# skyzh/tiny-llm

Hardware: AMD Instinct MI355X
Metric: Qwen3-4B int4 decode tokens/sec/GPU; achieved HBM GB/s vs roofline (higher is better)
Workload: dtype bf16; 1 GPU; Qwen3-4B int4 single-prompt KV-cache decode (BASELINE.json configs[1]); decode_steps=2003, batch_per_gpu=1, parallelism=request-parallel x1 (no collective on the data path), page_size=128, graph_replay=True, prefill_step=128, replay_route=aql

## Files before the change

### include/tinyllm_engine.h

```cpp
#ifndef TINYLLM_ENGINE_H
#define TINYLLM_ENGINE_H

#include <stddef.h>
#include <stdint.h>

#ifdef __cplusplus
extern "C" {
#endif

typedef struct tl_engine tl_engine;

typedef struct tl_w4 {
    const uint32_t *weight_dev;
    const void *scales_dev;
    const void *biases_dev;
    int rows;
    int cols;
} tl_w4;

typedef struct tl_layer_weights {
    tl_w4 wqkv, wo, wgu, wdown;
    const void *input_norm_dev;
    const void *post_norm_dev;
    const void *q_norm_dev;
// ... 75 lines not shown
    long parks, unparks, pages_out, pages_in;
    size_t record_bytes;
} tl_swap_stats;
int tl_engine_swap_space(tl_engine *e, int host_pages);
int tl_engine_park(tl_engine *e, int slot);
int tl_engine_unpark(tl_engine *e, int slot);
int tl_engine_slot_parked(const tl_engine *e, int slot);
int tl_engine_step_pages(const tl_engine *e, int batch, int *need, int *obtainable);
int tl_engine_swap_stats(const tl_engine *e, tl_swap_stats *out);
size_t tl_kv_page_record_bytes(const tl_kv_pool_desc *pools_host, int n_pools, int heads, int page_size);
int tl_kv_gather_pages(const tl_kv_pool_desc *pools_dev, const size_t *record_offsets_dev, int n_pools, int heads, int page_size,
                       const int32_t *page_ids_dev, int n_pages, int tail_rows, void *staging_dev, size_t record_bytes, void *stream);
int tl_kv_scatter_pages(const tl_kv_pool_desc *pools_dev, const size_t *record_offsets_dev, int n_pools, int heads, int page_size,
                        const int32_t *page_ids_dev, int n_pages, int tail_rows, const void *staging_dev, size_t record_bytes, void *stream);

int tl_engine_verify(tl_engine *e, int slot, const int32_t *tokens, int n, int32_t *out_ids);

int tl_engine_verify_sampled(tl_engine *e, int slot, const int32_t *tokens, int n, const void *draft_logits_dev, float draft_temperature,
                             int draft_top_k, float draft_top_p, int32_t *out_ids, int *out_count);

int tl_engine_set_token(tl_engine *e, int slot, int32_t token);

int tl_engine_set_sampling(tl_engine *e, int slot, float temperature, int top_k, float top_p, uint64_t seed);

#define TL_MAX_TOP_LOGPROBS 20
typedef struct tl_token_logprob {
    float logprob;
    int32_t top_ids[TL_MAX_TOP_LOGPROBS];
    float top_logprobs[TL_MAX_TOP_LOGPROBS];
} tl_token_logprob;
int tl_engine_set_logprobs(tl_engine *e, int slot, int top_n);
int tl_engine_read_logprobs(tl_engine *e, int slot, int count, tl_token_logprob *out);
int tl_engine_read_pending_logprobs(tl_engine *e, int count, tl_token_logprob *out);

#define TL_MAX_LOGIT_BIAS 1024
int tl_engine_set_penalties(tl_engine *e, int slot, float repetition_penalty, float presence_penalty, float frequency_penalty);
int tl_engine_set_logit_bias(tl_engine *e, int slot, const int32_t *ids, const float *values, int n);

int tl_engine_set_truncation(tl_engine *e, int slot, float min_p, float typical_p);
int tl_engine_set_mirostat(tl_engine *e, int slot, float tau, float eta);
int tl_engine_mirostat_mu(tl_engine *e, int slot, float *mu);
int tl_engine_copy_filtered_logits(tl_engine *e, void *dst_dev, int rows);

typedef struct tl_vocab tl_vocab;
typedef struct tl_grammar tl_grammar;
#define TL_GRAMMAR_END (-1)
int tl_vocab_create(int vocab, const int32_t *offsets, const uint8_t *bytes, void *stream, tl_vocab **out);
void tl_vocab_destroy(tl_vocab *v);
int tl_grammar_create(const tl_vocab *v, int n_states, const uint16_t *table, const uint8_t *accepting, int start, const int32_t *eos_ids,
                      int n_eos, void *stream, tl_grammar **out);
void tl_grammar_destroy(tl_grammar *g);
int tl_engine_set_grammar(tl_engine *e, int slot, const tl_grammar *g);
int tl_engine_grammar_state(tl_engine *e, int slot, int *state, int *accepting);
int tl_grammar_mask_rows(const tl_grammar *g, const void *logits_dev, int rows, const int32_t *states_dev, void *out_dev, void *stream);

int tl_grammar_create_stack(const tl_vocab *v, int n_states, const uint16_t *table, const uint8_t *ops, int n_pop, const uint16_t *pop_table,
                            const uint8_t *accepting, int start, const int32_t *eos_ids, int n_eos, void *stream, tl_grammar **out);
int tl_engine_grammar_config(tl_engine *e, int slot, int *state, int *depth, uint64_t *stack, int *accepting);
int tl_grammar_mask_rows_stack(const tl_grammar *g, const void *logits_dev, int rows, const int32_t *states_dev, const int32_t *depths_dev,
                               const uint64_t *stacks_dev, void *out_dev, void *stream);

int tl_engine_score(tl_engine *e, int slot, const int32_t *tokens, int n, int32_t next_token, float *out_logprobs, int32_t *out_argmax);

#define TL_POOL_LAST 0
#define TL_POOL_MEAN 1
int tl_engine_embed_packed(tl_engine *e, int n_seqs, const int *slots, const int32_t *tokens, const int *lens, const int *finish, int pooling,
                           int normalize, int dim, float *out_host);
int tl_engine_embed(tl_engine *e, int slot, const int32_t *tokens, int n, int finish, int pooling, int normalize, int dim, float *out_host);

#define TL_MAX_LORA_RANK 64
#define TL_MAX_LORA_ADAPTERS 32
enum { TL_LORA_Q, TL_LORA_K, TL_LORA_V, TL_LORA_O, TL_LORA_GATE, TL_LORA_UP, TL_LORA_DOWN, TL_LORA_TARGETS };
typedef struct tl_lora_layer {
    const void *a_dev[TL_LORA_TARGETS], *b_dev[TL_LORA_TARGETS];
} tl_lora_layer;
typedef struct tl_lora_stats {
    int resident;
    size_t bytes;
    long adapter_steps;
    long adapter_prefill_rows;
} tl_lora_stats;
int tl_engine_lora_load(tl_engine *e, const tl_lora_layer *layers, int rank, float scale, int *adapter);
int tl_engine_lora_unload(tl_engine *e, int adapter);
int tl_engine_set_lora(tl_engine *e, int slot, int adapter);
int tl_engine_slot_lora(const tl_engine *e, int slot);
int tl_engine_lora_stats(const tl_engine *e, tl_lora_stats *out);

enum { TL_LORA_ADD = 0, TL_LORA_RESIDUAL_PRE = 1, TL_LORA_SWIGLU = 2 };
typedef struct tl_lora_matrices {
    const void *a_dev, *b_dev;
    int rank, seg_mask;
    float scale;
} tl_lora_matrices;
int tl_lora_rows(const void *x_dev, int rows, int in, int out, const int32_t *row_adapter_dev, const tl_lora_matrices *adapters, int n_adapters,
                 int seg_mode, int seg_end0, int seg_end1, const int *tile_row0, const int *tile_rows, const int *tile_adapter, int n_tiles, int mode,
                 const void *base_or_residual_dev, void *out_dev, const void *norm_w_dev, float eps, void *stream);

#define TL_MAX_STOP_IDS 16
#define TL_MAX_STOP_STRINGS 16
#define TL_MAX_STOP_BYTES 1024
enum { TL_STOP_NONE = 0, TL_STOP_ID = 1, TL_STOP_STRING = 2, TL_STOP_LENGTH = 3 };
typedef struct tl_stop tl_stop;
typedef struct tl_stop_state {
    int32_t reason, index, generated, context;
    uint32_t text_bytes, cut_bytes;
} tl_stop_state;
int tl_stop_create(const tl_vocab *v, const int32_t *ids, int n_ids, const uint8_t *bytes, const int32_t *offsets, int n_strings, void *stream,
                   tl_stop **out);
void tl_stop_destroy(tl_stop *s);
int tl_engine_set_stop(tl_engine *e, int slot, const tl_stop *set, int max_new_tokens);
int tl_engine_stop_state(tl_engine *e, int slot, tl_stop_state *out);
int tl_stop_rows(const tl_stop *set, const int32_t *tokens_dev, int rows, const int32_t *armed_dev, const int32_t *max_new_dev,
                 int32_t *automaton_dev, tl_stop_state *states_dev, void *stream);

int tl_engine_decode(tl_engine *e, int batch, int steps, int use_graph);

int tl_engine_read_tokens(tl_engine *e, int slot, int count, int32_t *out);

int tl_engine_read_pending(tl_engine *e, int count, int32_t *out);

const void *tl_engine_logits_dev(const tl_engine *e);
int tl_engine_copy_logits(tl_engine *e, void *dst_dev, int rows);
int tl_engine_copy_processed_logits(tl_engine *e, void *dst_dev, int rows);
const int32_t *tl_engine_tokens_dev(const tl_engine *e);

int tl_engine_get_stats(const tl_engine *e, tl_engine_stats *out);

const char *tl_engine_replay_route(const tl_engine *e);

size_t tl_engine_step_bytes(const tl_engine *e, int batch);

typedef struct tl_step_profile {
    double kernel_us[8];
    int launches[8];
    double gemv_bytes[5];
    double span_us;
    int clock_khz;
    int n_splits;
} tl_step_profile;
int tl_engine_profile_step(tl_engine *e, int batch, tl_step_profile *out);

typedef struct tl_step_check {
    int launches, written_once_plan, n_splits;
    long double_writes, elements_written;
    int first_launch, first_kind, first_region;
    long first_offset;
} tl_step_check;
int tl_engine_check_step(tl_engine *e, int batch, tl_step_check *out);


typedef struct tl_tiled_w4 tl_tiled_w4;
int tl_tiled_w4_create(const tl_w4 *w, void *stream, tl_tiled_w4 **out);
void tl_tiled_w4_destroy(tl_tiled_w4 *t);

typedef struct tl_linear_info {
    int kernel;
    int launches;
    int rows_per_pass;
    int p[5];
} tl_linear_info;

size_t tl_decode_linear_workspace_bytes(int M, int rows, int cols);
int tl_decode_linear(const tl_tiled_w4 *w, const void *a_dev, void *out_dev, int M, int prologue, int epilogue,
                     const void *norm_w_dev, const void *residual_dev, float eps, int kernel, void *workspace_dev,
                     size_t workspace_bytes, void *stream, tl_linear_info *info);

typedef struct tl_linear_ex {
    const float *merge_ws_dev;
    int n_splits;
    const float *ss_in_dev;
    int ss_in_n;
    float *ss_out_dev;
    const void *norm_out_dev;
    void *out_w_dev;
    int fragment_order;
} tl_linear_ex;
int tl_decode_linear_ex(const tl_tiled_w4 *w, const void *a_dev, void *out_dev, int M, int prologue, int epilogue,
                        const void *norm_w_dev, const void *residual_dev, float eps, int kernel, void *workspace_dev,
                        size_t workspace_bytes, void *stream, const tl_linear_ex *ex, tl_linear_info *info);

int tl_prefill_weights_bf16(const tl_w4 *w, void *out_dev, void *stream);
int tl_prefill_matmul_bf16(const void *a_dev, const void *w_bf16_dev, void *out_dev, int M, int rows, int cols, int epilogue,
                           const void *residual_dev, void *stream);

int tl_decode_gemv_plan(int M, int rows, int cols, int *out5);
int tl_decode_gemv_variant_compiled(int MR, int KS, int CW, int LM);
int tl_decode_batched_plan(int M, int rows, int cols, int *out6);
int tl_decode_batched_variant_compiled(int MB, int GPW);
int tl_decode_streaming_plan(int M, int rows, int cols, int *out4);
int tl_decode_streaming_variant_compiled(int T, int GPW);
int tl_decode_attention_plan(int batch, int max_context, int num_heads, int num_kv_heads, int *out3);

typedef struct tl_attention_info {
    int n_splits, tokens_per_split, heads_per_workgroup;
    int launches;
} tl_attention_info;
size_t tl_decode_attention_fused_workspace_bytes(int batch, int num_heads, int head_dim);
int tl_decode_attention_fused(const void *qkv_dev, const void *q_norm_dev, const void *k_norm_dev, void *key_pages_dev,
                              void *value_pages_dev, const int32_t *block_table_dev, const int32_t *context_lens_dev,
                              void *out_dev, int batch, int num_heads, int num_kv_heads, int head_dim, int page_size,
                              int max_pages, float rope_theta, float eps, int max_context, void *workspace_dev,
                              size_t workspace_bytes, void *stream, tl_attention_info *info);
int tl_decode_attention_fused_fp8(const void *qkv_dev, const void *q_norm_dev, const void *k_norm_dev, void *key_pages_dev,
                                  float *key_scales_dev, void *value_pages_dev, float *value_scales_dev,
                                  const int32_t *block_table_dev, const int32_t *context_lens_dev, void *out_dev, int batch,
                                  int num_heads, int num_kv_heads, int head_dim, int page_size, int max_pages, float rope_theta,
                                  float eps, int max_context, void *workspace_dev, size_t workspace_bytes, void *stream,
                                  tl_attention_info *info);

int tl_sample_logits(const void *logits_dev, int rows, int vocab, const float *temperature_dev, const int32_t *top_k_dev,
                     const float *top_p_dev, const uint64_t *seed_dev, const int32_t *position_dev, int32_t *ids_dev, void *stream);

int tl_spec_sample_rows(const void *target_logits_dev, const void *draft_logits_dev, int rows, int vocab, const int32_t *proposal_dev,
                        const float *temperature_dev, const int32_t *top_k_dev, const float *top_p_dev, const float *draft_temperature_dev,
                        const int32_t *draft_top_k_dev, const float *draft_top_p_dev, const uint64_t *seed_dev, const int32_t *position_dev,
                        int32_t *accept_dev, int32_t *alt_dev, void *stream);

int tl_logprob_rows(const void *logits_dev, int rows, int vocab, const int32_t *ids_dev, int top_n, float *logprob_dev, int32_t *top_ids_dev,
                    float *top_logprobs_dev, void *stream);

int tl_pool_rows(const void *rows_dev, int hidden, int n_seqs, const int *row0, const int *len, const int *finish, const int *prior, int pooling,
                 float *sums_dev, int normalize, int dim, float *out_dev, void *stream);

int tl_truncate_rows(const void *logits_dev, int rows, int vocab, const float *temperature_dev, const float *min_p_dev, const float *typical_p_dev,
                     const float *mu_dev, void *out_dev, float *kept_logsum_dev, void *stream);
int tl_mirostat_update_rows(const void *filtered_dev, int rows, int vocab, const int32_t *ids_dev, const float *temperature_dev,
                            const float *kept_logsum_dev, const float *tau_dev, const float *eta_dev, float *mu_dev, void *stream);

int tl_process_logits(const void *logits_dev, int rows, int vocab, const uint16_t *history_dev, const float *repetition_dev,
                      const float *presence_dev, const float *frequency_dev, const int32_t *bias_ids_dev, const float *bias_values_dev,
                      const int32_t *bias_n_dev, void *out_dev, void *stream);

#ifdef __cplusplus
}
#endif
#endif
```

### tiny-llm_amd/csrc/decode_linear.h

```cpp
#pragma once

#include <algorithm>
#include <cstdlib>
#include <initializer_list>
#include <map>
#include <memory>
#include <string>
#include <vector>

#include "../../include/tinyllm_engine.h"
#include "common.h"
#include "device_block.h"
#include "engine_kernels.h"
#include "qmv.h"
#include "qmv3.h"
#include "qmm3.h"
#include "qmm6.h"
#include "qmm7.h"
#include "gemm8.h"

namespace tl {

#define TL_TRY(expr)                  \
    do {                              \
        const int rc__ = (expr);      \
        if (rc__ != TL_OK) return rc__; \
    } while (0)

struct WrittenOnceCheck {
    char *region[2] = {nullptr, nullptr};
    size_t bytes[2] = {0, 0};
    uint32_t *shadow[2] = {nullptr, nullptr};
    uint8_t *written[2] = {nullptr, nullptr};
    unsigned long long *report = nullptr;
};

struct ProfCtx {
    hipStream_t stream = nullptr;
    const WrittenOnceCheck *check = nullptr;
    DeviceBlock buf_mem, pairs_mem;
    prof_t *buf = nullptr;
    prof_t *pairs = nullptr;
    std::vector<int> kinds;
    int cap = 0;
    bool alloc(const tl_engine_config &c, int batch, hipStream_t st) {
        stream = st;
        const size_t buf_bytes = (size_t)(std::max(c.vocab_size / 4 + 64, 64 * 4 * c.num_kv_heads * batch) + 1024) * 2 * sizeof(prof_t);
        cap = c.num_layers * 12 + 8;
        if (buf_mem.alloc(buf_bytes, "hipMalloc(stamps) failed") != TL_OK || pairs_mem.alloc((size_t)cap * 2 * sizeof(prof_t), "hipMalloc(stamp pairs) failed") != TL_OK)
            return false;
        buf = buf_mem.at<prof_t>(), pairs = pairs_mem.at<prof_t>();
        return hipMemsetAsync(buf, 0, buf_bytes, stream) == hipSuccess;
    }
};

static void prof_after(ProfCtx *pc, int kind, int n_wg) {
    const int idx = (int)pc->kinds.size();
    if (idx >= pc->cap) return;
    hipLaunchKernelGGL(prof_reduce_kernel, dim3(1), dim3(1024), 0, pc->stream, pc->buf, n_wg, pc->pairs + 2 * (size_t)idx);
    pc->kinds.push_back(kind);
    if (pc->check)
        for (int rg = 0; rg < 2; ++rg)
            if (pc->check->bytes[rg])
                hipLaunchKernelGGL(written_once_check_kernel, dim3(1024), dim3(256), 0, pc->stream, (const uint32_t *)pc->check->region[rg],
                                   pc->check->shadow[rg], pc->check->written[rg], pc->check->bytes[rg] / 4, idx, rg, pc->check->report);
}

struct TiledW4 {
    uint32_t *wt = nullptr, *sbt = nullptr;
};
struct TiledW4Mem {
    DeviceBlock wt, sbt;
};
static int tiled_w4_make(const tl_w4 &w, hipStream_t st, TiledW4Mem &mem, TiledW4 &t, const char *alloc_failed, const char *repack_failed) {
    const size_t wbytes = (size_t)w.rows * w.cols / 2, sbytes = (size_t)w.rows * (w.cols / 128) * 4;
    TiledW4Mem m;
    TL_TRY(m.wt.alloc(wbytes + 16384, alloc_failed));
    TL_TRY(m.sbt.alloc(sbytes + 1024, alloc_failed));
    if (repack_w4_tiled(w.weight_dev, (const uint16_t *)w.scales_dev, (const uint16_t *)w.biases_dev, m.wt.at<uint32_t>(), m.sbt.at<uint32_t>(), w.rows,
                        w.cols, st) != 0)
        return fail(TL_ERR_HIP, repack_failed);
    t.wt = m.wt.at<uint32_t>(), t.sbt = m.sbt.at<uint32_t>();
    mem = std::move(m);
    return TL_OK;
}

struct LinearCtx {
    hipStream_t stream = nullptr;
    float rms_norm_eps = 0.f;
    std::map<const uint32_t *, TiledW4> tiled;
    std::map<const uint32_t *, uint16_t *> bf16w;
    uint16_t *xn = nullptr;
    void *splitk_ws = nullptr;
    size_t splitk_ws_bytes = 0;
    uint16_t *gu = nullptr, *tmp = nullptr;
    bool use_gemm8 = true;
    bool fuse_reduce_norm = true;
    bool gemm_fused_epilogue = true;
    bool gemv_producer_ss = true;
    bool gemv_weighted_rows = true;
    bool fuse_norm = true;
    int qmm3_min_rows = 5;
    bool use_qmm3 = true;
    bool use_qmm6 = true;
    bool use_qmm7 = true, force_qmm7 = false;
    tl_linear_info *linfo = nullptr;
    int force_linear = 0;
    int qmm3_mode = -1;
    void read_env() { if (const char *q = getenv("TL_QMM3_MIN_M")) qmm3_min_rows = std::max(1, atoi(q)); }
};

struct KeptPartials {
    const float *partial = nullptr;
    int slices = 0;
    long plane = 0;
};

struct Proj {
    const tl_w4 *w = nullptr;
    const uint16_t *a = nullptr;
    uint16_t *out = nullptr;
    int M = 0;
    int pro = PRO_NONE, epi = EPI_STORE;
    const void *norm_w = nullptr;
    const uint16_t *residual = nullptr;
    int kind = 0;
    const float *ss_in = nullptr;
    int ss_in_n = QM3_SS;
    float *ss_out = nullptr;
    const void *norm_out = nullptr;
    uint16_t *out_w = nullptr;
    bool frag = false;
    int out_w_frag = -1;
    bool keep = false;
    float *planes = nullptr;
    size_t planes_bytes = 0;
    const float *merge_ws = nullptr;
    int n_splits = 0;
    f32x2 *tile_max = nullptr;
};
static Proj proj(const tl_w4 &w, const uint16_t *a, uint16_t *out, int M) { return Proj{&w, a, out, M}; }

struct ProjResult {
    int ss_n = 0;
    KeptPartials kept;
    int maxima_rows = 0;
};

static int check_w4(const tl_w4 &w, int rows, int cols, const char *name) {
    if (!w.weight_dev || !w.scales_dev || !w.biases_dev)
        return fail(TL_ERR_INVALID, std::string("engine: null weight pointer in ") + name);
    if (w.rows != rows || w.cols != cols)
        return fail(TL_ERR_INVALID, std::string("engine: unexpected shape for ") + name + " (got " +
                                        std::to_string(w.rows) + "x" + std::to_string(w.cols) + ", want " +
                                        std::to_string(rows) + "x" + std::to_string(cols) + ")");
    if ((uintptr_t)w.weight_dev % 16 != 0)
        return fail(TL_ERR_INVALID, std::string("engine: weight not 16-byte aligned: ") + name);
    return TL_OK;
}

static void report_launch(const LinearCtx &ctx, int kernel, int launches, int rows_per_pass, std::initializer_list<int> plan = {}) {
    if (!ctx.linfo) return;
    tl_linear_info &li = *ctx.linfo;
    li.kernel = kernel == 1 && li.kernel == 3 ? 3 : kernel;
    li.launches += launches;
    li.rows_per_pass = rows_per_pass;
    std::copy(plan.begin(), plan.end(), li.p);
}

static int engine_qmv(LinearCtx &ctx, const Proj &p, ProfCtx *pc = nullptr, ProjResult *res = nullptr) {
    ProjResult none, &r = res ? *res : none;
    r = ProjResult{};
    const tl_w4 &w = *p.w;
    const int M = p.M;
    const bool merge = p.pro == PRO_ATTN_MERGE;
    bool all_emitted = p.ss_out != nullptr && p.epi == EPI_RESIDUAL && ctx.gemv_producer_ss;
    int step = std::min(M, 8);
    const auto tiled = ctx.tiled.find(w.weight_dev);
    const bool has_tiled = tiled != ctx.tiled.end();
    auto fits = [&](int rows) {
        return (has_tiled && qmv3_plan(rows, w.cols, w.rows).ok) || qmv_plan(rows, w.cols, w.rows).lds <= 150 * 1024;
    };
    while (!fits(step) && step > 1) step = (step + 1) / 2;
    const int out_cols = p.epi == EPI_SWIGLU ? w.rows / 2 : w.rows;
    for (int m0 = 0; m0 < M; m0 += step) {
        QmvArgs args{};
        args.scales = (const uint16_t *)w.scales_dev;
        args.biases = (const uint16_t *)w.biases_dev;
        args.b = w.weight_dev;
        args.a = p.a + (size_t)m0 * w.cols;
        args.out = p.out + (size_t)m0 * out_cols;
        args.norm_w = (const uint16_t *)p.norm_w;
        args.residual = p.residual ? p.residual + (size_t)m0 * w.rows : nullptr;
        args.eps = ctx.rms_norm_eps;
        args.M = std::min(step, M - m0);
        args.N = w.cols;
        args.K = w.rows;
        args.prof = pc ? pc->buf : nullptr;
        const Qmv3Plan p3 = qmv3_plan(args.M, args.N, args.K);
        if (has_tiled && (p3.ok || merge)) {
            Qmv3Args a3{};
            a3.wt = tiled->second.wt;
            a3.sbt = tiled->second.sbt;
            a3.a = merge ? nullptr : args.a;
            a3.merge_ws = merge ? const_cast<float *>(p.merge_ws) : nullptr;
            a3.out = args.out;
            a3.norm_w = args.norm_w;
            a3.residual = args.residual;
            a3.eps = args.eps;
            a3.M = args.M;
            a3.N = args.N;
            a3.K = args.K;
            a3.prof = args.prof;
            if (ctx.gemv_producer_ss) {
                if ((p.pro == PRO_RMSNORM || p.pro == PRO_RMS_WEIGHTED) && p.ss_in && p.ss_in_n > 0)
                    a3.ss_in = p.ss_in + (size_t)m0 * p.ss_in_n, a3.ss_n = p.ss_in_n;
                if (p.epi == EPI_RESIDUAL && p.ss_out) a3.ss_out = p.ss_out + (size_t)m0 * (w.rows / 16);
            }
            if (p.tile_max && p.epi == EPI_STORE && step == M && w.rows % 16 == 0) {
                a3.tile_max = p.tile_max;
                r.maxima_rows = M;
            }
            if (p.out_w) {
                TL_REQUIRE(p.epi == EPI_RESIDUAL && p.norm_out && step == M, "engine: weighted rows need the residual epilogue and one pass");
                a3.norm_out = (const uint16_t *)p.norm_out;
                a3.out_w = p.out_w;
            }
            if ((merge ? launch_qmv3_attn_merge_bf16(a3, p.n_splits, ctx.stream) : launch_qmv3_bf16(a3, p.pro, p.epi, ctx.stream)) != 0)
                return fail(TL_ERR_UNSUPPORTED, merge ? "engine: no wo GEMV that merges the attention partials for this shape" : "engine: MFMA GEMV launch failed");
            if (pc) prof_after(pc, p.kind, p3.blocks);
            report_launch(ctx, 1, 1, step, {p3.MR, p3.KS, p3.CW, p3.LM, p3.blocks});
            continue;
        }
        all_emitted = false;
        TL_REQUIRE(p.out_w == nullptr && p.pro != PRO_RMS_WEIGHTED && !merge, "engine: weighted rows are a route of the MFMA GEMV only");
        if (launch_qmv_fused_bf16(args, p.pro, p.epi, ctx.stream) != 0)
            return fail(TL_ERR_UNSUPPORTED, "engine: no GEMV configuration for this shape");
        if (pc) prof_after(pc, p.kind, qmv_plan(args.M, args.N, args.K).blocks);
        report_launch(ctx, 3, 1, step);
    }
    TL_CHECK_LAUNCH(merge ? "engine wo gemv with merge" : "engine gemv");
    if (all_emitted && w.rows % 16 == 0) r.ss_n = w.rows / 16;
    return TL_OK;
}

static int ensure_splitk(const LinearCtx &ctx, size_t bytes) {
    if (bytes <= ctx.splitk_ws_bytes) return TL_OK;
    return fail(TL_ERR_INVALID, "engine: matmul workspace too small for this shape (sized at tl_engine_create: " +
                                    std::to_string(ctx.splitk_ws_bytes) + " bytes, need " + std::to_string(bytes) + ")");
}

static int engine_qmm(LinearCtx &ctx, const tl_w4 &w, const uint16_t *a, uint16_t *out, int M) {
    const size_t need = tl_quantized_matmul_workspace_bytes(M, w.cols, w.rows, TL_BF16, 1, 1);
    TL_TRY(ensure_splitk(ctx, need));
    return tl_quantized_matmul(w.scales_dev, w.biases_dev, a, w.weight_dev, out, M, w.cols, w.rows, 128, 4, TL_BF16, 1, 1,
                               ctx.splitk_ws, ctx.splitk_ws_bytes, ctx.stream);
}

constexpr int GEMM8_MIN_ROWS = 1792;
static bool gemm8_wins(int M) { return M >= GEMM8_MIN_ROWS; }
static int engine_gemm(LinearCtx &ctx, const Proj &p, bool *norm_done = nullptr) {
    const tl_w4 &w = *p.w;
    const int M = p.M;
    if (norm_done) *norm_done = false;
    if (ctx.use_gemm8 && gemm8_wins(M)) {
        const auto wb = ctx.bf16w.find(w.weight_dev);
        if (wb != ctx.bf16w.end() && gemm8_applicable(M, w.rows, w.cols)) {
            Gemm8Args g{};
            g.a = p.a, g.w = wb->second, g.out = p.out, g.residual = p.residual, g.M = M, g.N = w.rows, g.K = w.cols;
            if (launch_gemm8_bf16(g, p.epi, ctx.stream) != 0) return fail(TL_ERR_UNSUPPORTED, "engine: bf16 GEMM launch failed");
            TL_CHECK_LAUNCH("engine bf16 matmul");
            return TL_OK;
        }
    }
    if (p.epi != EPI_STORE && M > 8 && ctx.gemm_fused_epilogue) {
        const size_t need = tl_quantized_matmul_workspace_bytes(M, w.cols, w.rows, TL_BF16, 1, 1);
        TL_TRY(ensure_splitk(ctx, need));
        TL_TRY(qmm_bf16_epilogue(w.scales_dev, w.biases_dev, p.a, w.weight_dev, p.out, M, w.cols, w.rows, p.epi, p.residual, ctx.splitk_ws,
                                 ctx.splitk_ws_bytes, ctx.stream, ctx.fuse_reduce_norm ? (const uint16_t *)p.norm_out : nullptr, p.out_w,
                                 ctx.rms_norm_eps, norm_done));
        TL_CHECK_LAUNCH("engine matmul");
        return TL_OK;
    }
    uint16_t *plain = p.epi == EPI_STORE ? p.out : (p.epi == EPI_SWIGLU ? ctx.gu : ctx.tmp);
    TL_TRY(engine_qmm(ctx, w, p.a, plain, M));
    if (p.epi == EPI_SWIGLU) {
        const long n4 = (long)M * (w.rows / 2) / 4;
        hipLaunchKernelGGL(swiglu_interleaved_kernel, dim3(ceil_div(n4, 256)), dim3(256), 0, ctx.stream, plain, p.out, n4);
    } else if (p.epi == EPI_RESIDUAL) {
        const long n8 = (long)M * w.rows / 8;
        hipLaunchKernelGGL(residual_add_kernel, dim3(ceil_div(n8, 256)), dim3(256), 0, ctx.stream, p.residual, plain, p.out, n8);
    }
    TL_CHECK_LAUNCH("engine matmul");
    return TL_OK;
}

static bool qmm6_takes(const LinearCtx &ctx, const tl_w4 &w, int M) {
    return ctx.use_qmm6 && ctx.force_linear == 0 && M >= ctx.qmm3_min_rows && M <= 64 && ctx.tiled.count(w.weight_dev) != 0 &&
           qmm6_plan(M, w.cols, w.rows).ok;
}
static int engine_qmm6(LinearCtx &ctx, const Proj &p, ProfCtx *pc = nullptr, ProjResult *res = nullptr) {
    ProjResult none, &r = res ? *res : none;
    r = ProjResult{};
    const tl_w4 &w = *p.w;
    const int M = p.M;
    const auto tiled = ctx.tiled.find(w.weight_dev);
    TL_REQUIRE(tiled != ctx.tiled.end(), "engine: the register-resident matmul needs the tiled weights");
    const bool a_frag = p.frag && p.ss_in != nullptr && p.epi != EPI_RESIDUAL;
    const Qmm7Plan p7 = (ctx.use_qmm7 || ctx.force_qmm7) && a_frag && p.out_w == nullptr ? qmm7_plan(M, w.cols, w.rows) : Qmm7Plan{};
    TL_REQUIRE(p7.ok || !ctx.force_qmm7, "engine: the row-streaming matmul takes weighted rows in fragment order (store / SwiGLU) at the shapes of qmm7_plan");
    const Qmm6Plan pl = qmm6_plan(M, w.cols, w.rows, a_frag);
    TL_REQUIRE(p7.ok || pl.ok, "engine: the register-resident matmul does not cover this shape");
    Qmm6Args q{};
    q.wt = tiled->second.wt;
    q.sbt = tiled->second.sbt;
    q.a = p.a;
    q.out = p.out;
    q.residual = p.residual;
    q.norm_out = (const uint16_t *)p.norm_out;
    q.out_w = p.out_w;
    q.ss = p.ss_in;
    q.ss_n = p.ss_in ? p.ss_in_n : 0;
    q.ss_out = p.epi == EPI_RESIDUAL ? p.ss_out : nullptr;
    q.eps = ctx.rms_norm_eps;
    q.M = M;
    q.N = w.cols;
    q.K = w.rows;
    q.prof = pc ? pc->buf : nullptr;
    q.a_frag = a_frag;
    q.out_w_frag = (p.out_w_frag >= 0 ? p.out_w_frag != 0 : p.frag) && p.out_w != nullptr;
    int n_wg = 0;
    if (p7.ok) {
        if (launch_qmm7_bf16(q, p.epi, ctx.stream, &n_wg) != 0) return fail(TL_ERR_UNSUPPORTED, "engine: row-streaming matmul launch failed");
        if (pc) prof_after(pc, p.kind, n_wg);
        report_launch(ctx, 6, 1, p7.MB * 16, {p7.MB, p7.GPW, p7.T, p7.row_blocks, n_wg});
        TL_CHECK_LAUNCH("engine row-streaming matmul");
        return TL_OK;
    }
    if (launch_qmm6_bf16(q, p.epi, ctx.stream, &n_wg) != 0) return fail(TL_ERR_UNSUPPORTED, "engine: register-resident matmul launch failed");
    if (pc) prof_after(pc, p.kind, n_wg);
    if (q.ss_out) r.ss_n = w.rows / 16;
    report_launch(ctx, 5, 1, pl.MB * 16, {pl.MB, pl.GPW, pl.NSETS, pl.row_blocks, n_wg});
    TL_CHECK_LAUNCH("engine register-resident matmul");
    return TL_OK;
}

static bool gemv_takes_rows(const LinearCtx &ctx, int M) {
    return ctx.force_linear == 1 || (ctx.force_linear != 2 && (M < ctx.qmm3_min_rows || (M <= 8 && !ctx.use_qmm3)));
}
static bool weighted_rows_apply(const LinearCtx &ctx, const tl_w4 &producer, const tl_w4 &consumer, int M) {
    if (!ctx.gemv_weighted_rows || !ctx.gemv_producer_ss || !gemv_takes_rows(ctx, M) || M > 8) return false;
    if (ctx.tiled.count(producer.weight_dev) == 0 || ctx.tiled.count(consumer.weight_dev) == 0) return false;
    const Qmv3Plan pp = qmv3_plan(M, producer.cols, producer.rows), pcn = qmv3_plan(M, consumer.cols, consumer.rows);
    if (!pp.ok || !pcn.ok || producer.rows != consumer.cols) return false;
    return qmv3_takes_weighted_rows(pcn, consumer.cols, producer.rows / 16);
}
static bool takes_skinny_matmul(const LinearCtx &ctx, const tl_w4 &w, int M) {
    return !gemv_takes_rows(ctx, M) && ctx.use_qmm3 && M <= 64 && ctx.tiled.count(w.weight_dev) != 0 && qmm3_plan(M, w.cols, w.rows, ctx.qmm3_mode).ok;
}

static int engine_linear(LinearCtx &ctx, const Proj &p, ProfCtx *pc = nullptr, ProjResult *res = nullptr) {
    ProjResult none, &r = res ? *res : none;
    r = ProjResult{};
    const tl_w4 &w = *p.w;
    const int M = p.M;
    if (gemv_takes_rows(ctx, M)) return engine_qmv(ctx, p, pc, &r);
    TL_REQUIRE(p.pro != PRO_ATTN_MERGE, "engine: merged attention partials are a route of the fused GEMV only");
    TL_REQUIRE(p.pro != PRO_RMS_WEIGHTED && (p.out_w == nullptr || (p.epi == EPI_RESIDUAL && p.norm_out != nullptr)),
               "engine: the skinny matmul leaves weighted rows behind a residual epilogue only, and takes none");
    const float *ss_in = qmm3_takes_ss(p.ss_in_n) ? p.ss_in : nullptr;
    const uint16_t *in = p.a;
    if (takes_skinny_matmul(ctx, w, M)) {
        const auto tiled = ctx.tiled.find(w.weight_dev);
        const Qmm3Plan p3 = qmm3_plan(M, w.cols, w.rows, ctx.qmm3_mode);
        const bool fused_norm = p.pro == PRO_RMSNORM && ss_in != nullptr && ctx.fuse_norm;
        if (p.pro == PRO_RMSNORM && !fused_norm) {
            TL_TRY(tl_rms_norm(p.a, p.norm_w, ctx.xn, M, w.cols, ctx.rms_norm_eps, TL_BF16, ctx.stream));
            in = ctx.xn;
        }
        if (p.planes) TL_REQUIRE(p3.partial_bytes <= p.planes_bytes, "engine: per-layer slice planes too small for this shape");
        else TL_TRY(ensure_splitk(ctx, p3.partial_bytes));
        Qmm3Args q{};
        q.wt = tiled->second.wt;
        q.sbt = tiled->second.sbt;
        q.a = in;
        q.partial = p.planes ? p.planes : (float *)ctx.splitk_ws;
        q.M = M;
        q.N = w.cols;
        q.K = w.rows;
        q.prof = pc ? pc->buf : nullptr;
        q.norm_w = (const uint16_t *)p.norm_w;
        q.ss = ss_in;
        q.ss_n = p.ss_in_n;
        q.eps = ctx.rms_norm_eps;
        if (launch_qmm3_bf16(q, ctx.stream, fused_norm ? PRO_RMSNORM : PRO_NONE, ctx.qmm3_mode) != 0)
            return fail(TL_ERR_UNSUPPORTED, "engine: skinny matmul launch failed");
        if (pc) prof_after(pc, p.kind, p3.persistent ? p3.grid_x : p3.grid_x * p3.slices);
        float *ss_dst = (p.ss_out && ctx.fuse_norm && qmm3_reduce_can_emit_ss(p.epi, w.rows)) ? p.ss_out : nullptr;
        const bool kept = p.keep && p.epi == EPI_STORE && ss_dst == nullptr;
        if (kept) {
            r.kept.partial = q.partial;
            r.kept.slices = p3.slices;
            r.kept.plane = (long)M * w.rows;
        } else {
            int reduce_wg = 0;
            if (launch_qmm3_reduce_bf16(q.partial, p3.slices, M, w.rows, p.epi, p.residual, p.out, q.prof, ctx.stream, ss_dst, &reduce_wg,
                                        p.out_w ? (const uint16_t *)p.norm_out : nullptr, p.out_w, p.frag ? 1 : 0) != 0)
                return fail(TL_ERR_UNSUPPORTED, "engine: skinny matmul reduction launch failed");
            if (pc) prof_after(pc, p.kind, reduce_wg);
        }
        r.ss_n = ss_dst != nullptr ? QM3_SS : 0;
        TL_CHECK_LAUNCH("engine skinny matmul");
        report_launch(ctx, 2, (kept ? 1 : 2) + (p.pro == PRO_RMSNORM && !fused_norm ? 1 : 0), M,
                      {p3.MB, p3.persistent ? 0 : p3.TW, p3.LM, p3.slices, p3.persistent ? p3.grid_x : p3.grid_x * p3.slices});
        return TL_OK;
    }
    if (ctx.force_linear == 2) return fail(TL_ERR_UNSUPPORTED, "engine: the skinny matmul does not cover this shape");
    TL_REQUIRE(p.out_w == nullptr, "engine: no kernel leaves weighted rows for this shape");
    if (M <= 8) return engine_qmv(ctx, p, pc, &r);
    Proj g = p;
    if (p.pro == PRO_RMSNORM) {
        TL_TRY(tl_rms_norm(p.a, p.norm_w, ctx.xn, M, w.cols, ctx.rms_norm_eps, TL_BF16, ctx.stream));
        g.a = ctx.xn;
    }
    if (ctx.linfo) ctx.linfo->kernel = 4;
    g.norm_out = nullptr;
    return engine_gemm(ctx, g);
}

struct LayerRoute {
    bool batched = false;
    bool qkv6 = false, wo6 = false;
    enum Down { DOWN_ROUTER, DOWN_SLICED_WEIGHTED, DOWN_QMM6 } down = DOWN_ROUTER;
    bool gemv_weighted = false;
    bool batched_written_once() const { return batched && qkv6 && down != DOWN_ROUTER; }
};
static LayerRoute plan_layer(const LinearCtx &ctx, const tl_layer_weights &w, int batch, bool is_moe) {
    LayerRoute r;
    if (is_moe || w.wgu.weight_dev == nullptr) return r;
    auto sliced_leaves_weighted = [&](const tl_w4 &m) {
        return takes_skinny_matmul(ctx, m, batch) && ctx.fuse_norm && qmm3_reduce_can_emit_ss(EPI_RESIDUAL, m.rows);
    };
    auto qmm6_leaves_weighted = [&](const tl_w4 &m) { return qmm6_takes(ctx, m, batch) && qmm3_takes_ss(m.rows / 16); };
    r.gemv_weighted = weighted_rows_apply(ctx, w.wo, w.wgu, batch);
    r.wo6 = qmm6_leaves_weighted(w.wo);
    r.batched = qmm6_takes(ctx, w.wgu, batch) && (r.wo6 || sliced_leaves_weighted(w.wo));
    r.qkv6 = qmm6_takes(ctx, w.wqkv, batch);
    r.down = sliced_leaves_weighted(w.wdown) ? LayerRoute::DOWN_SLICED_WEIGHTED
                                             : (qmm6_leaves_weighted(w.wdown) ? LayerRoute::DOWN_QMM6 : LayerRoute::DOWN_ROUTER);
    return r;
}
static bool rows_travel_in_fragment_order(const LinearCtx &ctx, const tl_layer_weights &first, int batch) {
    if (batch > 8) return true;
    if (!ctx.use_qmm7 || !first.wgu.weight_dev) return false;
    return qmm7_plan(batch, first.wgu.cols, first.wgu.rows).ok && qmm7_plan(batch, first.wqkv.cols, first.wqkv.rows).ok;
}

}

struct tl_tiled_w4 {
    tl_w4 w{};
    tl::TiledW4 t{};
    tl::TiledW4Mem mem;
};

extern "C" int tl_tiled_w4_create(const tl_w4 *w, void *stream, tl_tiled_w4 **out) {
    using namespace tl;
    TL_REQUIRE(w && out, "tiled_w4_create: null argument");
    TL_TRY(check_w4(*w, w->rows, w->cols, "tiled_w4_create"));
    TL_REQUIRE(w->rows > 0 && w->rows % 16 == 0 && w->cols > 0 && w->cols % 128 == 0,
               "tiled_w4_create: rows must be a multiple of 16 and cols a multiple of 128");
    auto t = std::make_unique<tl_tiled_w4>();
    t->w = *w;
    TL_TRY(tiled_w4_make(*w, (hipStream_t)stream, t->mem, t->t, "tiled_w4_create: hipMalloc failed", "tiled_w4_create: repack launch failed"));
    *out = t.release();
    return TL_OK;
}

extern "C" void tl_tiled_w4_destroy(tl_tiled_w4 *t) { delete t; }

extern "C" size_t tl_decode_linear_workspace_bytes(int M, int rows, int cols) {
    using namespace tl;
    if (M <= 0 || rows <= 0 || cols <= 0) return 0;
    size_t need = align_up((size_t)((M + 15) / 16 * 16) * cols * 2, 256);
    size_t partial = 0;
    for (int mode = 0; mode < 2; ++mode) {
        const Qmm3Plan p3 = qmm3_plan(std::min(M, 64), cols, rows, mode);
        if (p3.ok) partial = std::max(partial, p3.partial_bytes);
    }
    return need + partial;
}

static int decode_linear_impl(const tl_tiled_w4 *w, const void *a_dev, void *out_dev, int M, int prologue, int epilogue,
                              const void *norm_w_dev, const void *residual_dev, float eps, int kernel, void *workspace_dev,
                              size_t workspace_bytes, void *stream, const tl_linear_ex *ex, tl_linear_info *info) {
    using namespace tl;
    TL_REQUIRE(w && out_dev, "decode_linear: null argument");
    TL_REQUIRE(M >= 1 && M <= 64, "decode_linear: between 1 and 64 activation rows");
    TL_REQUIRE(prologue == PRO_NONE || prologue == PRO_RMSNORM || (ex && (prologue == PRO_ATTN_MERGE || prologue == PRO_RMS_WEIGHTED)),
               "decode_linear: prologue is 0 (none) or 1 (RMSNorm); tl_decode_linear_ex also takes 2 (merge of attention partials) and 3 (weighted rows)");
    TL_REQUIRE(epilogue == EPI_STORE || epilogue == EPI_RESIDUAL || epilogue == EPI_SWIGLU,
               "decode_linear: epilogue is 0 (store), 1 (residual add) or 2 (SwiGLU over interleaved rows)");
    TL_REQUIRE(prologue == PRO_ATTN_MERGE || a_dev, "decode_linear: null activation rows");
    TL_REQUIRE(prologue != PRO_RMSNORM || norm_w_dev, "decode_linear: the RMSNorm prologue needs its weight");
    TL_REQUIRE(epilogue != EPI_RESIDUAL || residual_dev, "decode_linear: the residual epilogue needs the residual rows");
    TL_REQUIRE(kernel >= 0 && kernel <= 6,
               "decode_linear: kernel is 0 (engine routing), 1 (fused GEMV), 2 (skinny matmul), 3 / 4 (its one-shot / persistent grid), 5 (register-resident matmul), 6 (row-streaming matmul)");
    TL_REQUIRE(epilogue != EPI_SWIGLU || w->w.rows % 2 == 0, "decode_linear: SwiGLU needs an even number of weight rows");
    TL_REQUIRE((prologue == PRO_NONE && epilogue != EPI_SWIGLU) || (prologue == PRO_RMSNORM && epilogue != EPI_RESIDUAL) ||
                   (prologue == PRO_ATTN_MERGE && epilogue == EPI_RESIDUAL) || (prologue == PRO_RMS_WEIGHTED && epilogue == EPI_SWIGLU) ||
                   ((kernel == 5 || kernel == 6) && prologue == PRO_RMS_WEIGHTED && epilogue == EPI_STORE),
               "decode_linear: no fused variant for this prologue / epilogue pair");
    const size_t need = tl_decode_linear_workspace_bytes(M, w->w.rows, w->w.cols);
    TL_REQUIRE(workspace_dev && workspace_bytes >= need, "decode_linear: workspace is missing or too small");
    if (info) *info = tl_linear_info{};
    LinearCtx ctx;
    ctx.rms_norm_eps = eps;
    ctx.stream = (hipStream_t)stream;
    ctx.tiled[w->w.weight_dev] = w->t;
    ctx.xn = (uint16_t *)workspace_dev;
    const size_t xn_bytes = align_up((size_t)((M + 15) / 16 * 16) * w->w.cols * 2, 256);
    ctx.splitk_ws = (char *)workspace_dev + xn_bytes;
    ctx.splitk_ws_bytes = workspace_bytes - xn_bytes;
    ctx.force_linear = kernel >= 2 && kernel <= 4 ? 2 : (kernel >= 5 ? 0 : kernel);
    ctx.use_qmm7 = false, ctx.force_qmm7 = kernel == 6;
    ctx.qmm3_mode = kernel == 3 ? 0 : (kernel == 4 ? 1 : -1);
    ctx.linfo = info;
    ctx.read_env();
    Proj p = proj(w->w, (const uint16_t *)a_dev, (uint16_t *)out_dev, M);
    p.pro = prologue, p.epi = epilogue, p.norm_w = norm_w_dev, p.residual = (const uint16_t *)residual_dev;
    if (ex) {
        p.ss_out = ex->ss_out_dev;
        p.norm_out = ex->norm_out_dev, p.out_w = (uint16_t *)ex->out_w_dev;
    }
    if (kernel == 6 && (prologue != PRO_RMS_WEIGHTED || epilogue == EPI_RESIDUAL))
        return fail(TL_ERR_INVALID, "decode_linear: the row-streaming matmul takes weighted rows with ss_in (prologue 3) and stores or applies SwiGLU (epilogue 0 / 2)");
    if (kernel == 5 || kernel == 6) {
        const bool weighted = prologue == PRO_RMS_WEIGHTED;
        if (prologue == PRO_RMSNORM || prologue == PRO_ATTN_MERGE)
            return fail(TL_ERR_INVALID, "decode_linear: the register-resident matmul takes plain rows (prologue 0) or weighted rows with ss_in (prologue 3)");
        if (weighted && (!ex || !ex->ss_in_dev || !qmm3_takes_ss(ex->ss_in_n)))
            return fail(TL_ERR_INVALID, "decode_linear_ex: weighted rows need ss_in (a multiple of 4, at most 256 partials per row)");
        if (ex && ((ex->out_w_dev != nullptr) != (ex->norm_out_dev != nullptr) || ((ex->out_w_dev || ex->ss_out_dev) && epilogue != EPI_RESIDUAL)))
            return fail(TL_ERR_INVALID, "decode_linear_ex: ss_out / (norm_out, out_w) belong to the residual epilogue; norm_out and out_w come together");
        if (kernel == 5 && !qmm6_plan(M, w->w.cols, w->w.rows).ok)
            return fail(TL_ERR_UNSUPPORTED, "decode_linear: the register-resident matmul does not cover this shape");
        if (kernel == 6 && !qmm7_plan(M, w->w.cols, w->w.rows).ok)
            return fail(TL_ERR_UNSUPPORTED, "decode_linear: the row-streaming matmul does not cover this shape");
        if (weighted && !ex->fragment_order) {
            const long n8 = (long)M * w->w.cols / 8;
            hipLaunchKernelGGL(weight_rows_kernel, dim3(ceil_div(n8, 256)), dim3(256), 0, ctx.stream, p.a, (const uint16_t *)nullptr, ctx.xn, n8, w->w.cols / 8, 1);
            p.a = ctx.xn;
        }
        if (weighted) p.ss_in = ex->ss_in_dev, p.ss_in_n = ex->ss_in_n;
        p.frag = weighted;
        p.out_w_frag = ex && ex->fragment_order ? 1 : 0;
        return engine_qmm6(ctx, p);
    }
    if (!ex) return engine_linear(ctx, p);
    const bool skinny_forced = kernel >= 2 && kernel <= 4;
    const bool gemv_only = prologue == PRO_ATTN_MERGE || prologue == PRO_RMS_WEIGHTED || ex->ss_out_dev || (ex->out_w_dev && !skinny_forced);
    if (gemv_only && !(kernel == 1 || (kernel == 0 && M < ctx.qmm3_min_rows)))
        return fail(TL_ERR_INVALID, "decode_linear_ex: merged partials, weighted rows, ss_out and out_w are routes of the fused GEMV (kernel 1, or 0 with fewer than 5 rows)");
    if ((ex->out_w_dev != nullptr) != (ex->norm_out_dev != nullptr) || (ex->out_w_dev && epilogue != EPI_RESIDUAL) ||
        (ex->ss_out_dev && epilogue != EPI_RESIDUAL))
        return fail(TL_ERR_INVALID, "decode_linear_ex: ss_out / (norm_out, out_w) belong to the residual epilogue; norm_out and out_w come together");
    if (ex->ss_in_dev && (ex->ss_in_n <= 0 || !(prologue == PRO_RMSNORM || prologue == PRO_RMS_WEIGHTED)))
        return fail(TL_ERR_INVALID, "decode_linear_ex: ss_in needs ss_in_n > 0 and a normalising prologue (1 or 3)");
    if (prologue == PRO_ATTN_MERGE) {
        if (M != 1 || !ex->merge_ws_dev) return fail(TL_ERR_INVALID, "decode_linear_ex: the merging prologue takes ONE row and the split partials (merge_ws_dev)");
        p.merge_ws = ex->merge_ws_dev, p.n_splits = ex->n_splits;
    }
    if (prologue == PRO_RMS_WEIGHTED) {
        const Qmv3Plan pl = qmv3_plan(std::min(M, 8), w->w.cols, w->w.rows);
        if (!ex->ss_in_dev || M > 8 || !qmv3_takes_weighted_rows(pl, w->w.cols, ex->ss_in_n))
            return fail(TL_ERR_INVALID, "decode_linear_ex: weighted rows need ss_in (a multiple of 4, at most 256 partials per row), at most 8 rows and a row that fits the staging registers");
    }
    p.ss_in = ex->ss_in_dev, p.ss_in_n = ex->ss_in_n;
    if (gemv_only || kernel == 1 || (kernel == 0 && M < ctx.qmm3_min_rows)) {
        if (M > 8) return fail(TL_ERR_INVALID, "decode_linear_ex: the fused GEMV takes at most 8 rows");
        ProjResult r;
        TL_TRY(engine_qmv(ctx, p, nullptr, &r));
        if (ex->ss_out_dev && r.ss_n != w->w.rows / 16)
            return fail(TL_ERR_UNSUPPORTED, "decode_linear_ex: the GEMV that ran left no sums of squares (packed-dot fallback or several passes)");
        return TL_OK;
    }
    if (ex->ss_in_dev && !qmm3_takes_ss(ex->ss_in_n))
        return fail(TL_ERR_INVALID, "decode_linear_ex: the skinny matmul reads a multiple of 4, at most 256, partial sums of squares per row");
    if (!ex->ss_in_dev) p.ss_in_n = 0;
    p.frag = ex->fragment_order != 0;
    return engine_linear(ctx, p);
}

extern "C" int tl_decode_linear(const tl_tiled_w4 *w, const void *a_dev, void *out_dev, int M, int prologue, int epilogue,
                                const void *norm_w_dev, const void *residual_dev, float eps, int kernel, void *workspace_dev,
                                size_t workspace_bytes, void *stream, tl_linear_info *info) {
    return decode_linear_impl(w, a_dev, out_dev, M, prologue, epilogue, norm_w_dev, residual_dev, eps, kernel, workspace_dev,
                              workspace_bytes, stream, nullptr, info);
}

extern "C" int tl_decode_linear_ex(const tl_tiled_w4 *w, const void *a_dev, void *out_dev, int M, int prologue, int epilogue,
                                   const void *norm_w_dev, const void *residual_dev, float eps, int kernel, void *workspace_dev,
                                   size_t workspace_bytes, void *stream, const tl_linear_ex *ex, tl_linear_info *info) {
    TL_REQUIRE(ex, "decode_linear_ex: null extension block (use tl_decode_linear)");
    return decode_linear_impl(w, a_dev, out_dev, M, prologue, epilogue, norm_w_dev, residual_dev, eps, kernel, workspace_dev,
                              workspace_bytes, stream, ex, info);
}
```

### tiny-llm_amd/csrc/engine.hip

```cpp
#include <dlfcn.h>

#include <cstddef>
#include <cstring>
#include <memory>

#include "decode_linear.h"
#include "device_block.h"
#include "step_end.h"
#include "logit_process.h"
#include "truncate.h"
#include "grammar_stack.h"
#include "attn_mfma.h"
#include "aql.h"
#include "prefix_cache.h"
#include "kv_copy.h"
#include "kv_swap.h"
#include "pool.h"
#include "lora.h"
#include "slot_table.h"
#include "stop.h"
#include "stop_set.h"

namespace tl {

// ... 1296 lines not shown
    const size_t o_log = carve((size_t)std::max(c.max_batch, 8) * c.vocab_size * 2);
    const size_t o_vid = carve(8 * 4);
    const size_t o_tmax = carve((size_t)8 * (c.vocab_size / 16 + 1) * sizeof(f32x2));
    const size_t ss_per_row = (size_t)std::max(QM3_SS, c.hidden_size / 16 + 1);
    const size_t o_ssx = carve((size_t)c.max_batch * ss_per_row * 4);
    const size_t o_ssh = carve((size_t)c.max_batch * ss_per_row * 4);
    const size_t ws_row = (size_t)c.head_dim + ATTN_WS_PAD;
    e->attn_ws_bytes = std::max((size_t)std::max(c.max_batch * 64, 4 * 256) * c.num_heads * ws_row * 4, (size_t)c.num_heads * 8 * 64 * ws_row * 4);
    for (int L = 1; L <= c.max_prefill_rows; ++L)
        e->attn_ws_bytes = std::max(e->attn_ws_bytes, tl_paged_attention_workspace_bytes(c.num_heads, L, c.head_dim, c.page_size,
                                                                                         c.max_pages_per_seq, c.num_heads,
                                                                                         c.num_kv_heads, 0));
    const size_t o_ws = carve(e->attn_ws_bytes);
    e->arena_bytes = carve.off;

    TL_TRY(e->arena.alloc(e->arena_bytes, "engine_create: hipMalloc(arena) failed"));
    TL_TRY(e->smp_mem.alloc((size_t)c.max_batch * 20, "engine_create: hipMalloc(sampling) failed"));
    e->smp_seed = e->smp_mem.at<uint64_t>();
    e->smp_temp = e->smp_mem.at<float>((size_t)c.max_batch * 8);
    e->smp_topk = e->smp_mem.at<int32_t>((size_t)c.max_batch * 12);
    e->smp_topp = e->smp_mem.at<float>((size_t)c.max_batch * 16);
    if (hipMemsetAsync(e->smp_mem.at(), 0, (size_t)c.max_batch * 20, e->stream) != hipSuccess) return fail(TL_ERR_HIP, "engine_create: memset failed");
    e->layer_pool_elems = (size_t)c.num_pages * c.num_kv_heads * c.page_size * c.head_dim;
    const size_t pool_bytes = e->layer_pool_elems * e->kv_elem_bytes() * c.num_layers;
    TL_TRY(e->kv_mem[0].alloc(pool_bytes, "engine_create: hipMalloc(key pages) failed"));
    TL_TRY(e->kv_mem[1].alloc(pool_bytes, "engine_create: hipMalloc(value pages) failed"));
    e->kpool = e->kv_mem[0].at<uint16_t>(), e->vpool = e->kv_mem[1].at<uint16_t>();
    e->kv_bytes = 2 * pool_bytes;
    if (kv_format == TL_KV_FP8_E4M3) {
        e->layer_scale_elems = (size_t)c.num_pages * c.num_kv_heads * c.page_size;
        const size_t scale_bytes = e->layer_scale_elems * 4 * c.num_layers;
        TL_TRY(e->kv_mem[2].alloc(scale_bytes, "engine_create: hipMalloc(key scales) failed"));
        TL_TRY(e->kv_mem[3].alloc(scale_bytes, "engine_create: hipMalloc(value scales) failed"));
        e->kscale_pool = e->kv_mem[2].at<float>(), e->vscale_pool = e->kv_mem[3].at<float>();
        if (hipMemsetAsync(e->kscale_pool, 0, scale_bytes, e->stream) != hipSuccess ||
            hipMemsetAsync(e->vscale_pool, 0, scale_bytes, e->stream) != hipSuccess)
            return fail(TL_ERR_HIP, "engine_create: memset(KV scales) failed");
        e->kv_bytes += 2 * scale_bytes;
    }
    if (hipMemsetAsync(e->kpool, 0, pool_bytes, e->stream) != hipSuccess ||
        hipMemsetAsync(e->vpool, 0, pool_bytes, e->stream) != hipSuccess)
        return fail(TL_ERR_HIP, "engine_create: memset(KV pools) failed");

    char *A = e->arena.at();
    e->block_table = (int32_t *)(A + o_bt);
    e->context_lens = (int32_t *)(A + o_ctx);
    e->tokens = (int32_t *)(A + o_tok);
    e->live = (int32_t *)(A + o_live);
    e->produced = (int32_t *)(A + o_prod);
    e->ring = (int32_t *)(A + o_ring);
    e->scratch_ctx = (int32_t *)(A + o_sctx);
    e->prefill_tokens = (int32_t *)(A + o_ptok);
    e->x = (uint16_t *)(A + o_x);
    e->h = (uint16_t *)(A + o_h);
    e->xn = (uint16_t *)(A + o_xn);
    e->lin.tmp = (uint16_t *)(A + o_tmp);
    e->qkv = (uint16_t *)(A + o_qkv);
    e->q_t = (uint16_t *)(A + o_qt);
    e->attn_t = (uint16_t *)(A + o_at);
    e->attn = (uint16_t *)(A + o_attn);
    e->lin.gu = (uint16_t *)(A + o_gu);
    e->act = (uint16_t *)(A + o_act);
    e->logits = (uint16_t *)(A + o_log);
    e->attn_ws = (float *)(A + o_ws);
    e->verify_ids = (int32_t *)(A + o_vid);
    e->lm_tile_max = (f32x2 *)(A + o_tmax);
    e->ss_x = (float *)(A + o_ssx);
    e->ss_h = (float *)(A + o_ssh);
    e->lin.stream = e->stream, e->lin.rms_norm_eps = c.rms_norm_eps, e->lin.xn = e->xn;
    e->lin.read_env();
    read_attention_knobs(e);
    const char *aql_env = getenv("TL_AQL");
    if (aql_env == nullptr || atoi(aql_env) != 0) {
        {
            AqlRuntime &rt = AqlRuntime::for_device(e->device);
            e->aql_rt = &rt;
            std::string why;
            e->aql_queue = std::make_unique<AqlQueue>();
            if (!rt.ensure_loaded(library_dir()) || !e->aql_queue->create(rt, why)) {
                e->aql_why = rt.ok() ? why : rt.why();
                e->aql_queue.reset();
                if (aql_env != nullptr) {
                    return fail(TL_ERR_UNSUPPORTED, "engine_create: TL_AQL=1 but the AQL route is not available: " + e->aql_why);
                }
            }
        }
        if (e->aql_queue) {
            e->aql_on = true;
            e->aql_fences.inner_acquire = e->aql_fences.inner_release = HSA_FENCE_SCOPE_NONE;
            {
                const int rows = std::min(c.max_batch, 64);
                const size_t ssr = (size_t)std::max(QM3_SS, c.hidden_size / 16 + 1);
                const size_t b_xf = align_up((size_t)((rows + 15) / 16 * 16) * c.hidden_size * 2, 256);
                const size_t b_x = align_up((size_t)rows * c.hidden_size * 2, 256), b_qkv = align_up((size_t)rows * qkv_dim * 2, 256),
                             b_attn = align_up((size_t)rows * q_dim * 2, 256), b_act = align_up((size_t)rows * c.intermediate_size * 2, 256),
                             b_ss = align_up((size_t)rows * ssr * 4, 256),
                             b_ws = align_up((size_t)std::min(rows * 64, std::max(4 * 64, std::min(rows * 16, 1024))) * c.num_heads * ws_row * 4, 256);
                size_t b_pl[2] = {0, 0};
                for (int M = std::min(5, e->lin.qmm3_min_rows); M <= rows; ++M) {
                    const Qmm3Plan pw = qmm3_plan(M, q_dim, c.hidden_size, -1), pd = qmm3_plan(M, c.intermediate_size, c.hidden_size, -1);
                    if (pw.ok) b_pl[0] = std::max(b_pl[0], align_up(pw.partial_bytes, 256));
                    if (pd.ok) b_pl[1] = std::max(b_pl[1], align_up(pd.partial_bytes, 256));
                }
                const size_t per_layer = 2 * b_x + 2 * b_xf + b_qkv + b_attn + b_act + 2 * b_ss + b_ws + b_pl[0] + b_pl[1];
                TL_TRY(e->layer_act_mem.alloc(per_layer * c.num_layers, "engine_create: hipMalloc(per-layer decode activations) failed"));
                if (hipMemsetAsync(e->layer_act_mem.at(), 0, per_layer * c.num_layers, e->stream) != hipSuccess)
                    return fail(TL_ERR_HIP, "engine_create: hipMalloc(per-layer decode activations) failed");
                e->layer_act.resize(c.num_layers);
                for (int l = 0; l < c.num_layers; ++l) {
                    char *m = e->layer_act_mem.at((size_t)l * per_layer);
                    tl_engine::LayerAct &a = e->layer_act[l];
                    a.x_out = (uint16_t *)m, m += b_x;
                    a.h = (uint16_t *)m, m += b_x;
                    a.xn = (uint16_t *)m, m += b_xf;
                    a.xw = (uint16_t *)m, m += b_xf;
                    a.qkv = (uint16_t *)m, m += b_qkv;
                    a.attn = (uint16_t *)m, m += b_attn;
                    a.act = (uint16_t *)m, m += b_act;
                    a.ss_x_out = (float *)m, m += b_ss;
                    a.ss_h = (float *)m, m += b_ss;
                    a.attn_ws = (float *)m, m += b_ws;
                    a.planes[0] = (float *)m, m += b_pl[0];
                    a.planes[1] = (float *)m;
                }
                e->layer_plane_bytes[0] = b_pl[0], e->layer_plane_bytes[1] = b_pl[1];
                e->layer_act_bytes = per_layer * c.num_layers;
                e->layer_act_rows = rows;
                e->layer_ws_bytes = b_ws;
            }
        }
    }

    if (hipMemsetAsync(e->arena.at(), 0, o_x, e->stream) != hipSuccess) return fail(TL_ERR_HIP, "engine_create: memset failed");
    const int bt_n = c.max_batch * c.max_pages_per_seq;
    hipLaunchKernelGGL(fill_i32_kernel, dim3(ceil_div(bt_n, 256)), dim3(256), 0, e->stream, e->block_table, -1, bt_n);
    if (hipGetLastError() != hipSuccess) return fail(TL_ERR_HIP, "engine_create: block-table init failed");

    {
        const long max_pos = std::min<long>((long)c.max_pages_per_seq * c.page_size + 1, 1 << 20);
        e->rope_positions = (int)max_pos;
        const int half = c.head_dim / 2;
        TL_TRY(e->rope_table_mem.alloc((size_t)max_pos * half * sizeof(float2), "engine_create: hipMalloc(rope table) failed"));
        e->rope_table = e->rope_table_mem.at<float2>();
        hipLaunchKernelGGL(rope_table_kernel, dim3(ceil_div(max_pos * half, 256)), dim3(256), 0, e->stream, e->rope_table,
                           (int)max_pos, half, c.rope_theta);
        if (hipGetLastError() != hipSuccess) return fail(TL_ERR_HIP, "engine_create: rope table kernel failed");
        TL_TRY(e->rope_cur_mem.alloc((size_t)c.max_batch * half * sizeof(float2), "engine_create: hipMalloc(rope state) failed"));
        e->rope_cur = e->rope_cur_mem.at<float2>();
        if (hipMemsetAsync(e->rope_cur, 0, (size_t)c.max_batch * half * sizeof(float2), e->stream) != hipSuccess)
            return fail(TL_ERR_HIP, "engine_create: hipMalloc(rope state) failed");
    }

    {
        auto add_tiled = [&](const tl_w4 &w) -> bool {
            if (w.rows % 16 != 0 || w.cols % 128 != 0 || e->lin.tiled.count(w.weight_dev)) return true;
            const char *failed = "engine_create: hipMalloc(tiled weights) failed";
            e->tiled_mem.emplace_back();
            if (tiled_w4_make(w, e->stream, e->tiled_mem.back(), e->lin.tiled[w.weight_dev], failed, failed) != TL_OK) return false;
            e->tiled_bytes += (size_t)w.rows * w.cols / 2 + (size_t)w.rows * (w.cols / 128) * 4;
            return true;
        };
        bool ok = true;
        for (const auto &l : e->layers) {
            ok = ok && add_tiled(l.wqkv) && add_tiled(l.wo);
            if (l.wgu.weight_dev) ok = ok && add_tiled(l.wgu) && add_tiled(l.wdown);
        }
        ok = ok && add_tiled(e->head());
        if (!ok) return fail(TL_ERR_HIP, "engine_create: hipMalloc(tiled weights) failed");
    }
    if (c.max_prefill_rows >= GEMM8_MIN_ROWS) {
        auto add_bf16 = [&](const tl_w4 &w) -> bool {
            if (!w.weight_dev || w.cols % 128 != 0 || e->lin.bf16w.count(w.weight_dev) || !gemm8_applicable(c.max_prefill_rows, w.rows, w.cols)) return true;
            const size_t bytes = (size_t)w.rows * w.cols * 2;
            DeviceBlock copy;
            if (copy.alloc(bytes, "engine_create: hipMalloc(bf16 weights for the prefill GEMM) failed") != TL_OK) return false;
            uint16_t *wb = copy.at<uint16_t>();
            if (dequant_w4_to_bf16(w.weight_dev, (const uint16_t *)w.scales_dev, (const uint16_t *)w.biases_dev, wb, w.rows, w.cols, e->stream) != 0) return false;
            e->bf16w_mem.push_back(std::move(copy));
            e->lin.bf16w[w.weight_dev] = wb;
            e->bf16w_bytes += bytes;
            return true;
        };
        bool ok = true;
        for (const auto &l : e->layers) {
            ok = ok && add_bf16(l.wqkv) && add_bf16(l.wo);
            if (l.wgu.weight_dev) ok = ok && add_bf16(l.wgu) && add_bf16(l.wdown);
        }
        if (!ok) return fail(TL_ERR_HIP, "engine_create: hipMalloc(bf16 weights for the prefill GEMM) failed");
    }

    {
        size_t need = 0;
        const tl_layer_weights *dense = &e->layers[0];
        for (const auto &l : e->layers)
            if (l.wgu.weight_dev) {
                dense = &l;
                break;
            }
        const tl_w4 *mats[5] = {&e->layers[0].wqkv, &e->layers[0].wo, &dense->wgu, &dense->wdown, &e->head()};
        for (const tl_w4 *w : mats) {
            if (!w->weight_dev) continue;
            for (int M = 1; M <= std::min(64, e->rows_cap); ++M) {
                const Qmm3Plan p3 = qmm3_plan(M, w->cols, w->rows);
                if (p3.ok) need = std::max(need, p3.partial_bytes);
            }
            for (int M = 9; M <= e->rows_cap; ++M)
                need = std::max(need, tl_quantized_matmul_workspace_bytes(M, w->cols, w->rows, TL_BF16, 1, 1));
        }
        if (need > 0) {
            TL_TRY(e->splitk_mem.alloc(need, "engine_create: hipMalloc(matmul workspace) failed"));
            e->lin.splitk_ws = e->splitk_mem.at<void>(), e->lin.splitk_ws_bytes = need;
        }
    }

    e->moe.assign(c.num_layers, tl_moe_weights{});
    e->table.init(c.max_batch, c.num_pages, c.page_size, c.max_pages_per_seq);
    e->smp.assign(c.max_batch, tl_engine::SampleParams{});
    e->pen.assign(c.max_batch, tl_engine::PenaltyParams{});
    e->trn.assign(c.max_batch, tl_engine::TruncParams{});
    e->gr_pending.assign(c.max_batch, 0);
    e->emb_rows.assign(c.max_batch, -1);
    e->lora_of.assign(c.max_batch, LORA_NONE);
    e->stop.assign(c.max_batch, tl_engine::StopSlot{});
    e->stats.kv_bytes = e->kv_bytes;
    e->stats.workspace_bytes = e->arena_bytes + e->tiled_bytes + e->bf16w_bytes;
    *out = owner.release();
    return TL_OK;
}

extern "C" int tl_engine_set_moe_layer(tl_engine *e, int layer, const tl_moe_weights *w) {
    TL_REQUIRE(e && w, "engine_set_moe_layer: null argument");
    const tl_engine_config &c = e->cfg;
    TL_REQUIRE(layer >= 0 && layer < c.num_layers, "engine_set_moe_layer: layer out of range");
    TL_REQUIRE(e->plans.empty() && e->stats.decode_steps == 0 && e->stats.prefill_tokens == 0,
               "engine_set_moe_layer: call it before the first prefill / decode");
    TL_REQUIRE(w->num_experts > 0 && w->num_experts <= 1024 && w->experts_per_token > 0 && w->experts_per_token <= 16 &&
                   w->experts_per_token <= w->num_experts,
               "engine_set_moe_layer: need 1 <= experts_per_token <= min(16, num_experts) and num_experts <= 1024");
    TL_REQUIRE(w->intermediate_size > 0 && w->intermediate_size % 128 == 0, "engine_set_moe_layer: intermediate_size must be a positive multiple of 128");
    TL_TRY(check_w4(w->router, w->num_experts, c.hidden_size, "moe router"));
    TL_REQUIRE(w->gate_dev && w->up_dev && w->down_dev && w->gate_scales_dev && w->gate_biases_dev && w->up_scales_dev &&
                   w->up_biases_dev && w->down_scales_dev && w->down_biases_dev,
               "engine_set_moe_layer: null expert tensor");
    TL_REQUIRE((long)e->rows_cap * w->experts_per_token <= 65535, "engine_set_moe_layer: max_prefill_rows x experts_per_token must stay below 65536 (one grouped launch)");
    for (int M : {1, 8, 9, e->rows_cap})
        TL_REQUIRE(tl_quantized_matmul_workspace_bytes(std::min(M, e->rows_cap), c.hidden_size, w->num_experts, TL_BF16, 1, 1) <= e->lin.splitk_ws_bytes,
                   "engine_set_moe_layer: the router matmul does not fit the engine's matmul workspace");
    const int k = std::max(e->moe_k_max, w->experts_per_token), E = std::max(e->moe_e_max, w->num_experts),
              I = std::max(e->moe_i_max, w->intermediate_size);
    if (k != e->moe_k_max || E != e->moe_e_max || I != e->moe_i_max) {
        const size_t R = (size_t)e->rows_cap;
        Carve carve;
        const size_t o_log = carve(R * E * 2), o_ids = carve(R * k * 4), o_sc = carve(R * k * 2), o_g = carve(R * k * I * 2),
                     o_u = carve(R * k * I * 2), o_a = carve(R * k * I * 2), o_y = carve(R * k * c.hidden_size * 2);
        TL_HIP(hipStreamSynchronize(e->stream));
        TL_TRY(e->moe_ws.alloc(carve.off, "hipMalloc((void **)&e->moe_ws, carve.off): " + std::string(hipGetErrorString(hipErrorOutOfMemory))));
        e->moe_ws_bytes = carve.off;
        char *A = e->moe_ws.at();
        e->moe_logits = (uint16_t *)(A + o_log);
        e->moe_ids = (int32_t *)(A + o_ids);
        e->moe_scores = (uint16_t *)(A + o_sc);
        e->moe_gate = (uint16_t *)(A + o_g);
        e->moe_up = (uint16_t *)(A + o_u);
        e->moe_act = (uint16_t *)(A + o_a);
        e->moe_y = (uint16_t *)(A + o_y);
        e->moe_k_max = k, e->moe_e_max = E, e->moe_i_max = I;
        e->stats.workspace_bytes = e->arena_bytes + e->tiled_bytes + e->moe_ws_bytes;
    }
    e->moe[layer] = *w;
    if (e->layer_act_mem) {
        TL_HIP(hipStreamSynchronize(e->stream));
        e->layer_act_mem.reset();
        e->layer_act.clear();
        e->layer_act_rows = 0, e->layer_act_bytes = 0, e->layer_ws_bytes = 0;
        e->layer_plane_bytes[0] = e->layer_plane_bytes[1] = 0;
    }
    return TL_OK;
}

extern "C" int tl_engine_set_option(tl_engine *e, const char *name, int value) {
    TL_REQUIRE(e && name, "engine_set_option: null argument");
    TL_REQUIRE(e->plans.empty() && e->stats.decode_steps == 0 && e->stats.prefill_tokens == 0,
               "engine_set_option: call it before the first prefill / decode (captured steps hold the routes they were captured with)");
    const std::string n = name;
    const bool on = value != 0;
    if (n == "qmm3") e->lin.use_qmm3 = on;
    else if (n == "qmm6") e->lin.use_qmm6 = on;
    else if (n == "qmm7") e->lin.use_qmm7 = on;
    else if (n == "attn_qkv_partials") e->attn_qkv_partials = on;
    else if (n == "lmhead_tile_max") e->lm_tile_max_on = on;
    else if (n == "gemm_fused_epilogue") e->lin.gemm_fused_epilogue = on;
    else if (n == "gemm8") e->lin.use_gemm8 = on;
    else if (n == "prefill_reduce_norm") e->lin.fuse_reduce_norm = on;
    else if (n == "aql_fences") e->aql_fences.inner_acquire = e->aql_fences.inner_release = on ? HSA_FENCE_SCOPE_AGENT : HSA_FENCE_SCOPE_NONE;
    else return fail(TL_ERR_INVALID, "engine_set_option: unknown option '" + n + "' (qmm3, qmm6, qmm7, gemm8, prefill_reduce_norm, attn_qkv_partials, lmhead_tile_max, gemm_fused_epilogue, aql_fences)");
    return TL_OK;
}

static void drop_plans(tl_engine *e) {
    for (auto &kv : e->plans) (void)hipGraphExecDestroy(kv.second.exec);
    e->plans.clear();
}

extern "C" void tl_engine_destroy(tl_engine *e) {
    if (!e) return;
    (void)aql_drain(e);
    (void)hipStreamSynchronize(e->stream);
    drop_plans(e);
    delete e;
}

extern "C" int tl_engine_kv_format(const tl_engine *e) { return e ? e->kv_format : TL_KV_BF16; }

extern "C" const char *tl_engine_replay_route(const tl_engine *e) {
    static thread_local std::string text;
    if (!e) return "";
    text = e->aql_on ? std::string("aql") : ("hipgraph" + (e->aql_why.empty() ? std::string() : ": " + e->aql_why));
    const char *why = e->aql_on ? graph_only_reason(step_features(e, 0, e->cfg.max_batch)) : nullptr;
    if (why) text = std::string("hipgraph: ") + why;
    return text.c_str();
}

extern "C" int tl_engine_synchronize(tl_engine *e) {
    TL_REQUIRE(e, "engine_synchronize: null engine");
    TL_HIP(hipStreamSynchronize(e->stream));
    return TL_OK;
}

extern "C" int tl_engine_begin(tl_engine *e, int slot) {
    TL_REQUIRE(e, "engine: null engine");
    TL_TRY(table_rc(e->table.begin(slot)));
    Pokes pk;
    pk.emplace_back(e->live + slot, 1);
    pk.emplace_back(e->context_lens + slot, 0);
    pk.emplace_back(e->produced + slot, 0);
    pk.emplace_back(e->tokens + slot, 0);
    TL_TRY(poke(e, pk));
    return settings_reset(e, slot);
}

extern "C" int tl_engine_reserve(tl_engine *e, int slot, int total_tokens) {
    TL_TRY(slot_check_unparked(e, slot));
    TL_REQUIRE(total_tokens >= 0, "engine_reserve: total_tokens must be nonnegative");
    SlotEdits ed;
    Pokes pk;
    TL_TRY(table_rc(e->table.reserve(slot, total_tokens, ed)));
    TL_TRY(apply_edits(e, ed, pk));
    return poke(e, pk);
}

extern "C" int tl_engine_release(tl_engine *e, int slot) {
    TL_REQUIRE(e, "engine: null engine");
    SlotEdits ed;
    Pokes pk;
    TL_TRY(table_rc(e->table.release(slot, ed)));
    TL_TRY(apply_edits(e, ed, pk));
    pk.emplace_back(e->live + slot, 0);
    pk.emplace_back(e->context_lens + slot, 0);
    pk.emplace_back(e->tokens + slot, 0);
    TL_TRY(poke(e, pk));
    return settings_reset(e, slot);
}

extern "C" int tl_engine_rewind(tl_engine *e, int slot, int n) {
    TL_TRY(slot_check_unparked(e, slot));
    TL_REQUIRE(!e->pen[slot].processes(), "engine_rewind: the slot processes its logits (its history would keep the dropped tokens; make it neutral first)");
    TL_REQUIRE(!e->trn[slot].mirostat(), "engine_rewind: the slot has Mirostat on (mu would no longer belong to the tokens held; switch it off first)");
    SlotEdits ed;
    Pokes pk;
    TL_TRY(table_rc(e->table.rewind(slot, n, ed)));
    e->emb_rows[slot] = -1;
    TL_TRY(apply_edits(e, ed, pk));
    pk.emplace_back(e->context_lens + slot, e->table.slots[slot].ctx);
    return poke(e, pk);
}

extern "C" int tl_engine_fork(tl_engine *e, int src, int dst) {
    TL_REQUIRE(e, "engine: null engine");
    TL_TRY(stop_reconcile(e));
    SlotEdits ed;
    Pokes pk;
    TL_TRY(table_rc(e->table.fork(src, dst, ed)));
    TL_TRY(apply_edits(e, ed, pk));
    pk.emplace_back(e->live + dst, e->table.slots[dst].stopped ? 0 : 1);
    pk.emplace_back(e->context_lens + dst, e->table.slots[dst].ctx);
    pk.emplace_back(e->produced + dst, 0);
    TL_TRY(poke(e, pk));
    return settings_carry(e, src, dst, false);
}

static int ensure_pool_table(tl_engine *e) {
    if (e->kv_pools_dev) return TL_OK;
    const tl_engine_config &c = e->cfg;
    std::vector<tl_kv_pool_desc> pools;
    for (int l = 0; l < c.num_layers; ++l) {
        pools.push_back({e->layer_k(l), (size_t)c.head_dim * e->kv_elem_bytes()});
        pools.push_back({e->layer_v(l), (size_t)c.head_dim * e->kv_elem_bytes()});
        if (e->kv_format == TL_KV_FP8_E4M3) {
            pools.push_back({e->layer_ks(l), sizeof(float)});
            pools.push_back({e->layer_vs(l), sizeof(float)});
        }
    }
    TL_TRY(alloc_filled(e->kv_pools_mem, pools.size() * sizeof(tl_kv_pool_desc), "engine: hipMalloc(pool table) failed", [&](char *m) -> int {
        const hipError_t rc = hipMemcpy(m, pools.data(), pools.size() * sizeof(tl_kv_pool_desc), hipMemcpyHostToDevice);
        return rc == hipSuccess ? TL_OK : fail(TL_ERR_HIP, std::string("engine: hipMemcpy(pool table): ") + hipGetErrorString(rc));
    }));
    e->kv_pools_dev = e->kv_pools_mem.at<tl_kv_pool_desc>();
    e->kv_pools_n = (int)pools.size();
    e->kv_pools_host = std::move(pools);
    return TL_OK;
}

extern "C" int tl_engine_prefix_cache(tl_engine *e, int enabled, int max_retained_pages) {
    TL_REQUIRE(e, "engine_prefix_cache: null engine");
    TL_REQUIRE(enabled == 0 || enabled == 1, "engine_prefix_cache: enabled is 0 or 1");
    TL_REQUIRE(max_retained_pages >= 0, "engine_prefix_cache: max_retained_pages must be nonnegative (0 = no cap)");
    if (!enabled) {
        e->table.prefix_disable();
        return TL_OK;
    }
    TL_TRY(ensure_pool_table(e));
    e->table.prefix_enable(max_retained_pages);
    return TL_OK;
}

extern "C" int tl_engine_prefix_clear(tl_engine *e) {
    TL_REQUIRE(e, "engine_prefix_clear: null engine");
    e->table.pool.clear();
    return TL_OK;
}

extern "C" int tl_engine_prefix_stats(const tl_engine *e, tl_prefix_stats *out) {
    TL_REQUIRE(e && out, "engine_prefix_stats: null argument");
    const PagePool &pool = e->table.pool;
    const PrefixCounters &k = pool.ctr;
    *out = tl_prefix_stats{k.lookups, k.hits, k.tokens_matched, k.tail_rows_copied, k.pages_registered, k.pages_evicted,
                           pool.n_entries, pool.retained, pool.max_retained, pool.enabled ? 1 : 0};
    return TL_OK;
}

extern "C" int tl_engine_prefix_extend(tl_engine *e, int slot, const int32_t *tokens, int n) {
    TL_TRY(slot_check_unparked(e, slot));
    TL_REQUIRE(tokens && n >= 1, "engine_prefix_extend: need at least one token");
    if (!e->table.pool.enabled || e->lora_slot(slot)) return TL_OK;
    for (int i = 0; i < n; ++i) TL_REQUIRE(tokens[i] >= 0 && tokens[i] < e->cfg.vocab_size, "engine_prefix_extend: token id out of range");
    return table_rc(e->table.extend(slot, tokens, n));
}

// ... 1623 lines not shown
    launch_embed_slots(e, batch);
    for (int rg = 0; rg < 2 && ok; ++rg)
        if (ck.bytes[rg]) ok = hipMemcpyAsync(ck.shadow[rg], ck.region[rg], ck.bytes[rg], hipMemcpyDeviceToDevice, e->stream) == hipSuccess &&
                               hipMemsetAsync(ck.written[rg], 0, ck.bytes[rg] / 2, e->stream) == hipSuccess;
    if (!ok) return fail(TL_ERR_HIP, "engine_check_step: shadow copy failed");
    SplitPlan sp;
    int rc = prepare_step(e, batch, &sp);
    if (rc == TL_OK) {
        pc.check = &ck;
        rc = enqueue_step(e, batch, sp, step_features(e, 0, batch), &pc);
    }
    if (rc != TL_OK) return rc;
    e->warmed = true;
    step_done(e, batch);
    (void)stop_reconcile(e);
    unsigned long long report[8] = {0};
    hipError_t he = hipStreamSynchronize(e->stream);
    if (he == hipSuccess) he = hipMemcpy(report, ck.report, sizeof(report), hipMemcpyDeviceToHost);
    const std::vector<int> &kinds = pc.kinds;
    if (he != hipSuccess) return fail(TL_ERR_HIP, std::string("engine_check_step: ") + hipGetErrorString(he));
    out->launches = (int)kinds.size();
    out->written_once_plan = e->step_written_once ? 1 : 0;
    out->n_splits = sp.n_splits;
    out->double_writes = (long)report[0];
    out->elements_written = (long)report[3];
    if (report[0]) {
        out->first_launch = (int)report[1];
        out->first_kind = report[1] < kinds.size() ? kinds[report[1]] : -1;
        out->first_region = (int)report[2];
        out->first_offset = (long)report[4];
    }
    return TL_OK;
}

extern "C" int tl_prefill_weights_bf16(const tl_w4 *w, void *out_dev, void *stream) {
    TL_REQUIRE(w && out_dev, "prefill_weights_bf16: null argument");
    TL_TRY(check_w4(*w, w->rows, w->cols, "prefill_weights_bf16"));
    TL_REQUIRE(w->cols % 128 == 0, "prefill_weights_bf16: columns must be a multiple of the quantisation group (128)");
    if (dequant_w4_to_bf16(w->weight_dev, (const uint16_t *)w->scales_dev, (const uint16_t *)w->biases_dev, (uint16_t *)out_dev, w->rows, w->cols, (hipStream_t)stream) != 0)
        return fail(TL_ERR_HIP, "prefill_weights_bf16: launch failed");
    return TL_OK;
}
extern "C" int tl_prefill_matmul_bf16(const void *a_dev, const void *w_bf16_dev, void *out_dev, int M, int rows, int cols, int epilogue,
                                      const void *residual_dev, void *stream) {
    TL_REQUIRE(a_dev && w_bf16_dev && out_dev, "prefill_matmul_bf16: null argument");
    TL_REQUIRE(epilogue == EPI_STORE || epilogue == EPI_RESIDUAL || epilogue == EPI_SWIGLU, "prefill_matmul_bf16: epilogue is 0 (store), 1 (residual add) or 2 (SwiGLU over interleaved rows)");
    TL_REQUIRE(epilogue != EPI_RESIDUAL || residual_dev, "prefill_matmul_bf16: the residual epilogue needs the residual rows");
    TL_REQUIRE(gemm8_applicable(M, rows, cols), "prefill_matmul_bf16: needs M >= 1, an even number of weight rows and columns in whole 64-wide steps");
    Gemm8Args g{};
    g.a = (const uint16_t *)a_dev, g.w = (const uint16_t *)w_bf16_dev, g.out = (uint16_t *)out_dev, g.residual = (const uint16_t *)residual_dev;
    g.M = M, g.N = rows, g.K = cols;
    if (launch_gemm8_bf16(g, epilogue, (hipStream_t)stream) != 0) return fail(TL_ERR_UNSUPPORTED, "prefill_matmul_bf16: launch failed");
    TL_CHECK_LAUNCH("prefill_matmul_bf16");
    return TL_OK;
}

__global__ __launch_bounds__(64) void rope_rows_kernel(const int32_t *__restrict__ context_lens, float2 *__restrict__ rope_cur,
                                                       int half, float base) {
    const int b = blockIdx.x;
    const int pos = context_lens[b];
    for (int item = threadIdx.x; item < half; item += 64) {
        const float fp = -(float)item / (float)half;
        const float angle = (float)pos * exp2f(fp * log2f(base));
        float sn, cs;
        sincosf(angle, &sn, &cs);
        rope_cur[(long)b * half + item] = make_float2(cs, sn);
    }
}

extern "C" size_t tl_decode_attention_fused_workspace_bytes(int batch, int num_heads, int head_dim) {
    if (batch <= 0 || num_heads <= 0 || head_dim <= 0) return 0;
    return align_up((size_t)batch * (head_dim / 2) * sizeof(float2), 256) +
           (size_t)batch * num_heads * 256 * (head_dim + ATTN_WS_PAD) * sizeof(float);
}

static int decode_attention_fused_impl(const void *qkv_dev, const void *q_norm_dev, const void *k_norm_dev, void *key_pages_dev,
                                       float *key_scales_dev, void *value_pages_dev, float *value_scales_dev,
                                       const int32_t *block_table_dev, const int32_t *context_lens_dev, void *out_dev, int batch,
                                       int num_heads, int num_kv_heads, int head_dim, int page_size, int max_pages, float rope_theta,
                                       float eps, int max_context, void *workspace_dev, size_t workspace_bytes, void *stream,
                                       tl_attention_info *info) {
    TL_REQUIRE(qkv_dev && q_norm_dev && k_norm_dev && key_pages_dev && value_pages_dev && block_table_dev && context_lens_dev &&
                   out_dev, "decode_attention_fused: null pointer");
    TL_REQUIRE(batch >= 1 && batch <= 256, "decode_attention_fused: between 1 and 256 sequences");
    TL_REQUIRE(num_heads > 0 && num_kv_heads > 0 && num_heads % num_kv_heads == 0,
               "decode_attention_fused: num_heads must be divisible by num_kv_heads");
    TL_REQUIRE(head_dim == 32 || head_dim == 64 || head_dim == 128, "decode_attention_fused: head_dim must be 32, 64 or 128");
    TL_REQUIRE(page_size > 0 && max_pages > 0 && max_context >= 0, "decode_attention_fused: bad page geometry");
    const size_t need = tl_decode_attention_fused_workspace_bytes(batch, num_heads, head_dim);
    TL_REQUIRE(workspace_dev && workspace_bytes >= need, "decode_attention_fused: workspace is missing or too small");
    tl_engine e;
    e.cfg.num_heads = num_heads;
    e.cfg.num_kv_heads = num_kv_heads;
    e.cfg.head_dim = head_dim;
    e.cfg.page_size = page_size;
    e.cfg.max_pages_per_seq = max_pages;
    e.cfg.rope_theta = rope_theta;
    e.cfg.rms_norm_eps = eps;
    e.stream = (hipStream_t)stream;
    e.block_table = const_cast<int32_t *>(block_table_dev);
    e.context_lens = const_cast<int32_t *>(context_lens_dev);
    e.rope_cur = (float2 *)workspace_dev;
    const size_t rc_bytes = align_up((size_t)batch * (head_dim / 2) * sizeof(float2), 256);
    e.attn_ws_bytes = workspace_bytes - rc_bytes;
    read_attention_knobs(&e);
    hipLaunchKernelGGL(rope_rows_kernel, dim3(batch), dim3(64), 0, e.stream, context_lens_dev, e.rope_cur, head_dim / 2, rope_theta);
    TL_CHECK_LAUNCH("decode_attention_fused rope");
    const SplitPlan sp = pick_decode_splits(&e, batch, std::max(1, max_context + 1));
    AttnCall at{};
    at.qkv = (const uint16_t *)qkv_dev, at.q_norm = q_norm_dev, at.k_norm = k_norm_dev, at.out = (uint16_t *)out_dev;
    at.key_pages = (uint16_t *)key_pages_dev, at.value_pages = (uint16_t *)value_pages_dev, at.key_scales = key_scales_dev, at.value_scales = value_scales_dev;
    at.ws = (float *)((char *)workspace_dev + rc_bytes);
    const int rc = engine_attention(&e, at, batch, sp, nullptr);
    if (info) {
        info->n_splits = sp.n_splits;
        info->tokens_per_split = sp.tokens_per_split;
        info->heads_per_workgroup = sp.rq;
        info->launches = e.last_attn_launches;
    }
    return rc;
}

extern "C" int tl_decode_attention_fused(const void *qkv_dev, const void *q_norm_dev, const void *k_norm_dev,
                                         void *key_pages_dev, void *value_pages_dev, const int32_t *block_table_dev,
                                         const int32_t *context_lens_dev, void *out_dev, int batch, int num_heads,
                                         int num_kv_heads, int head_dim, int page_size, int max_pages, float rope_theta,
                                         float eps, int max_context, void *workspace_dev, size_t workspace_bytes,
                                         void *stream, tl_attention_info *info) {
    return decode_attention_fused_impl(qkv_dev, q_norm_dev, k_norm_dev, key_pages_dev, nullptr, value_pages_dev, nullptr, block_table_dev,
                                       context_lens_dev, out_dev, batch, num_heads, num_kv_heads, head_dim, page_size, max_pages, rope_theta,
                                       eps, max_context, workspace_dev, workspace_bytes, stream, info);
}

extern "C" int tl_decode_attention_fused_fp8(const void *qkv_dev, const void *q_norm_dev, const void *k_norm_dev, void *key_pages_dev,
                                             float *key_scales_dev, void *value_pages_dev, float *value_scales_dev,
                                             const int32_t *block_table_dev, const int32_t *context_lens_dev, void *out_dev, int batch,
                                             int num_heads, int num_kv_heads, int head_dim, int page_size, int max_pages,
                                             float rope_theta, float eps, int max_context, void *workspace_dev, size_t workspace_bytes,
                                             void *stream, tl_attention_info *info) {
    TL_REQUIRE(key_scales_dev && value_scales_dev, "decode_attention_fused_fp8: null scale pointer");
    TL_REQUIRE(head_dim == 128, "decode_attention_fused_fp8: FP8 pages need head_dim 128");
    return decode_attention_fused_impl(qkv_dev, q_norm_dev, k_norm_dev, key_pages_dev, key_scales_dev, value_pages_dev, value_scales_dev,
                                       block_table_dev, context_lens_dev, out_dev, batch, num_heads, num_kv_heads, head_dim, page_size,
                                       max_pages, rope_theta, eps, max_context, workspace_dev, workspace_bytes, stream, info);
}

extern "C" int tl_decode_gemv_plan(int M, int rows, int cols, int *out5) {
    if (!out5 || M < 1 || rows <= 0 || cols <= 0) return 0;
    const Qmv3Plan pl = qmv3_plan(M, cols, rows);
    out5[0] = pl.MR, out5[1] = pl.KS, out5[2] = pl.CW, out5[3] = pl.LM, out5[4] = pl.blocks;
    return pl.ok ? 1 : 0;
}
extern "C" int tl_decode_gemv_variant_compiled(int MR, int KS, int CW, int LM) { return qmv3_variant_in_table(MR, KS, CW, LM) ? 1 : 0; }
extern "C" int tl_decode_batched_plan(int M, int rows, int cols, int *out6) {
    if (!out6 || M < 1 || rows <= 0 || cols <= 0) return 0;
    const Qmm6Plan pl = qmm6_plan(M, cols, rows);
    out6[0] = pl.MB, out6[1] = pl.GPW, out6[2] = pl.NSETS, out6[3] = pl.row_blocks, out6[4] = pl.wgs, out6[5] = pl.tiles_per_wg;
    return pl.ok ? 1 : 0;
}
extern "C" int tl_decode_batched_variant_compiled(int MB, int GPW) { return qmm6_variant_in_table(MB, GPW) ? 1 : 0; }
extern "C" int tl_decode_streaming_plan(int M, int rows, int cols, int *out4) {
    if (!out4 || M < 1 || rows <= 0 || cols <= 0) return 0;
    const Qmm7Plan pl = qmm7_plan(M, cols, rows);
    out4[0] = pl.MB, out4[1] = pl.T, out4[2] = pl.GPW, out4[3] = pl.wgs;
    return pl.ok ? 1 : 0;
}
extern "C" int tl_decode_streaming_variant_compiled(int T, int GPW) { return qmm7_variant_in_table(T, GPW) ? 1 : 0; }
extern "C" int tl_decode_attention_plan(int batch, int max_context, int num_heads, int num_kv_heads, int *out3) {
    if (!out3 || batch < 1 || max_context < 0 || num_heads <= 0 || num_kv_heads <= 0 || num_heads % num_kv_heads != 0) return 0;
    tl_engine e;
    e.cfg.num_heads = num_heads;
    e.cfg.num_kv_heads = num_kv_heads;
    e.cfg.head_dim = 128;
    e.cfg.page_size = 128;
    read_attention_knobs(&e);
    const SplitPlan sp = pick_decode_splits(&e, batch, std::max(1, max_context + 1));
    out3[0] = sp.n_splits, out3[1] = sp.tokens_per_split, out3[2] = sp.rq;
    return 1;
}

extern "C" int tl_kv_copy_rows(const tl_kv_pool_desc *pools_dev, int n_pools, int heads, int page_size, int from_page, int to_page,
                               int rows, void *stream) {
    return kv_copy_rows(pools_dev, n_pools, heads, page_size, from_page, to_page, rows, (hipStream_t)stream);
}

extern "C" size_t tl_kv_page_record_bytes(const tl_kv_pool_desc *pools_host, int n_pools, int heads, int page_size) {
    return kv_page_record_bytes(pools_host, n_pools, heads, page_size);
}
extern "C" int tl_kv_gather_pages(const tl_kv_pool_desc *pools_dev, const size_t *record_offsets_dev, int n_pools, int heads, int page_size,
                                  const int32_t *page_ids_dev, int n_pages, int tail_rows, void *staging_dev, size_t record_bytes, void *stream) {
    return kv_swap_pages<true>(pools_dev, record_offsets_dev, n_pools, heads, page_size, page_ids_dev, n_pages, tail_rows, staging_dev, record_bytes,
                               (hipStream_t)stream);
}
extern "C" int tl_kv_scatter_pages(const tl_kv_pool_desc *pools_dev, const size_t *record_offsets_dev, int n_pools, int heads, int page_size,
                                   const int32_t *page_ids_dev, int n_pages, int tail_rows, const void *staging_dev, size_t record_bytes, void *stream) {
    return kv_swap_pages<false>(pools_dev, record_offsets_dev, n_pools, heads, page_size, page_ids_dev, n_pages, tail_rows, (void *)staging_dev,
                                record_bytes, (hipStream_t)stream);
}
```

### tiny-llm_amd/csrc/qmv3.h

```cpp
#pragma once
#include "common.h"
#include "qmv.h"

namespace tl {

constexpr int Q3_LMAX = 10;
constexpr int Q3_PAD = 8;

struct Qmv3Args {
    const uint32_t *wt;
    const uint32_t *sbt;
    const uint16_t *a;
    uint16_t *out;
    const uint16_t *norm_w;
    const uint16_t *residual;
    float eps;
    int M, N, K;
    prof_t *prof;
#ifdef QMV3_TRACE
#define Q3_STAMP(i) do { if (p.trace && threadIdx.x == 0) p.trace[(size_t)blockIdx.x * 8 + (i)] = wall_clock64(); } while (0)
#else
#define Q3_STAMP(i) do { } while (0)
#endif
#ifdef QMV3_LAB
    int ablate;
#endif
#ifdef QMV3_TRACE
    unsigned long long *trace;
#endif
    const float *merge_ws;
    const float *ss_in;
    int ss_n;
    float *ss_out;
    const uint16_t *norm_out;
    uint16_t *out_w;
    f32x2 *tile_max;
};

#ifndef Q3_STORE_MODE
#define Q3_STORE_MODE 0
#endif
template <typename T> __device__ __forceinline__ void q3_store(T *ptr, T v) {
#if Q3_STORE_MODE == 1
    __builtin_nontemporal_store(v, ptr);
#elif Q3_STORE_MODE == 2
    __hip_atomic_store(ptr, v, __ATOMIC_RELAXED, __HIP_MEMORY_SCOPE_SYSTEM);
#else
    act_store(ptr, v);
#endif
}
#ifdef QMV3_LAB
#define Q3_ABL(bit) (p.ablate & (bit))
#else
#define Q3_ABL(bit) 0
#endif

__host__ __device__ inline size_t qmv3_lds_xsum_off(int MR, int N) {
    return (((size_t)MR * (N + Q3_PAD) + (size_t)Q3_LMAX * 128) * 2 + 15) & ~(size_t)15;
}
__host__ __device__ inline size_t qmv3_lds_red_off(int MR, int N) {
    return qmv3_lds_xsum_off(MR, N) + (size_t)(N / 128 + Q3_LMAX) * 16 * 4;
}
__host__ __device__ inline size_t qmv3_lds_bytes(int MR, int N, int KS, int CW) {
    size_t red = KS > 1 ? (size_t)CW * MR * 16 * 4 : 0;
    return qmv3_lds_red_off(MR, N) + red + (size_t)MR * CW * 4 + 64;
}

__device__ __forceinline__ u32x4 unpack_w4_bf16(uint32_t w, uint32_t mask_s, uint32_t magic_v) {
    return u32x4{(w & mask_s) | magic_v, ((w >> 4) & mask_s) | magic_v, ((w >> 8) & mask_s) | magic_v,
                 ((w >> 12) & mask_s) | magic_v};
}

template <int MR, int KS, int CW, int PRO, int EPI, int LM, int NS = 0>
__global__ __launch_bounds__(CW * 64) void qmv3_kernel(const Qmv3Args p) {
    static_assert(PRO != PRO_ATTN_MERGE || (MR == 1 && (NS == 2 || NS == 4 || NS == 8)), "PRO_ATTN_MERGE: one row, 2 / 4 / 8 splits");
    extern __shared__ __attribute__((aligned(16))) char smem[];
    constexpr int T = CW * 64;
    constexpr int WR = CW / KS;
    constexpr int ROWS = MR < 4 ? MR : 4;
    const prof_t prof_t0 = prof_begin(p.prof);
    Q3_STAMP(0);
    const int tid = threadIdx.x;
    const int wave = __builtin_amdgcn_readfirstlane(tid >> 6);
    const int lane = tid & 63;
    const int N = p.N, K = p.K, G = N >> 7;
    const int xstride = N + Q3_PAD;
    uint16_t *xs = reinterpret_cast<uint16_t *>(smem);
    float *xsum = reinterpret_cast<float *>(smem + qmv3_lds_xsum_off(MR, N));
    float *red = reinterpret_cast<float *>(smem + qmv3_lds_red_off(MR, N));

    const int r = lane & 15;
    const int c = lane >> 4;
    const int wt = wave / KS;
    const int ks = wave - wt * KS;
    const int tiles = K >> 4;
    const int tile = blockIdx.x * WR + wt;
    const bool tile_ok = tile < tiles;
    const int tile_c = tile_ok ? tile : 0;
    const int Lper = (G + KS - 1) / KS;
    const int g0 = ks * Lper;
    const int g1 = min(g0 + Lper, G);

    const int cpr = N >> 3;
    constexpr int CCU = MR <= 2 ? 3 : 2;
    const bool reg_path = cpr <= CCU * T;
    u32x4 xv[CCU][MR], nwv[CCU];
    constexpr int MS = PRO == PRO_ATTN_MERGE ? NS : 1;
    constexpr int MCCU = PRO == PRO_ATTN_MERGE ? 2 : 1;
    constexpr int MWS = 128 + 4;
    f32x4 mval[MCCU][MS][2];
    f32x2 mml[MCCU][MS];
    if constexpr (PRO == PRO_ATTN_MERGE) {
#pragma unroll
        for (int k = 0; k < MCCU; ++k) {
            const int cc = min(tid + k * T, cpr - 1);
            const float *hb = p.merge_ws + (size_t)(cc >> 4) * NS * MWS;
#pragma unroll
            for (int s2 = 0; s2 < NS; ++s2) mml[k][s2] = act_load(reinterpret_cast<const f32x2 *>(hb + s2 * MWS + 128));
#pragma unroll
            for (int s2 = 0; s2 < NS; ++s2)
#pragma unroll
                for (int e = 0; e < 2; ++e) mval[k][s2][e] = act_load(reinterpret_cast<const f32x4 *>(hb + s2 * MWS + (cc & 15) * 8 + 4 * e));
        }
    }
    const int orow = (tile_c << 4) + r;
    uint16_t resv[ROWS], nwo = 0;
    if constexpr (EPI == EPI_RESIDUAL) {
#pragma unroll
        for (int i2 = 0; i2 < ROWS; ++i2) {
            const int arow = 4 * c + i2;
            resv[i2] = act_load(p.residual + (size_t)((arow < MR && arow < p.M) ? arow : 0) * K + orow);
        }
        nwo = (p.out_w ? p.norm_out : p.residual)[orow];
    }
    constexpr bool NORMED = PRO == PRO_RMSNORM || PRO == PRO_RMS_WEIGHTED;
    const bool ss_given = NORMED && p.ss_in != nullptr && reg_path && p.ss_n <= 256 && (p.ss_n & 3) == 0;
    f32x4 ssv[MR];
    if constexpr (NORMED) {
#pragma unroll
        for (int m = 0; m < MR; ++m) {
            const bool ok = ss_given && m < p.M && 4 * lane < p.ss_n;
            const float *src = ss_given ? p.ss_in : reinterpret_cast<const float *>(p.norm_w);
            const f32x4 v = act_load(reinterpret_cast<const f32x4 *>(src + (ok ? (size_t)m * p.ss_n + 4 * lane : 0)));
            ssv[m] = ok ? v : f32x4{0.f, 0.f, 0.f, 0.f};
        }
    }
#pragma unroll
    for (int k = 0; k < CCU; ++k) {
        const int cc = tid + k * T;
        const bool okc = reg_path && cc < cpr;
        const size_t coff = (size_t)(okc ? cc : 0) * 8;
#pragma unroll
        for (int m = 0; m < MR; ++m) {
            if constexpr (PRO == PRO_ATTN_MERGE) {
                xv[k][m] = u32x4{0u, 0u, 0u, 0u};
                continue;
            }
            const bool ok = okc && m < p.M;
            if (Q3_ABL(4)) {
                xv[k][m] = u32x4{0x3f803f80u, 0x3f803f80u, 0x3f803f80u, 0x3f803f80u};
                continue;
            }
            xv[k][m] = act_load(reinterpret_cast<const u32x4 *>(p.a + (ok ? (size_t)m * N + coff : 0)));
            if (!ok) xv[k][m] = u32x4{0u, 0u, 0u, 0u};
        }
        if constexpr (PRO == PRO_RMSNORM)
            nwv[k] = *reinterpret_cast<const u32x4 *>(p.norm_w + coff);
        else
            nwv[k] = u32x4{0u, 0u, 0u, 0u};
    }
    Q3_STAMP(1);
    __builtin_amdgcn_sched_barrier(0);
    u32x4 wq[LM];
    uint32_t sq[LM];
    {
        const uint32_t *sp = p.sbt + (size_t)tile_c * G * 16 + r;
#pragma unroll
        for (int i = 0; i < LM; ++i) sq[i] = sp[(size_t)min(g0 + i, G - 1) * 16];
        const u32x4 *wp = reinterpret_cast<const u32x4 *>(p.wt) + (size_t)tile_c * G * 64 + lane;
#pragma unroll
        for (int i = 0; i < LM; ++i) wq[i] = __builtin_nontemporal_load(wp + (size_t)min(g0 + i, G - 1) * 64);
    }
    __builtin_amdgcn_sched_barrier(0);
    Q3_STAMP(2);

    {
        u32x4 *zx = reinterpret_cast<u32x4 *>(xs + (size_t)MR * xstride);
        for (int i = tid; i < Q3_LMAX * 16; i += T) zx[i] = u32x4{0u, 0u, 0u, 0u};
        if (tid < MR) *reinterpret_cast<u32x4 *>(xs + (size_t)tid * xstride + N) = u32x4{0u, 0u, 0u, 0u};
        f32x4 *zs = reinterpret_cast<f32x4 *>(xsum + (size_t)G * 16);
        for (int i = tid; i < Q3_LMAX * 4; i += T) zs[i] = f32x4{0.f, 0.f, 0.f, 0.f};
    }
    auto chunk_sumsq = [](const u32x4 &v) {
        float part = 0.f;
#pragma unroll
        for (int e = 0; e < 4; ++e) {
            const float lo = BF16::to_float((uint16_t)(v[e] & 0xffffu));
            const float hi = BF16::to_float((uint16_t)(v[e] >> 16));
            part += lo * lo + hi * hi;
        }
        return part;
    };
    auto finish_chunk = [&](int m, int cc, u32x4 v, const u32x4 &g, float iv) {
        float f[8];
#pragma unroll
        for (int e = 0; e < 4; ++e) {
            f[2 * e] = BF16::to_float((uint16_t)(v[e] & 0xffffu));
            f[2 * e + 1] = BF16::to_float((uint16_t)(v[e] >> 16));
        }
        if constexpr (PRO == PRO_RMSNORM) {
#pragma unroll
            for (int e = 0; e < 4; ++e) {
                f[2 * e] = bf16_round(f[2 * e] * iv * BF16::to_float((uint16_t)(g[e] & 0xffffu)));
                f[2 * e + 1] = bf16_round(f[2 * e + 1] * iv * BF16::to_float((uint16_t)(g[e] >> 16)));
                v[e] = BF16::pack2(f[2 * e], f[2 * e + 1]);
            }
        }
        *reinterpret_cast<u32x4 *>(xs + (size_t)m * xstride + (size_t)cc * 8) = v;
        float sum = ((f[0] + f[1]) + (f[2] + f[3])) + ((f[4] + f[5]) + (f[6] + f[7]));
        sum = group16_sum(sum);
        if ((cc & 15) == 0) xsum[(cc >> 4) * 16 + m] = sum;
    };
    if constexpr (PRO == PRO_ATTN_MERGE) {
#pragma unroll
        for (int k = 0; k < MCCU; ++k) {
            float gm = -1e30f;
#pragma unroll
            for (int s2 = 0; s2 < NS; ++s2) gm = fmaxf(gm, mml[k][s2][0]);
            float gl = 0.f, f2[NS];
#pragma unroll
            for (int s2 = 0; s2 < NS; ++s2) {
                f2[s2] = exp2_hw(mml[k][s2][0] - gm);
                gl += mml[k][s2][1] * f2[s2];
            }
            float o[8];
#pragma unroll
            for (int e = 0; e < 8; ++e) {
                float acc1 = 0.f;
#pragma unroll
                for (int s2 = 0; s2 < NS; ++s2) acc1 += mval[k][s2][e >> 2][e & 3] * f2[s2];
                o[e] = gl == 0.f ? 0.f : acc1 / gl;
            }
            const bool okc = reg_path && tid + k * T < cpr;
#pragma unroll
            for (int e = 0; e < 4; ++e) xv[k][0][e] = okc ? BF16::pack2(o[2 * e], o[2 * e + 1]) : 0u;
        }
    }
    float inv[MR];
#pragma unroll
    for (int m = 0; m < MR; ++m) inv[m] = 1.0f;
    auto inv_from_partials = [&]() {
#pragma unroll
        for (int m = 0; m < MR; ++m) {
            float v = (ssv[m][0] + ssv[m][1]) + (ssv[m][2] + ssv[m][3]);
            v = wave_sum(v);
            inv[m] = rsqrtf(v / (float)N + p.eps);
        }
    };
    if constexpr (PRO == PRO_RMSNORM) {
      if (ss_given) {
        inv_from_partials();
      } else if (!Q3_ABL(8)) {
        float ss[MR];
#pragma unroll
        for (int m = 0; m < MR; ++m) ss[m] = 0.f;
        if (reg_path) {
#pragma unroll
            for (int k = 0; k < CCU; ++k)
#pragma unroll
                for (int m = 0; m < MR; ++m) ss[m] += chunk_sumsq(xv[k][m]);
        } else {
            for (int cc = tid; cc < cpr; cc += T) {
#pragma unroll
                for (int m = 0; m < MR; ++m) {
                    const bool ok = m < p.M;
                    u32x4 v = act_load(reinterpret_cast<const u32x4 *>(p.a + (ok ? ((size_t)m * N + (size_t)cc * 8) : 0)));
                    if (!ok) v = u32x4{0u, 0u, 0u, 0u};
                    *reinterpret_cast<u32x4 *>(xs + (size_t)m * xstride + (size_t)cc * 8) = v;
                    ss[m] += chunk_sumsq(v);
                }
            }
        }
        float *scratch = red + (KS > 1 ? (size_t)CW * MR * 16 : 0);
#pragma unroll
        for (int m = 0; m < MR; ++m) {
            const float v = wave_sum(ss[m]);
            if (lane == 0) scratch[m * CW + wave] = v;
        }
        __syncthreads();
#pragma unroll
        for (int m = 0; m < MR; ++m) {
            float tot = 0.f;
#pragma unroll
            for (int w = 0; w < CW; ++w) tot += scratch[m * CW + w];
            inv[m] = rsqrtf(tot / (float)N + p.eps);
        }
      }
    }
    if (reg_path && !Q3_ABL(2)) {
#pragma unroll
        for (int k = 0; k < CCU; ++k) {
            const int cc = tid + k * T;
            if (cc < cpr) {
#pragma unroll
                for (int m = 0; m < MR; ++m) finish_chunk(m, cc, xv[k][m], nwv[k], inv[m]);
            }
        }
    } else if (!reg_path) {
        for (int cc = tid; cc < cpr; cc += T) {
            u32x4 g = u32x4{0u, 0u, 0u, 0u};
            if constexpr (PRO == PRO_RMSNORM) g = *reinterpret_cast<const u32x4 *>(p.norm_w + (size_t)cc * 8);
#pragma unroll
            for (int m = 0; m < MR; ++m) {
                u32x4 v;
                if constexpr (PRO == PRO_RMSNORM) {
                    v = *reinterpret_cast<const u32x4 *>(xs + (size_t)m * xstride + (size_t)cc * 8);
                } else {
                    const bool ok = m < p.M;
                    v = act_load(reinterpret_cast<const u32x4 *>(p.a + (ok ? ((size_t)m * N + (size_t)cc * 8) : 0)));
                    if (!ok) v = u32x4{0u, 0u, 0u, 0u};
                }
                finish_chunk(m, cc, v, g, inv[m]);
            }
        }
    }
    __syncthreads();
    Q3_STAMP(3);

    float acc[ROWS];
#pragma unroll
    for (int i2 = 0; i2 < ROWS; ++i2) acc[i2] = 0.f;
    const uint16_t *xbase = xs + (size_t)(r % MR) * xstride + 32 * c + (size_t)g0 * 128;
    const float *sbase = xsum + (size_t)g0 * 16 + 4 * c;
    uint32_t nib_mask = 0x000f000fu;
    uint32_t magic = 0x43004300u;
    asm volatile("" : "+s"(nib_mask));
    asm volatile("" : "+v"(magic));
#pragma unroll
    for (int i = 0; i < LM; ++i) {
        if (Q3_ABL(1)) {
            acc[0] += __uint_as_float((wq[i][0] ^ wq[i][1] ^ wq[i][2] ^ wq[i][3]) & 0x3fffffffu) + __uint_as_float(sq[i] & 0x3fffffffu);
            continue;
        }
        f32x4 d = {0.f, 0.f, 0.f, 0.f};
#pragma unroll
        for (int t = 0; t < 4; ++t) {
            const u32x4 bq = unpack_w4_bf16(wq[i][t], nib_mask, magic);
            const u32x4 ax = *reinterpret_cast<const u32x4 *>(xbase + i * 128 + 8 * t);
            d = __builtin_amdgcn_mfma_f32_16x16x32_bf16(__builtin_bit_cast(bf16x8_t, ax), __builtin_bit_cast(bf16x8_t, bq), d,
                                                        0, 0, 0);
        }
        const uint32_t sw = (g0 + i) < g1 ? sq[i] : 0u;
        const float sc = __uint_as_float(sw << 16);
        const float be = __uint_as_float(sw & 0xffff0000u) - 128.0f * sc;
        if constexpr (ROWS == 4) {
            const f32x4 xg = *reinterpret_cast<const f32x4 *>(sbase + i * 16);
#pragma unroll
            for (int i2 = 0; i2 < 4; ++i2) acc[i2] += sc * d[i2] + be * xg[i2];
        } else {
#pragma unroll
            for (int i2 = 0; i2 < ROWS; ++i2) acc[i2] += sc * d[i2] + be * sbase[i * 16 + i2];
        }
    }

    Q3_STAMP(4);
    if constexpr (KS > 1) {
#pragma unroll
        for (int i2 = 0; i2 < ROWS; ++i2) {
            const int arow = 4 * c + i2;
            if (arow < MR) red[((size_t)wave * MR + arow) * 16 + r] = acc[i2];
        }
        __syncthreads();
        if (ks != 0) {
            prof_end(p.prof, prof_t0);
            return;
        }
#pragma unroll
        for (int i2 = 0; i2 < ROWS; ++i2) {
            const int arow = 4 * c + i2;
            if (arow < MR) {
#pragma unroll
                for (int k2 = 1; k2 < KS; ++k2) acc[i2] += red[((size_t)(wave + k2) * MR + arow) * 16 + r];
            }
        }
    }

    if constexpr (PRO == PRO_RMS_WEIGHTED) {
        inv_from_partials();
#pragma unroll
        for (int i2 = 0; i2 < ROWS; ++i2) acc[i2] *= (MR > 4 && c == 1) ? inv[(4 + i2) % MR] : inv[i2 % MR];
    }
#pragma unroll
    for (int i2 = 0; i2 < ROWS; ++i2) {
        const int arow = 4 * c + i2;
        const bool live = tile_ok && arow < MR && arow < p.M;
        if constexpr (EPI == EPI_SWIGLU) {
            const float gv = bf16_round(acc[i2]);
            const float uv = lane_xor1(gv);
            if (live && (r & 1) == 0)
                q3_store(&p.out[(size_t)arow * (K >> 1) + (orow >> 1)], BF16::from_float((gv / (1.0f + expf(-gv))) * uv));
        } else if constexpr (EPI == EPI_RESIDUAL) {
            float sq_v = 0.f;
            if (live) {
                const size_t o = (size_t)arow * K + orow;
                const uint16_t ov = BF16::from_float(BF16::to_float(resv[i2]) + bf16_round(acc[i2]));
                q3_store(&p.out[o], ov);
                sq_v = BF16::to_float(ov) * BF16::to_float(ov);
                if (p.out_w) q3_store(&p.out_w[o], BF16::from_float(BF16::to_float(ov) * BF16::to_float(nwo)));
            }
            if (p.ss_out) {
                sq_v = group16_sum(sq_v);
                if (r == 0 && tile_ok && arow < MR && arow < p.M) q3_store(&p.ss_out[(size_t)arow * tiles + tile_c], sq_v);
            }
        } else {
            const uint16_t ov = BF16::from_float(acc[i2]);
            if (live) q3_store(&p.out[(size_t)arow * K + orow], ov);
            if (p.tile_max) {
                const float v = live ? BF16::to_float(ov) : -INFINITY;
                const float m = group16_max(v);
                const float cand = (v == m && live) ? (float)orow : 3.0e38f;
                const float lowest = -group16_max(-cand);
                if (r == 0 && tile_ok && arow < MR && arow < p.M) act_store(&p.tile_max[(size_t)arow * tiles + tile_c], f32x2{m, lowest});
            }
        }
    }
    Q3_STAMP(5);
    prof_end(p.prof, prof_t0);
}

struct Qmv3Plan {
    int MR, KS, CW, LM, blocks;
    size_t lds;
    bool ok;
};
inline bool qmv3_has_variant(int MR, int KS, int CW, int LM) {
    const bool mr = MR == 1 || MR == 2 || MR == 4 || MR == 8;
    const bool lm4 = LM == 4 || LM == 5 || LM == 8 || LM == 10, hi = LM == 8 || LM == 10;
    if (CW == 4 && KS == 1) return mr && lm4;
    if (CW == 4 && (KS == 2 || KS == 4)) return mr && (MR == 8 ? hi : lm4);
    if (CW == 8 && KS == 8) return mr && hi && !(MR == 4 && LM == 10);
    return MR == 4 && KS == 16 && CW == 16 && (LM == 4 || LM == 5);
}
inline int qmv3_round_lm(int lper) { return lper <= 4 ? 4 : (lper <= 5 ? 5 : (lper <= 8 ? 8 : Q3_LMAX)); }
inline Qmv3Plan qmv3_plan(int M, int N, int K, int force_ks = 0, int force_cw = 0) {
    Qmv3Plan pl{};
    pl.MR = M <= 1 ? 1 : (M <= 2 ? 2 : (M <= 4 ? 4 : 8));
    const int G = N / 128;
    const int tiles = K / 16;
    int ks = 1;
    while (ks < 8 && (G + ks - 1) / ks > Q3_LMAX) ks *= 2;
    {
        const int blocks = (tiles + (4 / ks) - 1) / (4 / (ks > 4 ? 4 : ks));
        const double x = blocks / 256.0;
        const double rounds = (double)(int)(x + 0.999999);
        if (M <= 4 && ks < 4 && x >= 1.0 && x < 4.0 && rounds / x > 1.2 && (G + 2 * ks - 1) / (2 * ks) >= 4) ks *= 2;
    }
    if (pl.MR == 4 && ks == 8 && (G + 15) / 16 >= 4 && (G + 15) / 16 <= 5) ks = 16;
    if (force_ks > 0) ks = force_ks;
    pl.KS = ks;
    pl.CW = ks >= 8 ? ks : 4;
    if (force_cw > 0 && force_cw >= ks) pl.CW = force_cw;
    pl.LM = qmv3_round_lm((G + ks - 1) / ks);
    const int wr = pl.CW / pl.KS;
    pl.blocks = (tiles + wr - 1) / wr;
    pl.lds = qmv3_lds_bytes(pl.MR, N, pl.KS, pl.CW);
    pl.ok = K > 0 && K % 16 == 0 && N % 128 == 0 && M >= 1 && M <= 8 && (G + ks - 1) / ks <= Q3_LMAX &&
            pl.lds <= 150 * 1024 && qmv3_has_variant(pl.MR, pl.KS, pl.CW, pl.LM);
    return pl;
}

inline bool qmv3_takes_weighted_rows(const Qmv3Plan &pl, int N, int ss_n) {
    return pl.ok && N / 8 <= (pl.MR <= 2 ? 3 : 2) * pl.CW * 64 && ss_n > 0 && ss_n <= 256 && (ss_n & 3) == 0;
}

bool qmv3_variant_in_table(int MR, int KS, int CW, int LM);
int launch_qmv3_bf16(const Qmv3Args &args, int pro, int epi, hipStream_t st, int force_ks = 0, int force_cw = 0);
int launch_qmv3_attn_merge_bf16(const Qmv3Args &args, int n_splits, hipStream_t st);
int repack_w4_tiled(const uint32_t *w, const uint16_t *scales, const uint16_t *biases, uint32_t *wt, uint32_t *sbt, int K,
                    int N, hipStream_t st);

}
```

### tiny-llm_amd/csrc/qmv3.hip

```cpp
#include "qmv3.h"

namespace tl {

__global__ __launch_bounds__(256) void repack_w4_tiled_kernel(const uint32_t *__restrict__ w,
                                                              const uint16_t *__restrict__ scales,
                                                              const uint16_t *__restrict__ biases,
                                                              uint32_t *__restrict__ wt, uint32_t *__restrict__ sbt, int K,
                                                              int N) {
    const int G = N >> 7, words = N >> 3;
    const size_t total = (size_t)K * words;
    const size_t idx = (size_t)blockIdx.x * 256 + threadIdx.x;
    if (idx < total) {
        const int t = (int)(idx & 3);
        const int lane = (int)((idx >> 2) & 63);
        const size_t tg = idx >> 8;
        const int g = (int)(tg % G);
        const size_t tile = tg / G;
        const int r = lane & 15, c = lane >> 4;
        const uint32_t v = w[(tile * 16 + r) * words + g * 16 + 4 * c + t];
        uint32_t o = 0;
#pragma unroll
        for (int i = 0; i < 4; ++i) {
            o |= ((v >> (8 * i)) & 0xfu) << (4 * i);
            o |= ((v >> (8 * i + 4)) & 0xfu) << (4 * i + 16);
        }
        wt[idx] = o;
    }
    const size_t stotal = (size_t)K * G;
    if (idx < stotal) {
        const int r = (int)(idx & 15);
        const size_t tg = idx >> 4;
        const int g = (int)(tg % G);
        const size_t tile = tg / G;
        const size_t src = (tile * 16 + r) * G + g;
        sbt[idx] = (uint32_t)scales[src] | ((uint32_t)biases[src] << 16);
    }
}

int repack_w4_tiled(const uint32_t *w, const uint16_t *scales, const uint16_t *biases, uint32_t *wt, uint32_t *sbt, int K,
                    int N, hipStream_t st) {
    const size_t total = (size_t)K * (N / 8);
    hipLaunchKernelGGL(repack_w4_tiled_kernel, dim3((unsigned)((total + 255) / 256)), dim3(256), 0, st, w, scales, biases, wt,
                       sbt, K, N);
    return hipGetLastError() == hipSuccess ? 0 : -1;
}

#define Q3_LM4(X, MRv, KSv, CWv) X(MRv, KSv, CWv, 4) X(MRv, KSv, CWv, 5) X(MRv, KSv, CWv, 8) X(MRv, KSv, CWv, 10)
#define Q3_LMHI(X, MRv, KSv, CWv) X(MRv, KSv, CWv, 8) X(MRv, KSv, CWv, 10)
#define Q3_TABLE(X)                                                                                                     \
    Q3_LM4(X, 1, 1, 4) Q3_LM4(X, 1, 2, 4) Q3_LM4(X, 1, 4, 4) Q3_LMHI(X, 1, 8, 8)                                        \
    Q3_LM4(X, 2, 1, 4) Q3_LM4(X, 2, 2, 4) Q3_LM4(X, 2, 4, 4) Q3_LMHI(X, 2, 8, 8)                                        \
    Q3_LM4(X, 4, 1, 4) Q3_LM4(X, 4, 2, 4) Q3_LM4(X, 4, 4, 4) X(4, 8, 8, 8)                                              \
    X(4, 16, 16, 4) X(4, 16, 16, 5)    \
    Q3_LM4(X, 8, 1, 4) Q3_LMHI(X, 8, 2, 4) Q3_LMHI(X, 8, 4, 4) Q3_LMHI(X, 8, 8, 8)

bool qmv3_variant_in_table(int MR, int KS, int CW, int LM) {
#define Q3_MEMBER(MRv, KSv, CWv, LMv) if (MR == MRv && KS == KSv && CW == CWv && LM == LMv) return true;
    Q3_TABLE(Q3_MEMBER)
#undef Q3_MEMBER
    return false;
}

template <int PRO, int EPI>
static int launch_variant3(const Qmv3Args &args, hipStream_t st, int force_ks, int force_cw) {
    const Qmv3Plan pl = qmv3_plan(args.M, args.N, args.K, force_ks, force_cw);
    if (!pl.ok) return -1;
    const dim3 grid(pl.blocks), block(pl.CW * 64);
#define Q3_CASE(MRv, KSv, CWv, LMv)                                                                                 \
    if (pl.MR == MRv && pl.KS == KSv && pl.CW == CWv && pl.LM == LMv) {                                             \
        auto kern = qmv3_kernel<MRv, KSv, CWv, PRO, EPI, LMv>;                                                      \
        if (pl.lds > 64 * 1024)                                                                                     \
            (void)hipFuncSetAttribute((const void *)kern, hipFuncAttributeMaxDynamicSharedMemorySize, (int)pl.lds); \
        hipLaunchKernelGGL(kern, grid, block, pl.lds, st, args);                                                    \
        return 0;                                                                                                   \
    }
    Q3_TABLE(Q3_CASE)
#undef Q3_CASE
    return -2;
}

template <int NS>
static int launch_merge_variant3(const Qmv3Args &args, hipStream_t st, const Qmv3Plan &pl) {
    const dim3 grid(pl.blocks), block(pl.CW * 64);
#define Q3_MCASE(KSv, CWv, LMv)                                                                                      \
    if (pl.KS == KSv && pl.CW == CWv && pl.LM == LMv) {                                                              \
        auto kern = qmv3_kernel<1, KSv, CWv, PRO_ATTN_MERGE, EPI_RESIDUAL, LMv, NS>;                                  \
        if (pl.lds > 64 * 1024)                                                                                      \
            (void)hipFuncSetAttribute((const void *)kern, hipFuncAttributeMaxDynamicSharedMemorySize, (int)pl.lds);  \
        hipLaunchKernelGGL(kern, grid, block, pl.lds, st, args);                                                     \
        return 0;                                                                                                    \
    }
#define Q3_MLM(KSv, CWv) Q3_MCASE(KSv, CWv, 4) Q3_MCASE(KSv, CWv, 5) Q3_MCASE(KSv, CWv, 8) Q3_MCASE(KSv, CWv, 10)
    Q3_MLM(2, 4) Q3_MLM(4, 4) Q3_MCASE(8, 8, 8) Q3_MCASE(8, 8, 10)
#undef Q3_MLM
#undef Q3_MCASE
    return -1;
}
int launch_qmv3_attn_merge_bf16(const Qmv3Args &args, int n_splits, hipStream_t st) {
    if (args.M != 1 || !args.merge_ws || !args.residual || args.N % 128 != 0) return -1;
    const Qmv3Plan pl = qmv3_plan(1, args.N, args.K);
    if (!pl.ok || pl.MR != 1 || args.N / 8 > 2 * pl.CW * 64) return -1;
    if (n_splits == 2) return launch_merge_variant3<2>(args, st, pl);
    if (n_splits == 4) return launch_merge_variant3<4>(args, st, pl);
    if (n_splits == 8) return launch_merge_variant3<8>(args, st, pl);
    return -1;
}

int launch_qmv3_bf16(const Qmv3Args &args, int pro, int epi, hipStream_t st, int force_ks, int force_cw) {
    if (pro == PRO_NONE && epi == EPI_STORE) return launch_variant3<PRO_NONE, EPI_STORE>(args, st, force_ks, force_cw);
    if (pro == PRO_RMSNORM && epi == EPI_STORE) return launch_variant3<PRO_RMSNORM, EPI_STORE>(args, st, force_ks, force_cw);
    if (pro == PRO_NONE && epi == EPI_RESIDUAL) return launch_variant3<PRO_NONE, EPI_RESIDUAL>(args, st, force_ks, force_cw);
    if (pro == PRO_RMSNORM && epi == EPI_SWIGLU) return launch_variant3<PRO_RMSNORM, EPI_SWIGLU>(args, st, force_ks, force_cw);
    if (pro == PRO_RMS_WEIGHTED && epi == EPI_SWIGLU) {
        if (!args.ss_in || !qmv3_takes_weighted_rows(qmv3_plan(args.M, args.N, args.K, force_ks, force_cw), args.N, args.ss_n)) return -1;
        return launch_variant3<PRO_RMS_WEIGHTED, EPI_SWIGLU>(args, st, force_ks, force_cw);
    }
    return -2;
}

}
```

### tiny-llm_amd/extensions_hip/tiny_llm_ext_hip/__init__.py

```python

from __future__ import annotations

import ctypes
import os
from pathlib import Path

import torch

_LIB_NAME = "libtinyllm_hip.so"
_LIB_PATH = Path(__file__).resolve().parent / _LIB_NAME

if not _LIB_PATH.exists():
    raise ImportError(
        f"{_LIB_PATH} is missing: build it with `python -c 'import __graft_entry__ as g; g.build()'` "
        "or `make -C tiny-llm_amd/csrc` (hipcc, gfx950). There is no CPU fallback."
    )

_lib = ctypes.CDLL(str(_LIB_PATH), mode=os.RTLD_LOCAL if hasattr(os, "RTLD_LOCAL") else 0)

_c_void_p = ctypes.c_void_p
_c_int = ctypes.c_int
_c_float = ctypes.c_float
_c_size_t = ctypes.c_size_t

# ... 2 lines not shown

_SIGNATURES = {
    "tl_last_error": (ctypes.c_char_p, []),
    "tl_abi_version": (_c_int, []),
    "tl_load_library": (_c_int, [ctypes.c_char_p]),
    "tl_quantized_matmul": (
        _c_int,
        [_c_void_p] * 5 + [_c_int] * 5 + [_c_int, _c_int, _c_int, _c_void_p, _c_size_t, _c_void_p],
    ),
    "tl_quantized_matmul_workspace_bytes": (_c_size_t, [_c_int] * 6),
    "tl_gather_quantized_matvec": (_c_int, [_c_void_p] * 6 + [_c_int] * 7 + [_c_void_p]),
    "tl_quantized_matmul_split_k": (_c_int, [_c_int] * 5),
    "tl_quantized_embedding": (_c_int, [_c_void_p, _c_int] + [_c_void_p] * 4 + [_c_int] * 6 + [_c_void_p]),
    "tl_rms_norm": (_c_int, [_c_void_p] * 3 + [_c_int, _c_int, _c_float, _c_int, _c_void_p]),
    "tl_rope": (_c_int, [_c_void_p] * 3 + [_c_int] * 5 + [_c_float, _c_int, _c_int, _c_void_p]),
    "tl_swiglu": (_c_int, [_c_void_p] * 3 + [_c_size_t, _c_int, _c_void_p]),
    "tl_decode_attention": (_c_int, [_c_void_p] * 5 + [_c_int] * 6 + [_c_float, _c_int, _c_int, _c_int, _c_void_p]),
    "tl_paged_cache_update": (_c_int, [_c_void_p] * 2 + [_c_int] * 8 + [_c_void_p]),
    "tl_paged_attention": (
        _c_int,
        [_c_void_p] * 6 + [_c_int] * 8 + [_c_float, _c_int, _c_int, _c_int, _c_void_p, _c_size_t, _c_void_p],
    ),
    "tl_paged_attention_workspace_bytes": (_c_size_t, [_c_int] * 8),
    "tl_paged_attention_waves": (_c_int, [_c_int]),
    "tl_kv_fp8_quantize_rows": (_c_int, [_c_void_p, _c_void_p, _c_void_p, ctypes.c_long, _c_int, _c_void_p]),
    "tl_kv_fp8_dequantize_rows": (_c_int, [_c_void_p, _c_void_p, _c_void_p, ctypes.c_long, _c_int, _c_void_p]),
    "tl_paged_cache_update_fp8": (_c_int, [_c_void_p] * 3 + [_c_int] * 7 + [_c_void_p]),
    "tl_paged_attention_fp8": (
        _c_int,
        [_c_void_p] * 8 + [_c_int] * 8 + [_c_float, _c_int, _c_int, _c_void_p, _c_size_t, _c_void_p],
    ),
}



class TlW4(ctypes.Structure):
    _fields_ = [("weight_dev", _c_void_p), ("scales_dev", _c_void_p), ("biases_dev", _c_void_p),
                ("rows", _c_int), ("cols", _c_int)]


class TlLayerWeights(ctypes.Structure):
    _fields_ = [("wqkv", TlW4), ("wo", TlW4), ("wgu", TlW4), ("wdown", TlW4),
                ("input_norm_dev", _c_void_p), ("post_norm_dev", _c_void_p),
                ("q_norm_dev", _c_void_p), ("k_norm_dev", _c_void_p)]


class TlMoeWeights(ctypes.Structure):
    _fields_ = [("router", TlW4), ("gate_dev", _c_void_p), ("up_dev", _c_void_p), ("down_dev", _c_void_p),
                ("gate_scales_dev", _c_void_p), ("gate_biases_dev", _c_void_p), ("up_scales_dev", _c_void_p),
                ("up_biases_dev", _c_void_p), ("down_scales_dev", _c_void_p), ("down_biases_dev", _c_void_p),
                ("num_experts", _c_int), ("experts_per_token", _c_int), ("intermediate_size", _c_int),
                ("norm_topk_prob", _c_int)]


class TlEngineConfig(ctypes.Structure):
    _fields_ = [("hidden_size", _c_int), ("num_layers", _c_int), ("num_heads", _c_int), ("num_kv_heads", _c_int),
                ("head_dim", _c_int), ("intermediate_size", _c_int), ("vocab_size", _c_int),
                ("rope_theta", _c_float), ("rms_norm_eps", _c_float),
                ("page_size", _c_int), ("num_pages", _c_int), ("max_batch", _c_int), ("max_pages_per_seq", _c_int),
                ("max_prefill_rows", _c_int)]


class TlEngineStats(ctypes.Structure):
    _fields_ = [("pages_in_use", _c_int), ("pages_free", _c_int), ("peak_pages_in_use", _c_int),
                ("page_allocations", ctypes.c_long), ("reused_page_allocations", ctypes.c_long),
                ("decode_steps", ctypes.c_long), ("graph_captures", ctypes.c_long), ("graph_replays", ctypes.c_long),
                ("prefill_tokens", ctypes.c_long), ("kv_bytes", _c_size_t), ("workspace_bytes", _c_size_t),
                ("graph_cache_flushes", ctypes.c_long), ("aql_steps", ctypes.c_long)]


class TlStepProfile(ctypes.Structure):
    _fields_ = [("kernel_us", ctypes.c_double * 8), ("launches", _c_int * 8), ("gemv_bytes", ctypes.c_double * 5),
                ("span_us", ctypes.c_double), ("clock_khz", _c_int), ("n_splits", _c_int)]


class TlStepCheck(ctypes.Structure):
    _fields_ = [("launches", _c_int), ("written_once_plan", _c_int), ("n_splits", _c_int), ("double_writes", ctypes.c_long),
                ("elements_written", ctypes.c_long), ("first_launch", _c_int), ("first_kind", _c_int), ("first_region", _c_int),
                ("first_offset", ctypes.c_long)]


TL_MAX_TOP_LOGPROBS = 20
TL_MAX_LOGIT_BIAS = 1024


class TlTokenLogprob(ctypes.Structure):
    _fields_ = [("logprob", ctypes.c_float), ("top_ids", ctypes.c_int32 * TL_MAX_TOP_LOGPROBS),
                ("top_logprobs", ctypes.c_float * TL_MAX_TOP_LOGPROBS)]


class TlLinearInfo(ctypes.Structure):
    _fields_ = [("kernel", _c_int), ("launches", _c_int), ("rows_per_pass", _c_int), ("p", _c_int * 5)]


class TlLinearEx(ctypes.Structure):
    _fields_ = [("merge_ws_dev", _c_void_p), ("n_splits", _c_int), ("ss_in_dev", _c_void_p), ("ss_in_n", _c_int),
                ("ss_out_dev", _c_void_p), ("norm_out_dev", _c_void_p), ("out_w_dev", _c_void_p), ("fragment_order", _c_int)]


class TlPrefixStats(ctypes.Structure):
    _fields_ = [("lookups", ctypes.c_long), ("hits", ctypes.c_long), ("tokens_matched", ctypes.c_long),
                ("tail_rows_copied", ctypes.c_long), ("pages_registered", ctypes.c_long), ("pages_evicted", ctypes.c_long),
                ("entries", _c_int), ("pages_retained", _c_int), ("max_retained_pages", _c_int), ("enabled", _c_int)]


class TlKvPoolDesc(ctypes.Structure):
    _fields_ = [("base_dev", _c_void_p), ("row_bytes", _c_size_t)]


class TlSwapStats(ctypes.Structure):
    _fields_ = [("host_pages", _c_int), ("host_pages_in_use", _c_int), ("parks", ctypes.c_long), ("unparks", ctypes.c_long),
                ("pages_out", ctypes.c_long), ("pages_in", ctypes.c_long), ("record_bytes", _c_size_t)]


TL_MAX_LORA_RANK = 64
TL_MAX_LORA_ADAPTERS = 32
LORA_TARGETS = ("q", "k", "v", "o", "gate", "up", "down")
LORA_MODES = {"add": 0, "residual_pre": 1, "swiglu": 2}
LORA_SEG_MODES = {"plain": 0, "blocks": 1, "interleaved": 2}


class TlLoraLayer(ctypes.Structure):
    _fields_ = [("a_dev", _c_void_p * len(LORA_TARGETS)), ("b_dev", _c_void_p * len(LORA_TARGETS))]


class TlLoraStats(ctypes.Structure):
    _fields_ = [("resident", _c_int), ("bytes", _c_size_t), ("adapter_steps", ctypes.c_long), ("adapter_prefill_rows", ctypes.c_long)]


class TlLoraMatrices(ctypes.Structure):
    _fields_ = [("a_dev", _c_void_p), ("b_dev", _c_void_p), ("rank", _c_int), ("seg_mask", _c_int), ("scale", _c_float)]


TL_MAX_STOP_IDS = 16
TL_MAX_STOP_STRINGS = 16
TL_MAX_STOP_BYTES = 1024
STOP_REASONS = ("none", "id", "string", "length")


class TlStopState(ctypes.Structure):
    _fields_ = [("reason", ctypes.c_int32), ("index", ctypes.c_int32), ("generated", ctypes.c_int32), ("context", ctypes.c_int32),
                ("text_bytes", ctypes.c_uint32), ("cut_bytes", ctypes.c_uint32)]


class TlAttentionInfo(ctypes.Structure):
    _fields_ = [("n_splits", _c_int), ("tokens_per_split", _c_int), ("heads_per_workgroup", _c_int),
                ("launches", _c_int)]


_P = ctypes.POINTER
_SIGNATURES.update({
    "tl_tiled_w4_create": (_c_int, [_P(TlW4), _c_void_p, _P(_c_void_p)]),
    "tl_tiled_w4_destroy": (None, [_c_void_p]),
    "tl_decode_linear_workspace_bytes": (_c_size_t, [_c_int, _c_int, _c_int]),
    "tl_decode_linear": (_c_int, [_c_void_p, _c_void_p, _c_void_p, _c_int, _c_int, _c_int, _c_void_p, _c_void_p, _c_float,
                                  _c_int, _c_void_p, _c_size_t, _c_void_p, _P(TlLinearInfo)]),
    "tl_decode_linear_ex": (_c_int, [_c_void_p, _c_void_p, _c_void_p, _c_int, _c_int, _c_int, _c_void_p, _c_void_p, _c_float,
                                     _c_int, _c_void_p, _c_size_t, _c_void_p, _P(TlLinearEx), _P(TlLinearInfo)]),
    "tl_prefill_weights_bf16": (_c_int, [_P(TlW4), _c_void_p, _c_void_p]),
    "tl_prefill_matmul_bf16": (_c_int, [_c_void_p, _c_void_p, _c_void_p, _c_int, _c_int, _c_int, _c_int, _c_void_p, _c_void_p]),
    "tl_decode_gemv_variant_compiled": (_c_int, [_c_int, _c_int, _c_int, _c_int]),
    "tl_decode_attention_fused_workspace_bytes": (_c_size_t, [_c_int, _c_int, _c_int]),
    "tl_decode_attention_fused": (_c_int, [_c_void_p] * 8 + [_c_int] * 6 + [_c_float, _c_float, _c_int, _c_void_p, _c_size_t,
                                                             _c_void_p, _P(TlAttentionInfo)]),
    "tl_engine_profile_step": (_c_int, [_c_void_p, _c_int, _P(TlStepProfile)]),
    "tl_engine_check_step": (_c_int, [_c_void_p, _c_int, _P(TlStepCheck)]),
    "tl_engine_create": (_c_int, [_P(TlEngineConfig), _P(TlLayerWeights), _P(TlW4), _c_void_p, _P(TlW4), _c_void_p,
                                  _P(_c_void_p)]),
    "tl_engine_create_kv": (_c_int, [_P(TlEngineConfig), _P(TlLayerWeights), _P(TlW4), _c_void_p, _P(TlW4), _c_void_p, _c_int,
                                     _P(_c_void_p)]),
    "tl_engine_kv_format": (_c_int, [_c_void_p]),
    "tl_decode_attention_fused_fp8": (_c_int, [_c_void_p] * 10 + [_c_int] * 6 + [_c_float, _c_float, _c_int, _c_void_p, _c_size_t,
                                                                  _c_void_p, _P(TlAttentionInfo)]),
    "tl_engine_set_moe_layer": (_c_int, [_c_void_p, _c_int, _P(TlMoeWeights)]),
    "tl_decode_gemv_plan": (_c_int, [_c_int, _c_int, _c_int, _P(_c_int)]),
    "tl_decode_batched_plan": (_c_int, [_c_int, _c_int, _c_int, _P(_c_int)]),
    "tl_decode_batched_variant_compiled": (_c_int, [_c_int, _c_int]),
    "tl_decode_streaming_plan": (_c_int, [_c_int, _c_int, _c_int, _P(_c_int)]),
    "tl_decode_streaming_variant_compiled": (_c_int, [_c_int, _c_int]),
    "tl_decode_attention_plan": (_c_int, [_c_int, _c_int, _c_int, _c_int, _P(_c_int)]),
    "tl_engine_set_option": (_c_int, [_c_void_p, ctypes.c_char_p, _c_int]),
    "tl_engine_destroy": (None, [_c_void_p]),
    "tl_engine_synchronize": (_c_int, [_c_void_p]),
    "tl_engine_begin": (_c_int, [_c_void_p, _c_int]),
    "tl_engine_reserve": (_c_int, [_c_void_p, _c_int, _c_int]),
    "tl_engine_release": (_c_int, [_c_void_p, _c_int]),
    "tl_engine_rewind": (_c_int, [_c_void_p, _c_int, _c_int]),
    "tl_engine_context_len": (_c_int, [_c_void_p, _c_int]),
    "tl_engine_move": (_c_int, [_c_void_p, _c_int, _c_int]),
    "tl_engine_fork": (_c_int, [_c_void_p, _c_int, _c_int]),
    "tl_engine_read_pending": (_c_int, [_c_void_p, _c_int, _P(ctypes.c_int32)]),
    "tl_engine_prefix_cache": (_c_int, [_c_void_p, _c_int, _c_int]),
    "tl_engine_prefix_attach": (_c_int, [_c_void_p, _c_int, _P(ctypes.c_int32), _c_int, _P(_c_int)]),
    "tl_engine_prefix_extend": (_c_int, [_c_void_p, _c_int, _P(ctypes.c_int32), _c_int]),
    "tl_engine_prefix_clear": (_c_int, [_c_void_p]),
    "tl_engine_prefix_stats": (_c_int, [_c_void_p, _P(TlPrefixStats)]),
    "tl_kv_copy_rows": (_c_int, [_c_void_p, _c_int, _c_int, _c_int, _c_int, _c_int, _c_int, _c_void_p]),
    "tl_engine_swap_space": (_c_int, [_c_void_p, _c_int]),
    "tl_engine_park": (_c_int, [_c_void_p, _c_int]),
    "tl_engine_unpark": (_c_int, [_c_void_p, _c_int]),
    "tl_engine_slot_parked": (_c_int, [_c_void_p, _c_int]),
    "tl_engine_step_pages": (_c_int, [_c_void_p, _c_int, _P(_c_int), _P(_c_int)]),
    "tl_engine_swap_stats": (_c_int, [_c_void_p, _P(TlSwapStats)]),
    "tl_kv_page_record_bytes": (_c_size_t, [_c_void_p, _c_int, _c_int, _c_int]),
    "tl_kv_gather_pages": (_c_int, [_c_void_p, _c_void_p, _c_int, _c_int, _c_int, _c_void_p, _c_int, _c_int, _c_void_p, _c_size_t, _c_void_p]),
    "tl_kv_scatter_pages": (_c_int, [_c_void_p, _c_void_p, _c_int, _c_int, _c_int, _c_void_p, _c_int, _c_int, _c_void_p, _c_size_t, _c_void_p]),
    "tl_engine_prefill": (_c_int, [_c_void_p, _c_int, _P(ctypes.c_int32), _c_int, _c_int]),
    "tl_engine_prefill_packed": (_c_int, [_c_void_p, _c_int, _P(ctypes.c_int), _P(ctypes.c_int32), _P(ctypes.c_int), _P(ctypes.c_int)]),
    "tl_engine_verify": (_c_int, [_c_void_p, _c_int, _P(ctypes.c_int32), _c_int, _P(ctypes.c_int32)]),
    "tl_engine_verify_sampled": (_c_int, [_c_void_p, _c_int, _P(ctypes.c_int32), _c_int, _c_void_p, ctypes.c_float, _c_int, ctypes.c_float,
                                          _P(ctypes.c_int32), _P(_c_int)]),
    "tl_engine_set_token": (_c_int, [_c_void_p, _c_int, ctypes.c_int32]),
    "tl_engine_set_sampling": (_c_int, [_c_void_p, _c_int, _c_float, _c_int, _c_float, ctypes.c_uint64]),
    "tl_sample_logits": (_c_int, [_c_void_p, _c_int, _c_int] + [_c_void_p] * 7),
    "tl_engine_set_logprobs": (_c_int, [_c_void_p, _c_int, _c_int]),
    "tl_engine_set_penalties": (_c_int, [_c_void_p, _c_int, _c_float, _c_float, _c_float]),
    "tl_engine_set_logit_bias": (_c_int, [_c_void_p, _c_int, _P(ctypes.c_int32), _P(_c_float), _c_int]),
    "tl_process_logits": (_c_int, [_c_void_p, _c_int, _c_int] + [_c_void_p] * 9),
    "tl_engine_set_truncation": (_c_int, [_c_void_p, _c_int, _c_float, _c_float]),
    "tl_engine_set_mirostat": (_c_int, [_c_void_p, _c_int, _c_float, _c_float]),
    "tl_engine_mirostat_mu": (_c_int, [_c_void_p, _c_int, _P(_c_float)]),
    "tl_engine_copy_filtered_logits": (_c_int, [_c_void_p, _c_void_p, _c_int]),
    "tl_truncate_rows": (_c_int, [_c_void_p, _c_int, _c_int] + [_c_void_p] * 7),
    "tl_spec_sample_rows": (_c_int, [_c_void_p, _c_void_p, _c_int, _c_int] + [_c_void_p] * 12),
    "tl_mirostat_update_rows": (_c_int, [_c_void_p, _c_int, _c_int] + [_c_void_p] * 7),
    "tl_vocab_create": (_c_int, [_c_int, _c_void_p, _c_void_p, _c_void_p, _P(_c_void_p)]),
    "tl_vocab_destroy": (None, [_c_void_p]),
    "tl_grammar_create": (_c_int, [_c_void_p, _c_int, _c_void_p, _c_void_p, _c_int, _c_void_p, _c_int, _c_void_p, _P(_c_void_p)]),
    "tl_grammar_destroy": (None, [_c_void_p]),
    "tl_engine_set_grammar": (_c_int, [_c_void_p, _c_int, _c_void_p]),
    "tl_engine_grammar_state": (_c_int, [_c_void_p, _c_int, _P(_c_int), _P(_c_int)]),
    "tl_grammar_mask_rows": (_c_int, [_c_void_p, _c_void_p, _c_int, _c_void_p, _c_void_p, _c_void_p]),
    "tl_grammar_create_stack": (_c_int, [_c_void_p, _c_int, _c_void_p, _c_void_p, _c_int, _c_void_p, _c_void_p, _c_int, _c_void_p, _c_int,
                                         _c_void_p, _P(_c_void_p)]),
    "tl_engine_grammar_config": (_c_int, [_c_void_p, _c_int, _P(_c_int), _P(_c_int), _P(ctypes.c_uint64), _P(_c_int)]),
    "tl_grammar_mask_rows_stack": (_c_int, [_c_void_p, _c_void_p, _c_int, _c_void_p, _c_void_p, _c_void_p, _c_void_p, _c_void_p]),
    "tl_engine_read_logprobs": (_c_int, [_c_void_p, _c_int, _c_int, _P(TlTokenLogprob)]),
    "tl_engine_read_pending_logprobs": (_c_int, [_c_void_p, _c_int, _P(TlTokenLogprob)]),
    "tl_engine_score": (_c_int, [_c_void_p, _c_int, _P(ctypes.c_int32), _c_int, ctypes.c_int32, _P(_c_float), _P(ctypes.c_int32)]),
    "tl_logprob_rows": (_c_int, [_c_void_p, _c_int, _c_int, _c_void_p, _c_int, _c_void_p, _c_void_p, _c_void_p, _c_void_p]),
    "tl_engine_embed_packed": (_c_int, [_c_void_p, _c_int, _P(ctypes.c_int), _P(ctypes.c_int32), _P(ctypes.c_int), _P(ctypes.c_int), _c_int, _c_int,
                                        _c_int, _P(_c_float)]),
    "tl_engine_embed": (_c_int, [_c_void_p, _c_int, _P(ctypes.c_int32), _c_int, _c_int, _c_int, _c_int, _c_int, _P(_c_float)]),
    "tl_pool_rows": (_c_int, [_c_void_p, _c_int, _c_int, _P(ctypes.c_int), _P(ctypes.c_int), _P(ctypes.c_int), _P(ctypes.c_int), _c_int, _c_void_p,
                              _c_int, _c_int, _c_void_p, _c_void_p]),
    "tl_engine_lora_load": (_c_int, [_c_void_p, _P(TlLoraLayer), _c_int, _c_float, _P(_c_int)]),
    "tl_engine_lora_unload": (_c_int, [_c_void_p, _c_int]),
    "tl_engine_set_lora": (_c_int, [_c_void_p, _c_int, _c_int]),
    "tl_engine_slot_lora": (_c_int, [_c_void_p, _c_int]),
    "tl_engine_lora_stats": (_c_int, [_c_void_p, _P(TlLoraStats)]),
    "tl_lora_rows": (_c_int, [_c_void_p, _c_int, _c_int, _c_int, _c_void_p, _P(TlLoraMatrices), _c_int, _c_int, _c_int, _c_int, _P(ctypes.c_int),
                              _P(ctypes.c_int), _P(ctypes.c_int), _c_int, _c_int, _c_void_p, _c_void_p, _c_void_p, _c_float, _c_void_p]),
    "tl_stop_create": (_c_int, [_c_void_p, _P(ctypes.c_int32), _c_int, _c_void_p, _P(ctypes.c_int32), _c_int, _c_void_p, _P(_c_void_p)]),
    "tl_stop_destroy": (None, [_c_void_p]),
    "tl_engine_set_stop": (_c_int, [_c_void_p, _c_int, _c_void_p, _c_int]),
    "tl_engine_stop_state": (_c_int, [_c_void_p, _c_int, _P(TlStopState)]),
    "tl_stop_rows": (_c_int, [_c_void_p, _c_void_p, _c_int, _c_void_p, _c_void_p, _c_void_p, _c_void_p, _c_void_p]),
    "tl_engine_decode": (_c_int, [_c_void_p, _c_int, _c_int, _c_int]),
    "tl_engine_read_tokens": (_c_int, [_c_void_p, _c_int, _c_int, _P(ctypes.c_int32)]),
    "tl_engine_logits_dev": (_c_void_p, [_c_void_p]),
    "tl_engine_copy_logits": (_c_int, [_c_void_p, _c_void_p, _c_int]),
    "tl_engine_copy_processed_logits": (_c_int, [_c_void_p, _c_void_p, _c_int]),
    "tl_engine_tokens_dev": (_c_void_p, [_c_void_p]),
    "tl_engine_get_stats": (_c_int, [_c_void_p, _P(TlEngineStats)]),
    "tl_engine_replay_route": (ctypes.c_char_p, [_c_void_p]),
    "tl_engine_step_bytes": (_c_size_t, [_c_void_p, _c_int]),
})

for _name, (_res, _args) in _SIGNATURES.items():
    _fn = getattr(_lib, _name)
    _fn.restype = _res
    _fn.argtypes = _args


def _bind_optional(name: str, restype, argtypes) -> bool:
    fn = getattr(_lib, name, None)
    if fn is None:
        return False
    fn.restype = restype
    fn.argtypes = argtypes
    return True


def lib() -> ctypes.CDLL:
    return _lib


def check(status: int) -> None:
    _check(status)


def library_path() -> str:
    return str(_LIB_PATH)


def _check(status: int) -> None:
    if status != 0:
        message = _lib.tl_last_error()
        raise RuntimeError(message.decode() if message else f"tinyllm_hip error {status}")


def _stream() -> int:
    return torch.cuda.current_stream().cuda_stream


def _require_gpu(op: str, *tensors: torch.Tensor) -> None:
# ... 215 lines not shown
    if (
        query.dim() != 3 or key.dim() != 3 or value.dim() != 3 or query.shape[2] > 256
        or query.shape[2] != key.shape[2] or query.shape[2] != value.shape[2] or key.shape != value.shape
        or num_heads % num_kv_heads != 0
    ):
        raise RuntimeError("decode_attention: incompatible attention shapes")
    if has_mask and (
        mask.dim() != 3 or mask.shape[0] != query.shape[0] or mask.shape[1] != query.shape[1]
        or mask.shape[2] != key.shape[1]
    ):
        raise RuntimeError("decode_attention: mask must have shape [B*Hq,L,S]")
    _require_gpu("decode_attention", query, key, value)
    if has_mask:
        _require_gpu("decode_attention", mask)
    query, key, value, mask = query.contiguous(), key.contiguous(), value.contiguous(), mask.contiguous()
    out = torch.empty_like(query)
    q_rows, L, D = query.shape
    S = key.shape[1]
    _check(
        _lib.tl_decode_attention(
            _ptr(query), _ptr(key), _ptr(value), _ptr(mask) if has_mask else None, _ptr(out), q_rows, L, S, D,
            int(num_heads), int(num_kv_heads), float(scale), int(bool(is_causal)), int(bool(has_mask)),
            _DTYPES[query.dtype], _stream(),
        )
    )
    return out


def paged_cache_update(pages: torch.Tensor, values: torch.Tensor, page_id: int, start: int, stream=None) -> torch.Tensor:
    if pages.dtype not in (torch.float32, torch.bfloat16) or values.dtype != pages.dtype:
        raise RuntimeError("paged_cache_update: pages and values must have the same float32 or bfloat16 dtype")
    if pages.dim() != 4 or values.dim() != 4 or values.shape[0] != 1:
        raise RuntimeError("paged_cache_update: expected pages [P, H, page_size, D] and values [1, H, length, D]")
    if values.shape[1] != pages.shape[1] or values.shape[3] != pages.shape[3]:
        raise RuntimeError("paged_cache_update: values must match the page head count and head dimension")
    if page_id < 0 or page_id >= pages.shape[0] or start < 0 or start + values.shape[2] > pages.shape[2]:
        raise RuntimeError("paged_cache_update: destination slice is outside page storage")
    _require_gpu("paged_cache_update", pages, values)
    if not pages.is_contiguous() or not values.is_contiguous():
        raise RuntimeError("paged_cache_update: pages and values must be contiguous")
    P, H, page_size, D = pages.shape
    _check(
        _lib.tl_paged_cache_update(_ptr(pages), _ptr(values), P, H, page_size, D, values.shape[2], int(page_id),
                                   int(start), _DTYPES[pages.dtype], _stream())
    )
    return pages


def paged_attention(
    query: torch.Tensor,
    key_pages: torch.Tensor,
    value_pages: torch.Tensor,
    block_table: torch.Tensor,
    context_lens: torch.Tensor,
    scale: float = 1.0,
    is_causal: bool = False,
    *,
    num_kv_heads: int,
    num_heads: int,
    stream=None,
    max_context_hint: int = 0,
) -> torch.Tensor:
    if query.dtype not in (torch.float32, torch.bfloat16) or key_pages.dtype != query.dtype \
            or value_pages.dtype != query.dtype:
        raise RuntimeError(
            "paged_attention: q, key_pages, and value_pages must have the same float32 or bfloat16 dtype")
    if block_table.dtype != torch.int32 or context_lens.dtype != torch.int32:
        raise RuntimeError("paged_attention: block_table and context_lens must be int32")
    if query.dim() != 3:
        raise RuntimeError("paged_attention: q must be 3D [B * H_q, L, D]")
    if key_pages.dim() != 4 or value_pages.dim() != 4:
        raise RuntimeError("paged_attention: page tensors must be 4D [P, H_kv, page_size, D]")
    if block_table.dim() != 2 or context_lens.dim() != 1:
        raise RuntimeError("paged_attention: block_table must be 2D and context_lens must be 1D")
    if num_heads % num_kv_heads != 0:
        raise RuntimeError("paged_attention: num_heads must be divisible by num_kv_heads")
    if query.shape[0] % num_heads != 0:
        raise RuntimeError("paged_attention: q.shape[0] must be divisible by num_heads")
    if key_pages.shape != value_pages.shape:
        raise RuntimeError("paged_attention: key_pages and value_pages must have the same shape")
    if key_pages.shape[1] != num_kv_heads:
        raise RuntimeError("paged_attention: page tensor head count must equal num_kv_heads")
    if query.shape[2] != key_pages.shape[3]:
        raise RuntimeError("paged_attention: q and page tensors must have the same head dimension")
    if block_table.shape[0] != context_lens.shape[0]:
        raise RuntimeError("paged_attention: block_table and context_lens batch sizes must match")
    if query.shape[0] // num_heads != block_table.shape[0]:
        raise RuntimeError("paged_attention: q batch size must match block_table batch size")
    _require_gpu("paged_attention", query, key_pages, value_pages, block_table, context_lens)
    N, L, D = query.shape
    P, _, page_size, _ = key_pages.shape
    max_pages = block_table.shape[1]
    if D > 128:
        raise RuntimeError("paged_attention: head dimension must be at most 128")
    if L > 8 and query.dtype == torch.bfloat16 and D != 128:
        raise RuntimeError("paged_attention: bfloat16 prefill requires head dimension 128")
    for name, t in (("q", query), ("key_pages", key_pages), ("value_pages", value_pages),
                    ("block_table", block_table), ("context_lens", context_lens)):
        if not t.is_contiguous():
            raise RuntimeError(f"paged_attention: {name} must be contiguous")
    out = torch.empty_like(query)
    ws_bytes = _lib.tl_paged_attention_workspace_bytes(N, L, D, page_size, max_pages, num_heads, num_kv_heads,
                                                       int(max_context_hint))
    ws = _workspace(ws_bytes, query.device)
    _check(
        _lib.tl_paged_attention(
            _ptr(query), _ptr(key_pages), _ptr(value_pages), _ptr(block_table), _ptr(context_lens), _ptr(out), N, L,
            D, P, page_size, max_pages, int(num_heads), int(num_kv_heads), float(scale), int(bool(is_causal)),
            int(max_context_hint), _DTYPES[query.dtype], _ptr(ws) if ws is not None else None,
            ws.numel() if ws is not None else 0, _stream(),
        )
    )
    return out


__all__ = [
    "load_library",
    "quantized_matmul",
    "gather_quantized_matvec",
    "quantized_embedding",
    "rms_norm",
    "rope",
    "swiglu",
    "decode_attention",
    "paged_cache_update",
    "paged_attention",
]


PRO_NONE, PRO_RMSNORM, PRO_ATTN_MERGE, PRO_RMS_WEIGHTED = 0, 1, 2, 3
EPI_STORE, EPI_RESIDUAL, EPI_SWIGLU = 0, 1, 2
ATTN_PARTIAL_ROW = 128 + 4
LINEAR_KERNELS = {1: "qmv3 (fused MFMA GEMV)", 2: "qmm3 (skinny MFMA matmul + slice reduction)",
                  3: "qmv (packed-dot GEMV fallback)", 4: "prefill GEMM path", 5: "qmm6 (register-resident batched matmul)"}


class TiledW4:

    def __init__(self, weight: torch.Tensor, scales: torch.Tensor, biases: torch.Tensor):
        _require_gpu("TiledW4", weight, scales, biases)
        if weight.dtype not in (torch.int32, torch.uint32) or weight.dim() != 2:
            raise RuntimeError("TiledW4: weight must be a 2-D uint32 tensor [rows, cols/8]")
        if scales.dtype != torch.bfloat16 or biases.dtype != torch.bfloat16:
            raise RuntimeError("TiledW4: the decode path is bfloat16")
        self.weight, self.scales, self.biases = weight.contiguous(), scales.contiguous(), biases.contiguous()
        self.rows, self.cols = int(weight.shape[0]), int(weight.shape[1]) * 8
        if tuple(self.scales.shape) != (self.rows, self.cols // 128) or self.scales.shape != self.biases.shape:
            raise RuntimeError("TiledW4: scales / biases must be [rows, cols/128]")
        w4 = TlW4(_ptr(self.weight), _ptr(self.scales), _ptr(self.biases), self.rows, self.cols)
        handle = _c_void_p()
        _check(_lib.tl_tiled_w4_create(ctypes.byref(w4), _stream(), ctypes.byref(handle)))
        self._h = handle

    def close(self) -> None:
        if getattr(self, "_h", None):
            torch.cuda.synchronize()
            _lib.tl_tiled_w4_destroy(self._h)
            self._h = None

    def __del__(self):
        try:
            self.close()
        except Exception:
            pass


def decode_linear(w: TiledW4, a: torch.Tensor | None, *, prologue: int = PRO_NONE, epilogue: int = EPI_STORE,
                  norm_weight: torch.Tensor | None = None, residual: torch.Tensor | None = None, eps: float = 1e-6,
                  kernel: int = 0, merge_partials: torch.Tensor | None = None, ss_in: torch.Tensor | None = None,
                  want_ss_out: bool = False, norm_out: torch.Tensor | None = None, fragment_order: bool = False,
                  fragment_rows: int | None = None):
    extended = merge_partials is not None or ss_in is not None or want_ss_out or norm_out is not None or fragment_order \
        or prologue in (PRO_ATTN_MERGE, PRO_RMS_WEIGHTED)
    if prologue == PRO_ATTN_MERGE:
        if merge_partials is None or a is not None:
            raise RuntimeError("decode_linear: the merging prologue takes merge_partials and no activation rows")
        _require_gpu("decode_linear", merge_partials)
        if merge_partials.dtype != torch.float32 or merge_partials.dim() != 3 or not merge_partials.is_contiguous() \
                or merge_partials.shape[0] * 128 != w.cols or merge_partials.shape[2] != ATTN_PARTIAL_ROW:
            raise RuntimeError("decode_linear: merge_partials must be contiguous float32 [cols / 128, n_splits, 132]")
        M, device = 1, merge_partials.device
    else:
        _require_gpu("decode_linear", a)
        if a.dtype != torch.bfloat16 or a.dim() != 2 or a.shape[1] != w.cols or not a.is_contiguous():
            raise RuntimeError("decode_linear: a must be a contiguous bfloat16 [M, cols] tensor")
        M, device = int(a.shape[0]), a.device
        if fragment_order and prologue == PRO_RMS_WEIGHTED:
            if M % 16 != 0 or fragment_rows is None or not (M - 16 < fragment_rows <= M):
                raise RuntimeError("decode_linear: rows in fragment order come as [ceil16(M), cols] with fragment_rows = M")
            M = int(fragment_rows)
    out_cols = w.rows // 2 if epilogue == EPI_SWIGLU else w.rows
    out = torch.empty((M, out_cols), dtype=torch.bfloat16, device=device)
    if residual is not None and (residual.dtype != torch.bfloat16 or tuple(residual.shape) != (M, w.rows)
                                 or not residual.is_contiguous()):
        raise RuntimeError("decode_linear: residual must be a contiguous bfloat16 [M, rows] tensor")
    if norm_weight is not None and (norm_weight.dtype != torch.bfloat16 or tuple(norm_weight.shape) != (w.cols,)):
        raise RuntimeError("decode_linear: norm_weight must be bfloat16 [cols]")
    ws_bytes = _lib.tl_decode_linear_workspace_bytes(M, w.rows, w.cols)
    ws = _workspace(ws_bytes, device)
    info = TlLinearInfo()
    common = (w._h, _ptr(a) if a is not None else None, _ptr(out), M, int(prologue), int(epilogue),
              _ptr(norm_weight) if norm_weight is not None else None, _ptr(residual) if residual is not None else None,
              float(eps), int(kernel), _ptr(ws) if ws is not None else None, ws.numel() if ws is not None else 0, _stream())
    extra = {}
    if not extended:
        _check(_lib.tl_decode_linear(*common, ctypes.byref(info)))
    else:
        ex = TlLinearEx()
        if merge_partials is not None:
            ex.merge_ws_dev, ex.n_splits = _ptr(merge_partials), int(merge_partials.shape[1])
        if ss_in is not None:
            if ss_in.dtype != torch.float32 or ss_in.dim() != 2 or ss_in.shape[0] != M or not ss_in.is_contiguous():
                raise RuntimeError("decode_linear: ss_in must be contiguous float32 [M, partials]")
            _require_gpu("decode_linear", ss_in)
            ex.ss_in_dev, ex.ss_in_n = _ptr(ss_in), int(ss_in.shape[1])
        if want_ss_out:
            extra["ss_out"] = torch.full((M, w.rows // 16), float("nan"), dtype=torch.float32, device=device)
            ex.ss_out_dev = _ptr(extra["ss_out"])
        if norm_out is not None:
            if norm_out.dtype != torch.bfloat16 or tuple(norm_out.shape) != (w.rows,):
                raise RuntimeError("decode_linear: norm_out must be bfloat16 [rows]")
            extra["out_w"] = torch.zeros(((M + 15) // 16 * 16 if fragment_order else M, w.rows), dtype=torch.bfloat16, device=device)
            ex.norm_out_dev, ex.out_w_dev = _ptr(norm_out), _ptr(extra["out_w"])
        ex.fragment_order = 1 if fragment_order else 0
        _check(_lib.tl_decode_linear_ex(*common, ctypes.byref(ex), ctypes.byref(info)))
    return out, {"kernel": info.kernel, "kernel_name": LINEAR_KERNELS.get(info.kernel, "?"), "launches": info.launches,
                 "rows_per_pass": info.rows_per_pass, "p": list(info.p), **extra}


def prefill_weights_bf16(weight: torch.Tensor, scales: torch.Tensor, biases: torch.Tensor) -> torch.Tensor:
    _require_gpu("prefill_weights_bf16", weight, scales, biases)
    rows, cols = int(weight.shape[0]), int(weight.shape[1]) * 8
    w4 = TlW4(_ptr(weight.contiguous()), _ptr(scales.contiguous()), _ptr(biases.contiguous()), rows, cols)
    out = torch.empty((rows, cols), dtype=torch.bfloat16, device=weight.device)
    _check(_lib.tl_prefill_weights_bf16(ctypes.byref(w4), _ptr(out), _stream()))
    return out


def prefill_matmul_bf16(a: torch.Tensor, w_bf16: torch.Tensor, *, epilogue: int = 0, residual: torch.Tensor | None = None) -> torch.Tensor:
    _require_gpu("prefill_matmul_bf16", a, w_bf16)
    if a.dtype != torch.bfloat16 or w_bf16.dtype != torch.bfloat16 or a.dim() != 2 or w_bf16.dim() != 2 or a.shape[1] != w_bf16.shape[1]:
        raise RuntimeError("prefill_matmul_bf16: a [M, cols] and w_bf16 [rows, cols] must be bfloat16 with the same cols")
    M, rows, cols = int(a.shape[0]), int(w_bf16.shape[0]), int(a.shape[1])
    out = torch.empty((M, rows // 2 if epilogue == 2 else rows), dtype=torch.bfloat16, device=a.device)
    res = residual.contiguous() if residual is not None else None
    _check(_lib.tl_prefill_matmul_bf16(_ptr(a.contiguous()), _ptr(w_bf16.contiguous()), _ptr(out), M, rows, cols, int(epilogue),
                                       _ptr(res) if res is not None else None, _stream()))
    return out


def fragment_order_of(rows: torch.Tensor) -> torch.Tensor:
    M, cols = rows.shape
    pad = (M + 15) // 16 * 16
    x = torch.zeros((pad, cols), dtype=rows.dtype, device=rows.device)
    x[:M] = rows
    x = x.reshape(pad // 16, 16, cols // 128, 4, 4, 8)
    return x.permute(0, 2, 4, 3, 1, 5).contiguous().reshape(pad, cols)


def rows_from_fragment_order(frag: torch.Tensor, M: int) -> torch.Tensor:
    pad, cols = frag.shape
    x = frag.reshape(pad // 16, cols // 128, 4, 4, 16, 8)
    return x.permute(0, 4, 1, 3, 2, 5).contiguous().reshape(pad, cols)[:M]


def decode_attention_fused(qkv: torch.Tensor, q_norm: torch.Tensor, k_norm: torch.Tensor, key_pages: torch.Tensor,
                           value_pages: torch.Tensor, block_table: torch.Tensor, context_lens: torch.Tensor, *,
                           num_heads: int, num_kv_heads: int, rope_theta: float, eps: float,
                           max_context: int) -> tuple[torch.Tensor, dict]:
    _require_gpu("decode_attention_fused", qkv, q_norm, k_norm, key_pages, value_pages, block_table, context_lens)
    B = int(qkv.shape[0])
    P, Hkv, page, D = (int(x) for x in key_pages.shape)
    if Hkv != num_kv_heads or tuple(value_pages.shape) != tuple(key_pages.shape):
        raise RuntimeError("decode_attention_fused: page pools must be [P, num_kv_heads, page_size, D] and alike")
    if qkv.dim() != 2 or qkv.shape[1] != (num_heads + 2 * num_kv_heads) * D:
        raise RuntimeError("decode_attention_fused: qkv must be [batch, (Hq + 2 Hkv) * D]")
    for name, t in (("qkv", qkv), ("key_pages", key_pages), ("value_pages", value_pages), ("q_norm", q_norm),
                    ("k_norm", k_norm)):
        if t.dtype != torch.bfloat16 or not t.is_contiguous():
            raise RuntimeError(f"decode_attention_fused: {name} must be contiguous bfloat16")
    if block_table.dtype != torch.int32 or context_lens.dtype != torch.int32 or block_table.dim() != 2 \
            or block_table.shape[0] != B or tuple(context_lens.shape) != (B,):
        raise RuntimeError("decode_attention_fused: block_table [B, max_pages] and context_lens [B] must be int32")
    out = torch.empty((B, num_heads * D), dtype=torch.bfloat16, device=qkv.device)
    ws_bytes = _lib.tl_decode_attention_fused_workspace_bytes(B, num_heads, D)
    ws = _workspace(ws_bytes, qkv.device)
    info = TlAttentionInfo()
    _check(_lib.tl_decode_attention_fused(_ptr(qkv), _ptr(q_norm), _ptr(k_norm), _ptr(key_pages), _ptr(value_pages),
                                          _ptr(block_table.contiguous()), _ptr(context_lens), _ptr(out), B, num_heads,
                                          num_kv_heads, D, page, int(block_table.shape[1]), float(rope_theta), float(eps),
                                          int(max_context), _ptr(ws), ws.numel(), _stream(), ctypes.byref(info)))
    return out, {name: getattr(info, name) for name, _ in info._fields_}


KV_BF16, KV_FP8_E4M3 = 0, 1


def kv_fp8_quantize_rows(values: torch.Tensor) -> tuple[torch.Tensor, torch.Tensor]:
    _require_gpu("kv_fp8_quantize_rows", values)
    if values.dtype != torch.bfloat16 or values.shape[-1] != 128 or not values.is_contiguous():
        raise RuntimeError("kv_fp8_quantize_rows: contiguous bfloat16 rows of 128 values")
    rows = values.numel() // 128
    codes = torch.empty(values.shape, dtype=torch.uint8, device=values.device)
    scales = torch.empty(values.shape[:-1], dtype=torch.float32, device=values.device)
    _check(_lib.tl_kv_fp8_quantize_rows(_ptr(values), _ptr(codes), _ptr(scales), rows, 128, _stream()))
    return codes, scales
# ... 373 lines not shown
```

Before: 964.5 tokens/s.

## Add slice-major scale/bias layout for one-row qmv3 decode GEMV

Adds a second copy of each tiled int4 weight's scales and biases, repacked slice-major so every lane's LM scale words sit next to each other. These can then be loaded with vector loads instead of LM strided scalar loads. The one-row qmv3 kernel gets a SLICED template variant, and optionally a trimmed chunk-set count, which the engine selects for CW=4 non-merge plans. This costs extra device memory for the duplicated scales and more kernel instantiations.

```diff
diff --git a/include/tinyllm_engine.h b/include/tinyllm_engine.h
--- a/include/tinyllm_engine.h
+++ b/include/tinyllm_engine.h
@@ -251,6 +251,8 @@
 typedef struct tl_tiled_w4 tl_tiled_w4;
 int tl_tiled_w4_create(const tl_w4 *w, void *stream, tl_tiled_w4 **out);
 void tl_tiled_w4_destroy(tl_tiled_w4 *t);
+int tl_tiled_w4_set_sliced_scales(tl_tiled_w4 *t, int on);
+int tl_tiled_w4_sliced_scales(const tl_tiled_w4 *t, int *out2);
 
 typedef struct tl_linear_info {
     int kernel;
@@ -284,6 +286,9 @@
 
 int tl_decode_gemv_plan(int M, int rows, int cols, int *out5);
 int tl_decode_gemv_variant_compiled(int MR, int KS, int CW, int LM);
+long tl_decode_gemv_sbs_offset(int KS, int LM, int tile, int ks, int r, int i);
+int tl_decode_gemv_sbs_group(int G, int KS, int LM, int ks, int i);
+long tl_decode_gemv_sbs_words(int rows, int KS, int LM);
 int tl_decode_batched_plan(int M, int rows, int cols, int *out6);
 int tl_decode_batched_variant_compiled(int MB, int GPW);
 int tl_decode_streaming_plan(int M, int rows, int cols, int *out4);
diff --git a/tiny-llm_amd/csrc/decode_linear.h b/tiny-llm_amd/csrc/decode_linear.h
--- a/tiny-llm_amd/csrc/decode_linear.h
+++ b/tiny-llm_amd/csrc/decode_linear.h
@@ -68,9 +68,12 @@
 
 struct TiledW4 {
     uint32_t *wt = nullptr, *sbt = nullptr;
+    uint32_t *sbs = nullptr;
+    int sbs_ks = 0, sbs_lm = 0;
+    size_t sbs_bytes = 0;
 };
 struct TiledW4Mem {
-    DeviceBlock wt, sbt;
+    DeviceBlock wt, sbt, sbs;
 };
 static int tiled_w4_make(const tl_w4 &w, hipStream_t st, TiledW4Mem &mem, TiledW4 &t, const char *alloc_failed, const char *repack_failed) {
     const size_t wbytes = (size_t)w.rows * w.cols / 2, sbytes = (size_t)w.rows * (w.cols / 128) * 4;
@@ -80,8 +83,21 @@
     if (repack_w4_tiled(w.weight_dev, (const uint16_t *)w.scales_dev, (const uint16_t *)w.biases_dev, m.wt.at<uint32_t>(), m.sbt.at<uint32_t>(), w.rows,
                         w.cols, st) != 0)
         return fail(TL_ERR_HIP, repack_failed);
+    t = TiledW4{};
     t.wt = m.wt.at<uint32_t>(), t.sbt = m.sbt.at<uint32_t>();
     mem = std::move(m);
+    return TL_OK;
+}
+static int tiled_w4_add_sliced_scales(const tl_w4 &w, hipStream_t st, TiledW4Mem &mem, TiledW4 &t, const char *alloc_failed, const char *repack_failed, bool every_plan) {
+    const Qmv3Plan one = qmv3_plan(1, w.cols, w.rows);
+    if (!(every_plan ? one.ok : qmv3_sliced_pays(one, false))) return TL_OK;
+    const size_t bytes = qmv3_sbs_words(w.rows, one.KS, one.LM) * 4;
+    DeviceBlock b;
+    TL_TRY(b.alloc(bytes, alloc_failed));
+    if (repack_w4_sbs((const uint16_t *)w.scales_dev, (const uint16_t *)w.biases_dev, b.at<uint32_t>(), w.rows, w.cols, one.KS, one.LM, st) != 0)
+        return fail(TL_ERR_HIP, repack_failed);
+    mem.sbs = std::move(b);
+    t.sbs = mem.sbs.at<uint32_t>(), t.sbs_ks = one.KS, t.sbs_lm = one.LM, t.sbs_bytes = bytes;
     return TL_OK;
 }
 
@@ -99,6 +115,8 @@
     bool gemm_fused_epilogue = true;
     bool gemv_producer_ss = true;
     bool gemv_weighted_rows = true;
+    int qmv3_sliced_scales = 1;
+    bool qmv3_sliced_everywhere = false;
     bool fuse_norm = true;
     int qmm3_min_rows = 5;
     bool use_qmm3 = true;
@@ -202,6 +220,9 @@
             Qmv3Args a3{};
             a3.wt = tiled->second.wt;
             a3.sbt = tiled->second.sbt;
+            if (ctx.qmv3_sliced_scales && tiled->second.sbs && p3.ok && p3.MR == 1 && p3.KS == tiled->second.sbs_ks && p3.LM == tiled->second.sbs_lm &&
+                (ctx.qmv3_sliced_everywhere || qmv3_sliced_pays(p3, merge)))
+                a3.sbt = tiled->second.sbs, a3.sliced = ctx.qmv3_sliced_scales == 2 ? 1 : 3;
             a3.a = merge ? nullptr : args.a;
             a3.merge_ws = merge ? const_cast<float *>(p.merge_ws) : nullptr;
             a3.out = args.out;
@@ -462,6 +483,7 @@
     tl_w4 w{};
     tl::TiledW4 t{};
     tl::TiledW4Mem mem;
+    int sliced_scales = 1;
 };
 
 extern "C" int tl_tiled_w4_create(const tl_w4 *w, void *stream, tl_tiled_w4 **out) {
@@ -473,11 +495,25 @@
     auto t = std::make_unique<tl_tiled_w4>();
     t->w = *w;
     TL_TRY(tiled_w4_make(*w, (hipStream_t)stream, t->mem, t->t, "tiled_w4_create: hipMalloc failed", "tiled_w4_create: repack launch failed"));
+    TL_TRY(tiled_w4_add_sliced_scales(*w, (hipStream_t)stream, t->mem, t->t, "tiled_w4_create: hipMalloc failed", "tiled_w4_create: repack launch failed", true));
     *out = t.release();
     return TL_OK;
 }
 
 extern "C" void tl_tiled_w4_destroy(tl_tiled_w4 *t) { delete t; }
+
+extern "C" int tl_tiled_w4_set_sliced_scales(tl_tiled_w4 *t, int on) {
+    using namespace tl;
+    TL_REQUIRE(t, "tiled_w4_set_sliced_scales: null handle");
+    TL_REQUIRE(on >= 0 && on <= 2, "tiled_w4_set_sliced_scales: 0 (tiled array), 1 (slice-major array), 2 (slice-major array, chunk sets as over the tiled one)");
+    t->sliced_scales = on;
+    return TL_OK;
+}
+extern "C" int tl_tiled_w4_sliced_scales(const tl_tiled_w4 *t, int *out2) {
+    if (!t || !t->sliced_scales || !t->t.sbs) return 0;
+    if (out2) out2[0] = t->t.sbs_ks, out2[1] = t->t.sbs_lm;
+    return 1;
+}
 
 extern "C" size_t tl_decode_linear_workspace_bytes(int M, int rows, int cols) {
     using namespace tl;
@@ -518,7 +554,8 @@
     ctx.rms_norm_eps = eps;
     ctx.stream = (hipStream_t)stream;
     ctx.tiled[w->w.weight_dev] = w->t;
-    ctx.xn = (uint16_t *)workspace_dev;
+    ctx.qmv3_sliced_scales = w->sliced_scales, ctx.qmv3_sliced_everywhere = true;
+    ctx.xn =(uint16_t *)workspace_dev;
     const size_t xn_bytes = align_up((size_t)((M + 15) / 16 * 16) * w->w.cols * 2, 256);
     ctx.splitk_ws = (char *)workspace_dev + xn_bytes;
     ctx.splitk_ws_bytes = workspace_bytes - xn_bytes;
diff --git a/tiny-llm_amd/csrc/engine.hip b/tiny-llm_amd/csrc/engine.hip
--- a/tiny-llm_amd/csrc/engine.hip
+++ b/tiny-llm_amd/csrc/engine.hip
@@ -1472,12 +1472,14 @@
     }
 
     {
+        const char *failed = "engine_create: hipMalloc(tiled weights) failed";
+        std::vector<tl_w4> made;
         auto add_tiled = [&](const tl_w4 &w) -> bool {
             if (w.rows % 16 != 0 || w.cols % 128 != 0 || e->lin.tiled.count(w.weight_dev)) return true;
-            const char *failed = "engine_create: hipMalloc(tiled weights) failed";
             e->tiled_mem.emplace_back();
             if (tiled_w4_make(w, e->stream, e->tiled_mem.back(), e->lin.tiled[w.weight_dev], failed, failed) != TL_OK) return false;
             e->tiled_bytes += (size_t)w.rows * w.cols / 2 + (size_t)w.rows * (w.cols / 128) * 4;
+            made.push_back(w);
             return true;
         };
         bool ok = true;
@@ -1486,6 +1488,11 @@
             if (l.wgu.weight_dev) ok = ok && add_tiled(l.wgu) && add_tiled(l.wdown);
         }
         ok = ok && add_tiled(e->head());
+        for (size_t i = 0; ok && i < made.size(); ++i) {
+            TiledW4 &t = e->lin.tiled[made[i].weight_dev];
+            ok = tiled_w4_add_sliced_scales(made[i], e->stream, e->tiled_mem[e->tiled_mem.size() - made.size() + i], t, failed, failed, false) == TL_OK;
+            e->tiled_bytes += t.sbs_bytes;
+        }
         if (!ok) return fail(TL_ERR_HIP, "engine_create: hipMalloc(tiled weights) failed");
     }
     if (c.max_prefill_rows >= GEMM8_MIN_ROWS) {
@@ -1613,7 +1620,8 @@
     else if (n == "gemm8") e->lin.use_gemm8 = on;
     else if (n == "prefill_reduce_norm") e->lin.fuse_reduce_norm = on;
     else if (n == "aql_fences") e->aql_fences.inner_acquire = e->aql_fences.inner_release = on ? HSA_FENCE_SCOPE_AGENT : HSA_FENCE_SCOPE_NONE;
-    else return fail(TL_ERR_INVALID, "engine_set_option: unknown option '" + n + "' (qmm3, qmm6, qmm7, gemm8, prefill_reduce_norm, attn_qkv_partials, lmhead_tile_max, gemm_fused_epilogue, aql_fences)");
+    else if (n == "qmv3_sliced_scales") e->lin.qmv3_sliced_scales = value == 2 ? 2 : (on ? 1 : 0);
+    else return fail(TL_ERR_INVALID, "engine_set_option: unknown option '" + n + "' (qmm3, qmm6, qmm7, gemm8, prefill_reduce_norm, attn_qkv_partials, lmhead_tile_max, gemm_fused_epilogue, aql_fences, qmv3_sliced_scales)");
     return TL_OK;
 }
 
@@ -3543,6 +3551,9 @@
     return pl.ok ? 1 : 0;
 }
 extern "C" int tl_decode_gemv_variant_compiled(int MR, int KS, int CW, int LM) { return qmv3_variant_in_table(MR, KS, CW, LM) ? 1 : 0; }
+extern "C" long tl_decode_gemv_sbs_offset(int KS, int LM, int tile, int ks, int r, int i) { return (long)qmv3_sbs_offset(KS, LM, tile, ks, r, i); }
+extern "C" int tl_decode_gemv_sbs_group(int G, int KS, int LM, int ks, int i) { return qmv3_sbs_group(G, KS, LM, ks, i); }
+extern "C" long tl_decode_gemv_sbs_words(int rows, int KS, int LM) { return (long)qmv3_sbs_words(rows, KS, LM); }
 extern "C" int tl_decode_batched_plan(int M, int rows, int cols, int *out6) {
     if (!out6 || M < 1 || rows <= 0 || cols <= 0) return 0;
     const Qmm6Plan pl = qmm6_plan(M, cols, rows);
diff --git a/tiny-llm_amd/csrc/qmv3.h b/tiny-llm_amd/csrc/qmv3.h
--- a/tiny-llm_amd/csrc/qmv3.h
+++ b/tiny-llm_amd/csrc/qmv3.h
@@ -35,7 +35,33 @@
     const uint16_t *norm_out;
     uint16_t *out_w;
     f32x2 *tile_max;
+    int sliced;
 };
+
+__host__ __device__ constexpr int qmv3_sbs_row_words(int LM) {
+#ifdef Q3_SBS_PAD4
+    return (LM + 3) & ~3;
+#else
+    return LM;
+#endif
+}
+__host__ __device__ constexpr size_t qmv3_sbs_offset(int KS, int LM, int tile, int ks, int r, int i) {
+    return (((size_t)tile * KS + ks) * 16 + r) * qmv3_sbs_row_words(LM) + i;
+}
+__host__ __device__ constexpr size_t qmv3_sbs_words(int K, int KS, int LM) { return qmv3_sbs_offset(KS, LM, K / 16, 0, 0, 0); }
+__host__ __device__ constexpr int qmv3_sbs_group(int G, int KS, int LM, int ks, int i) {
+    const int lper = (G + KS - 1) / KS;
+    return i < lper && i < LM && ks * lper + i < G ? ks * lper + i : -1;
+}
+constexpr int Q3_SLICED = 16;
+constexpr int Q3_SETS(int sets) { return sets << 5; }
+
+__host__ __device__ constexpr int qmv3_max_chunk_sets(int MR) { return MR <= 2 ? 3 : 2; }
+constexpr int Q3_MERGE_SETS = 2;
+__host__ __device__ constexpr int qmv3_chunk_sets_needed(int N, int threads) { return (N / 8 + threads - 1) / threads; }
+__host__ __device__ constexpr bool qmv3_row_fits_sets(int N, int threads, int sets) { return N / 8 <= sets * threads; }
+typedef uint32_t u32x4_a4 __attribute__((ext_vector_type(4), aligned(4)));
+typedef uint32_t u32x2_a4 __attribute__((ext_vector_type(2), aligned(4)));
 
 #ifndef Q3_STORE_MODE
 #define Q3_STORE_MODE 0
@@ -71,8 +97,13 @@
                  ((w >> 12) & mask_s) | magic_v};
 }
 
-template <int MR, int KS, int CW, int PRO, int EPI, int LM, int NS = 0>
+template <int MR, int KS, int CW, int PRO, int EPI, int LM, int NSF = 0>
 __global__ __launch_bounds__(CW * 64) void qmv3_kernel(const Qmv3Args p) {
+    constexpr int NS = NSF & (Q3_SLICED - 1);
+    constexpr bool SLICED = (NSF & Q3_SLICED) != 0;
+    constexpr int SETS = NSF >> 5;
+    static_assert(SETS == 0 || (SLICED && MR == 1 && SETS <= qmv3_max_chunk_sets(MR)), "trimmed chunk sets come with the one-row sliced kernels");
+    static_assert(!SLICED || MR == 1, "the slice-major scales follow the one-row plan");
     static_assert(PRO != PRO_ATTN_MERGE || (MR == 1 && (NS == 2 || NS == 4 || NS == 8)), "PRO_ATTN_MERGE: one row, 2 / 4 / 8 splits");
     extern __shared__ __attribute__((aligned(16))) char smem[];
     constexpr int T = CW * 64;
@@ -102,11 +133,11 @@
     const int g1 = min(g0 + Lper, G);
 
     const int cpr = N >> 3;
-    constexpr int CCU = MR <= 2 ? 3 : 2;
-    const bool reg_path = cpr <= CCU * T;
+    constexpr int CCU = SETS ? SETS : qmv3_max_chunk_sets(MR);
+    const bool reg_path = qmv3_row_fits_sets(N, T, CCU);
     u32x4 xv[CCU][MR], nwv[CCU];
     constexpr int MS = PRO == PRO_ATTN_MERGE ? NS : 1;
-    constexpr int MCCU = PRO == PRO_ATTN_MERGE ? 2 : 1;
+    constexpr int MCCU = PRO == PRO_ATTN_MERGE ? Q3_MERGE_SETS : 1;
     constexpr int MWS = 128 + 4;
     f32x4 mval[MCCU][MS][2];
     f32x2 mml[MCCU][MS];
@@ -173,14 +204,37 @@
     __builtin_amdgcn_sched_barrier(0);
     u32x4 wq[LM];
     uint32_t sq[LM];
+    auto load_scales = [&]() {
+        if constexpr (SLICED) {
+            const uint32_t *sp = p.sbt + qmv3_sbs_offset(KS, LM, tile_c, ks, r, 0);
+#pragma unroll
+            for (int i = 0; i + 4 <= LM; i += 4) {
+                const u32x4_a4 v = *reinterpret_cast<const u32x4_a4 *>(sp + i);
+                sq[i] = v[0], sq[i + 1] = v[1], sq[i + 2] = v[2], sq[i + 3] = v[3];
+            }
+            if constexpr (LM % 4 >= 2) {
+                const u32x2_a4 v = *reinterpret_cast<const u32x2_a4 *>(sp + (LM & ~3));
+                sq[LM & ~3] = v[0], sq[(LM & ~3) + 1] = v[1];
+            }
+            if constexpr (LM % 2 == 1) sq[LM - 1] = sp[LM - 1];
+        } else {
+            const uint32_t *sp = p.sbt + (size_t)tile_c * G * 16 + r;
+#pragma unroll
+            for (int i = 0; i < LM; ++i) sq[i] = sp[(size_t)min(g0 + i, G - 1) * 16];
+        }
+    };
+#ifndef Q3_SCALES_LAST
+    load_scales();
+#endif
     {
-        const uint32_t *sp = p.sbt + (size_t)tile_c * G * 16 + r;
-#pragma unroll
-        for (int i = 0; i < LM; ++i) sq[i] = sp[(size_t)min(g0 + i, G - 1) * 16];
         const u32x4 *wp = reinterpret_cast<const u32x4 *>(p.wt) + (size_t)tile_c * G * 64 + lane;
 #pragma unroll
         for (int i = 0; i < LM; ++i) wq[i] = __builtin_nontemporal_load(wp + (size_t)min(g0 + i, G - 1) * 64);
     }
+#ifdef Q3_SCALES_LAST
+    __builtin_amdgcn_sched_barrier(0);
+    load_scales();
+#endif
     __builtin_amdgcn_sched_barrier(0);
     Q3_STAMP(2);
 
@@ -350,7 +404,7 @@
             d = __builtin_amdgcn_mfma_f32_16x16x32_bf16(__builtin_bit_cast(bf16x8_t, ax), __builtin_bit_cast(bf16x8_t, bq), d,
                                                         0, 0, 0);
         }
-        const uint32_t sw = (g0 + i) < g1 ? sq[i] : 0u;
+        const uint32_t sw = SLICED ? sq[i] : ((g0 + i) < g1 ? sq[i] : 0u);
         const float sc = __uint_as_float(sw << 16);
         const float be = __uint_as_float(sw & 0xffff0000u) - 128.0f * sc;
         if constexpr (ROWS == 4) {
@@ -470,13 +524,16 @@
 }
 
 inline bool qmv3_takes_weighted_rows(const Qmv3Plan &pl, int N, int ss_n) {
-    return pl.ok && N / 8 <= (pl.MR <= 2 ? 3 : 2) * pl.CW * 64 && ss_n > 0 && ss_n <= 256 && (ss_n & 3) == 0;
-}
+    return pl.ok && qmv3_row_fits_sets(N, pl.CW * 64, qmv3_max_chunk_sets(pl.MR)) && ss_n > 0 && ss_n <= 256 && (ss_n & 3) == 0;
+}
+
+inline bool qmv3_sliced_pays(const Qmv3Plan &pl, bool merge) { return pl.ok && pl.MR == 1 && pl.CW == 4 && !merge; }
 
 bool qmv3_variant_in_table(int MR, int KS, int CW, int LM);
 int launch_qmv3_bf16(const Qmv3Args &args, int pro, int epi, hipStream_t st, int force_ks = 0, int force_cw = 0);
 int launch_qmv3_attn_merge_bf16(const Qmv3Args &args, int n_splits, hipStream_t st);
 int repack_w4_tiled(const uint32_t *w, const uint16_t *scales, const uint16_t *biases, uint32_t *wt, uint32_t *sbt, int K,
                     int N, hipStream_t st);
-
-}
+int repack_w4_sbs(const uint16_t *scales, const uint16_t *biases, uint32_t *sbs, int K, int N, int KS, int LM, hipStream_t st);
+
+}
diff --git a/tiny-llm_amd/csrc/qmv3.hip b/tiny-llm_amd/csrc/qmv3.hip
--- a/tiny-llm_amd/csrc/qmv3.hip
+++ b/tiny-llm_amd/csrc/qmv3.hip
@@ -45,6 +45,26 @@
     return hipGetLastError() == hipSuccess ? 0 : -1;
 }
 
+__global__ __launch_bounds__(256) void repack_w4_sbs_kernel(const uint16_t *__restrict__ scales, const uint16_t *__restrict__ biases,
+                                                            uint32_t *__restrict__ sbs, int K, int N, int KS, int LM) {
+    const int G = N >> 7, rw = qmv3_sbs_row_words(LM);
+    const size_t idx = (size_t)blockIdx.x * 256 + threadIdx.x;
+    if (idx >= qmv3_sbs_words(K, KS, LM)) return;
+    const int i = (int)(idx % rw);
+    const int r = (int)((idx / rw) & 15);
+    const size_t ts = idx / rw >> 4;
+    const int ks = (int)(ts % KS), tile = (int)(ts / KS);
+    const int g = qmv3_sbs_group(G, KS, LM, ks, i);
+    const size_t src = ((size_t)tile * 16 + r) * G + (g < 0 ? 0 : g);
+    sbs[qmv3_sbs_offset(KS, LM, tile, ks, r, i)] = g < 0 ? 0u : ((uint32_t)scales[src] | ((uint32_t)biases[src] << 16));
+}
+
+int repack_w4_sbs(const uint16_t *scales, const uint16_t *biases, uint32_t *sbs, int K, int N, int KS, int LM, hipStream_t st) {
+    const size_t total = qmv3_sbs_words(K, KS, LM);
+    hipLaunchKernelGGL(repack_w4_sbs_kernel, dim3((unsigned)((total + 255) / 256)), dim3(256), 0, st, scales, biases, sbs, K, N, KS, LM);
+    return hipGetLastError() == hipSuccess ? 0 : -1;
+}
+
 #define Q3_LM4(X, MRv, KSv, CWv) X(MRv, KSv, CWv, 4) X(MRv, KSv, CWv, 5) X(MRv, KSv, CWv, 8) X(MRv, KSv, CWv, 10)
 #define Q3_LMHI(X, MRv, KSv, CWv) X(MRv, KSv, CWv, 8) X(MRv, KSv, CWv, 10)
 #define Q3_TABLE(X)                                                                                                     \
@@ -61,45 +81,76 @@
     return false;
 }
 
+#define Q3_LAUNCH(kern)                                                                                              \
+    do {                                                                                                             \
+        if (pl.lds > 64 * 1024)                                                                                      \
+            (void)hipFuncSetAttribute((const void *)(kern), hipFuncAttributeMaxDynamicSharedMemorySize, (int)pl.lds); \
+        hipLaunchKernelGGL(kern, dim3(pl.blocks), dim3(pl.CW * 64), pl.lds, st, args);                               \
+        return 0;                                                                                                    \
+    } while (0)
+
+template <int PRO, int EPI>
+static int launch_sliced3(const Qmv3Args &args, hipStream_t st, const Qmv3Plan &pl);
+template <int NS>
+static int launch_merge_sliced3(const Qmv3Args &args, hipStream_t st, const Qmv3Plan &pl);
+
 template <int PRO, int EPI>
 static int launch_variant3(const Qmv3Args &args, hipStream_t st, int force_ks, int force_cw) {
     const Qmv3Plan pl = qmv3_plan(args.M, args.N, args.K, force_ks, force_cw);
     if (!pl.ok) return -1;
-    const dim3 grid(pl.blocks), block(pl.CW * 64);
-#define Q3_CASE(MRv, KSv, CWv, LMv)                                                                                 \
-    if (pl.MR == MRv && pl.KS == KSv && pl.CW == CWv && pl.LM == LMv) {                                             \
-        auto kern = qmv3_kernel<MRv, KSv, CWv, PRO, EPI, LMv>;                                                      \
-        if (pl.lds > 64 * 1024)                                                                                     \
-            (void)hipFuncSetAttribute((const void *)kern, hipFuncAttributeMaxDynamicSharedMemorySize, (int)pl.lds); \
-        hipLaunchKernelGGL(kern, grid, block, pl.lds, st, args);                                                    \
-        return 0;                                                                                                   \
+    if (args.sliced) {
+        if (pl.MR != 1 || force_ks > 0 || force_cw > 0) return -1;
+        return launch_sliced3<PRO, EPI>(args, st, pl);
+    }
+#define Q3_CASE(MRv, KSv, CWv, LMv) \
+    if (pl.MR == MRv && pl.KS == KSv && pl.CW == CWv && pl.LM == LMv) Q3_LAUNCH((qmv3_kernel<MRv, KSv, CWv, PRO, EPI, LMv>));
+    Q3_TABLE(Q3_CASE)
+#undef Q3_CASE
+    return -2;
+}
+
+#define Q3_MLM(KSv, CWv) Q3_MCASE(KSv, CWv, 4) Q3_MCASE(KSv, CWv, 5) Q3_MCASE(KSv, CWv, 8) Q3_MCASE(KSv, CWv, 10)
+#define Q3_MTABLE Q3_MLM(2, 4) Q3_MLM(4, 4) Q3_MCASE(8, 8, 8) Q3_MCASE(8, 8, 10)
+template <int NS>
+static int launch_merge_variant3(const Qmv3Args &args, hipStream_t st, const Qmv3Plan &pl) {
+    if (args.sliced) return launch_merge_sliced3<NS>(args, st, pl);
+#define Q3_MCASE(KSv, CWv, LMv) \
+    if (pl.KS == KSv && pl.CW == CWv && pl.LM == LMv) Q3_LAUNCH((qmv3_kernel<1, KSv, CWv, PRO_ATTN_MERGE, EPI_RESIDUAL, LMv, NS>));
+    Q3_MTABLE
+#undef Q3_MCASE
+    return -1;
+}
+
+template <int PRO, int EPI>
+static int launch_sliced3(const Qmv3Args &args, hipStream_t st, const Qmv3Plan &pl) {
+    const bool two_sets = (args.sliced & 2) != 0 && qmv3_chunk_sets_needed(args.N, pl.CW * 64) <= 2;
+#define Q3_CASE(MRv, KSv, CWv, LMv)                                                                     \
+    if constexpr (MRv == 1) {                                                                           \
+        if (pl.KS == KSv && pl.CW == CWv && pl.LM == LMv) {                                             \
+            if (two_sets) Q3_LAUNCH((qmv3_kernel<1, KSv, CWv, PRO, EPI, LMv, Q3_SLICED | Q3_SETS(2)>)); \
+            Q3_LAUNCH((qmv3_kernel<1, KSv, CWv, PRO, EPI, LMv, Q3_SLICED>));                            \
+        }                                                                                               \
     }
     Q3_TABLE(Q3_CASE)
 #undef Q3_CASE
     return -2;
 }
-
 template <int NS>
-static int launch_merge_variant3(const Qmv3Args &args, hipStream_t st, const Qmv3Plan &pl) {
-    const dim3 grid(pl.blocks), block(pl.CW * 64);
-#define Q3_MCASE(KSv, CWv, LMv)                                                                                      \
-    if (pl.KS == KSv && pl.CW == CWv && pl.LM == LMv) {                                                              \
-        auto kern = qmv3_kernel<1, KSv, CWv, PRO_ATTN_MERGE, EPI_RESIDUAL, LMv, NS>;                                  \
-        if (pl.lds > 64 * 1024)                                                                                      \
-            (void)hipFuncSetAttribute((const void *)kern, hipFuncAttributeMaxDynamicSharedMemorySize, (int)pl.lds);  \
-        hipLaunchKernelGGL(kern, grid, block, pl.lds, st, args);                                                     \
-        return 0;                                                                                                    \
-    }
-#define Q3_MLM(KSv, CWv) Q3_MCASE(KSv, CWv, 4) Q3_MCASE(KSv, CWv, 5) Q3_MCASE(KSv, CWv, 8) Q3_MCASE(KSv, CWv, 10)
-    Q3_MLM(2, 4) Q3_MLM(4, 4) Q3_MCASE(8, 8, 8) Q3_MCASE(8, 8, 10)
-#undef Q3_MLM
+static int launch_merge_sliced3(const Qmv3Args &args, hipStream_t st, const Qmv3Plan &pl) {
+#define Q3_MCASE(KSv, CWv, LMv) \
+    if (pl.KS == KSv && pl.CW == CWv && pl.LM == LMv) Q3_LAUNCH((qmv3_kernel<1, KSv, CWv, PRO_ATTN_MERGE, EPI_RESIDUAL, LMv, NS | Q3_SLICED>));
+    Q3_MTABLE
 #undef Q3_MCASE
     return -1;
 }
+#undef Q3_MTABLE
+#undef Q3_MLM
+#undef Q3_LAUNCH
+
 int launch_qmv3_attn_merge_bf16(const Qmv3Args &args, int n_splits, hipStream_t st) {
     if (args.M != 1 || !args.merge_ws || !args.residual || args.N % 128 != 0) return -1;
     const Qmv3Plan pl = qmv3_plan(1, args.N, args.K);
-    if (!pl.ok || pl.MR != 1 || args.N / 8 > 2 * pl.CW * 64) return -1;
+    if (!pl.ok || pl.MR != 1 || !qmv3_row_fits_sets(args.N, pl.CW * 64, Q3_MERGE_SETS)) return -1;
     if (n_splits == 2) return launch_merge_variant3<2>(args, st, pl);
     if (n_splits == 4) return launch_merge_variant3<4>(args, st, pl);
     if (n_splits == 8) return launch_merge_variant3<8>(args, st, pl);
diff --git a/tiny-llm_amd/extensions_hip/tiny_llm_ext_hip/__init__.py b/tiny-llm_amd/extensions_hip/tiny_llm_ext_hip/__init__.py
--- a/tiny-llm_amd/extensions_hip/tiny_llm_ext_hip/__init__.py
+++ b/tiny-llm_amd/extensions_hip/tiny_llm_ext_hip/__init__.py
@@ -178,6 +178,11 @@
 _SIGNATURES.update({
     "tl_tiled_w4_create": (_c_int, [_P(TlW4), _c_void_p, _P(_c_void_p)]),
     "tl_tiled_w4_destroy": (None, [_c_void_p]),
+    "tl_tiled_w4_set_sliced_scales": (_c_int, [_c_void_p, _c_int]),
+    "tl_tiled_w4_sliced_scales": (_c_int, [_c_void_p, _P(_c_int)]),
+    "tl_decode_gemv_sbs_offset": (ctypes.c_long, [_c_int] * 6),
+    "tl_decode_gemv_sbs_group": (_c_int, [_c_int] * 5),
+    "tl_decode_gemv_sbs_words": (ctypes.c_long, [_c_int] * 3),
     "tl_decode_linear_workspace_bytes": (_c_size_t, [_c_int, _c_int, _c_int]),
     "tl_decode_linear": (_c_int, [_c_void_p, _c_void_p, _c_void_p, _c_int, _c_int, _c_int, _c_void_p, _c_void_p, _c_float,
                                   _c_int, _c_void_p, _c_size_t, _c_void_p, _P(TlLinearInfo)]),
@@ -699,6 +704,13 @@
         _check(_lib.tl_tiled_w4_create(ctypes.byref(w4), _stream(), ctypes.byref(handle)))
         self._h = handle
 
+    def set_sliced_scales(self, on: bool | int) -> None:
+        _check(_lib.tl_tiled_w4_set_sliced_scales(self._h, int(on)))
+
+    def sliced_scales(self) -> tuple[int, int] | None:
+        out = (_c_int * 2)()
+        return (out[0], out[1]) if _lib.tl_tiled_w4_sliced_scales(self._h, out) == 1 else None
+
     def close(self) -> None:
         if getattr(self, "_h", None):
             torch.cuda.synchronize()
```

Result: no change. 969.6 tokens/s, median of 3 (+0.5%).
